# nahomes-15/pointclouds-rs

Hardware: NVIDIA B200
Metric: sor_normals_points_per_sec (higher is better)
Workload: dtype f32

## Files before the change

include/pcr_b200.h:

```cpp
#ifndef PCR_B200_H
#define PCR_B200_H

#include <stddef.h>
#include <stdint.h>

#ifdef __cplusplus
extern "C" {
#endif

#define PCR_B200_VERSION 122

typedef enum pcr_status {
    PCR_OK = 0,
    PCR_ERR_INVALID_ARG = 1,
    PCR_ERR_NORMALS_MISMATCH = 2,
    PCR_ERR_CUDA = 3,
    PCR_ERR_NCCL = 4,
    PCR_ERR_OOM = 5,
    PCR_ERR_NO_DEVICE = 6,
    PCR_ERR_UNSUPPORTED = 7,
    PCR_ERR_CAPACITY = 8
} pcr_status;

#define PCR_MAX_K 1024

typedef struct pcr_ctx pcr_ctx;
typedef struct pcr_index pcr_index;

int pcr_version(void);
int pcr_device_count(void);
int pcr_ctx_create(int device, pcr_ctx **out);
int pcr_ctx_create_on_stream(int device, void *cuda_stream, pcr_ctx **out);
void pcr_ctx_destroy(pcr_ctx *ctx);
int pcr_ctx_synchronize(pcr_ctx *ctx);
const char *pcr_last_error(const pcr_ctx *ctx);
uint64_t pcr_ctx_launch_count(const pcr_ctx *ctx);
#define PCR_NUM_TIMING_TAGS 8
int pcr_ctx_set_timing(pcr_ctx *ctx, int enable);
int pcr_ctx_get_timing(pcr_ctx *ctx, double *ms_per_tag ,
                       uint64_t *spans_per_tag );
int pcr_ctx_get_knn_counters(pcr_ctx *ctx, uint64_t out[2]);
int pcr_ctx_set_cell_size(pcr_ctx *ctx, float cell_size);
int pcr_ctx_set_frame_stream(pcr_ctx *ctx, int enable);
#define PCR_NUM_HINT_STATS 8
int pcr_ctx_get_hint_stats(pcr_ctx *ctx, uint64_t out[PCR_NUM_HINT_STATS]);

#define PCR_UNIQUE_ID_BYTES 128
int pcr_comm_unique_id(void *out_id );
int pcr_ctx_comm_init(pcr_ctx *ctx, const void *id, int rank, int world_size);
int pcr_ctx_comm_rank(const pcr_ctx *ctx);
int pcr_ctx_comm_size(const pcr_ctx *ctx);
#define PCR_COMM_NONE 0
#define PCR_COMM_NCCL 1
#define PCR_COMM_PEER 2
int pcr_ctx_comm_kind(const pcr_ctx *ctx);
int pcr_ctx_set_query_sharding(pcr_ctx *ctx, int enable);
int pcr_ctx_debug_set_shard(pcr_ctx *ctx, int rank, int world_size);

int pcr_index_build(pcr_ctx *ctx, const float *x, const float *y, const float *z, size_t n,
                    size_t k_hint, pcr_index **out);
int pcr_index_build_dev(pcr_ctx *ctx, const float *d_x, const float *d_y, const float *d_z, size_t n,
                        size_t k_hint, pcr_index **out);
void pcr_index_free(pcr_index *index);
size_t pcr_index_len(const pcr_index *index);
int pcr_index_info(const pcr_index *index, float *cell_size, int32_t dims[3], size_t *n_indexed);

int pcr_knn(pcr_index *index, const float *qx, const float *qy, const float *qz, size_t nq,
            size_t k, uint32_t *idx, float *dist, uint32_t *counts);
int pcr_knn_dev(pcr_index *index, const float *d_qx, const float *d_qy, const float *d_qz, size_t nq,
                size_t k, uint32_t *d_idx, float *d_dist, uint32_t *d_counts);

int pcr_radius_count(pcr_index *index, const float *qx, const float *qy, const float *qz, size_t nq,
                     float radius, uint32_t *counts);
int pcr_radius_search(pcr_index *index, const float *qx, const float *qy, const float *qz, size_t nq,
                      float radius, uint64_t *offsets, uint32_t *idx, size_t cap, size_t *total);

int pcr_index_build_batch(pcr_ctx *ctx, const float *x, const float *y, const float *z,
                          const uint64_t *frame_offsets, size_t n_frames, size_t k_hint, pcr_index **out);
int pcr_index_build_batch_dev(pcr_ctx *ctx, const float *d_x, const float *d_y, const float *d_z,
                              const uint64_t *frame_offsets , size_t n_frames, size_t k_hint, pcr_index **out);
int pcr_knn_batch(pcr_index *index, const float *qx, const float *qy, const float *qz,
                  const uint64_t *query_offsets, size_t n_frames, size_t k, uint32_t *idx, float *dist, uint32_t *counts);
int pcr_knn_batch_dev(pcr_index *index, const float *d_qx, const float *d_qy, const float *d_qz,
                      const uint64_t *query_offsets , size_t n_frames, size_t k, uint32_t *d_idx,
                      float *d_dist, uint32_t *d_counts);
int pcr_radius_count_batch(pcr_index *index, const float *qx, const float *qy, const float *qz,
                           const uint64_t *query_offsets, size_t n_frames, float radius, uint32_t *counts);
int pcr_radius_count_batch_dev(pcr_index *index, const float *d_qx, const float *d_qy, const float *d_qz,
                               const uint64_t *query_offsets , size_t n_frames, float radius,
                               uint32_t *d_counts);
int pcr_radius_search_batch(pcr_index *index, const float *qx, const float *qy, const float *qz,
                            const uint64_t *query_offsets, size_t n_frames, float radius, uint64_t *offsets,
                            uint32_t *idx, size_t cap, size_t *total);
int pcr_find_correspondences_batch(pcr_index *target, const float *sx, const float *sy, const float *sz,
                                   const uint64_t *query_offsets, size_t n_frames, float max_distance,
                                   uint32_t *src_idx, uint32_t *tgt_idx, float *dist, uint64_t *corr_offsets);

int pcr_sor(pcr_ctx *ctx, const float *x, const float *y, const float *z, size_t n, size_t k,
            float std_mul, uint8_t *keep, size_t *n_kept, float *mean_d, float *stats);
int pcr_sor_dev(pcr_ctx *ctx, const float *d_x, const float *d_y, const float *d_z, size_t n,
                size_t k, float std_mul, uint8_t *d_keep, float *d_mean_d );
int pcr_radius_outlier(pcr_ctx *ctx, const float *x, const float *y, const float *z, size_t n,
                       float radius, size_t min_neighbors, uint8_t *keep, size_t *n_kept);

int pcr_radius_outlier_dev(pcr_ctx *ctx, const float *d_x, const float *d_y, const float *d_z, size_t n,
                           float radius, size_t min_neighbors, uint8_t *d_keep);
int pcr_radius_outlier_batch(pcr_ctx *ctx, const float *x, const float *y, const float *z, const uint64_t *frame_offsets,
                             size_t n_frames, float radius, size_t min_neighbors, uint8_t *keep, uint64_t *n_kept_per_frame);
int pcr_radius_outlier_batch_dev(pcr_ctx *ctx, const float *d_x, const float *d_y, const float *d_z, const uint64_t *frame_offsets,
                                 size_t n_frames, float radius, size_t min_neighbors, uint8_t *d_keep);

int pcr_estimate_normals(pcr_ctx *ctx, const float *x, const float *y, const float *z, size_t n,
                         size_t k, const float viewpoint[3], float *nx, float *ny, float *nz);
int pcr_estimate_normals_dev(pcr_ctx *ctx, const float *d_x, const float *d_y, const float *d_z,
                             size_t n, size_t k, const float viewpoint[3], float *d_nx, float *d_ny,
                             float *d_nz);

typedef struct pcr_icp_params {
    uint64_t max_iterations;
    float tolerance;
    float max_correspondence_distance;
} pcr_icp_params;

typedef struct pcr_icp_result {
    float rotation[9];
    float translation[3];
    float fitness;
    float rmse;
    int32_t converged;
    uint64_t num_iterations;
} pcr_icp_result;

int pcr_find_correspondences(pcr_index *target, const float *sx, const float *sy, const float *sz,
                             size_t ns, float max_distance, uint32_t *src_idx, uint32_t *tgt_idx,
                             float *dist, size_t *count);
int pcr_apply_transform(pcr_ctx *ctx, const float *x, const float *y, const float *z, size_t n,
                        const float rotation[9], const float translation[3], float *ox, float *oy,
                        float *oz);
int pcr_apply_transform_batch(pcr_ctx *ctx, const float *x, const float *y, const float *z,
                              const uint64_t *frame_offsets, size_t n_frames, const float *transforms,
                              float *ox, float *oy, float *oz);
int pcr_apply_transform_batch_dev(pcr_ctx *ctx, const float *d_x, const float *d_y, const float *d_z,
                                  const uint64_t *frame_offsets, size_t n_frames, const float *transforms,
                                  float *d_ox, float *d_oy, float *d_oz);
int pcr_transform_compose(const float first[12], const float then[12], float out[12]);
int pcr_icp_point_to_point(pcr_ctx *ctx, const float *sx, const float *sy, const float *sz, size_t ns,
                           const float *tx, const float *ty, const float *tz, size_t nt,
                           const pcr_icp_params *params, pcr_icp_result *result);
int pcr_icp_point_to_plane(pcr_ctx *ctx, const float *sx, const float *sy, const float *sz, size_t ns,
                           const float *tx, const float *ty, const float *tz, size_t nt,
                           const float *nx, const float *ny, const float *nz, size_t n_normals,
                           const pcr_icp_params *params, pcr_icp_result *result);
int pcr_icp_point_to_point_dev(pcr_ctx *ctx, const float *d_sx, const float *d_sy, const float *d_sz,
                               size_t ns, const float *d_tx, const float *d_ty, const float *d_tz,
                               size_t nt, const pcr_icp_params *params, pcr_icp_result *result);
int pcr_icp_point_to_plane_dev(pcr_ctx *ctx, const float *d_sx, const float *d_sy, const float *d_sz,
                               size_t ns, const float *d_tx, const float *d_ty, const float *d_tz,
                               size_t nt, const float *d_nx, const float *d_ny, const float *d_nz,
                               size_t n_normals, const pcr_icp_params *params, pcr_icp_result *result);

int pcr_icp_point_to_point_batch(pcr_ctx *ctx, const float *x, const float *y, const float *z,
                                 const uint64_t *frame_offsets, size_t n_frames,
                                 const uint32_t *pairs, size_t n_pairs,
                                 const pcr_icp_params *params, pcr_icp_result *results );
int pcr_icp_point_to_plane_batch(pcr_ctx *ctx, const float *x, const float *y, const float *z,
                                 const uint64_t *frame_offsets, size_t n_frames,
                                 const float *nx, const float *ny, const float *nz, size_t n_normals,
                                 const uint32_t *pairs, size_t n_pairs,
                                 const pcr_icp_params *params, pcr_icp_result *results);
int pcr_icp_point_to_point_batch_dev(pcr_ctx *ctx, const float *d_x, const float *d_y, const float *d_z,
                                     const uint64_t *frame_offsets, size_t n_frames,
                                     const uint32_t *pairs, size_t n_pairs,
                                     const pcr_icp_params *params, pcr_icp_result *results);
int pcr_icp_point_to_plane_batch_dev(pcr_ctx *ctx, const float *d_x, const float *d_y, const float *d_z,
                                     const uint64_t *frame_offsets, size_t n_frames,
                                     const float *d_nx, const float *d_ny, const float *d_nz, size_t n_normals,
                                     const uint32_t *pairs, size_t n_pairs,
                                     const pcr_icp_params *params, pcr_icp_result *results);

int pcr_voxel_downsample(pcr_ctx *ctx, const float *x, const float *y, const float *z, size_t n,
                         float voxel_size, float *ox, float *oy, float *oz, size_t *n_out);
int pcr_voxel_downsample_dev(pcr_ctx *ctx, const float *d_x, const float *d_y, const float *d_z,
                             size_t n, float voxel_size, float *d_ox, float *d_oy, float *d_oz,
                             size_t *n_out);

int pcr_euclidean_cluster(pcr_ctx *ctx, const float *x, const float *y, const float *z, size_t n,
                          float distance_threshold, size_t min_size, size_t max_size,
                          uint32_t *offsets, uint32_t *indices, size_t *n_clusters);
int pcr_cluster_labels_dev(pcr_ctx *ctx, const float *d_x, const float *d_y, const float *d_z,
                           size_t n, float distance_threshold, uint32_t *d_labels);

typedef struct pcr_cloud pcr_cloud;

int pcr_ransac_plane_samples(pcr_ctx *ctx, const float *x, const float *y, const float *z, size_t n,
                             float distance_threshold, const uint32_t *samples, size_t m, float model[4],
                             uint32_t *inliers, size_t *n_inliers);
int pcr_cloud_ransac_plane_samples(const pcr_cloud *cloud, float distance_threshold, const uint32_t *samples,
                                   size_t m, float model[4], uint32_t *inliers, size_t *n_inliers);
// ... 117 lines not shown
```

pointclouds_rs_b200/__init__.py:

```python
from __future__ import annotations

import ctypes as C
import math
import os
import weakref
from typing import List, Optional, Sequence

import numpy as np

from . import _ffi
from ._ffi import PcrError

__all__ = [
    "PointCloud", "KdTree", "IcpResult", "Context",
    "statistical_outlier_removal", "radius_outlier_removal", "estimate_normals",
    "icp_point_to_point", "icp_point_to_plane", "apply_transform", "find_correspondences",
    "icp_point_to_point_batch", "icp_point_to_plane_batch", "voxel_downsample_batch", "estimate_normals_batch",
    "sor_normals_batch", "default_context", "PcrError", "euclidean_cluster", "voxel_downsample", "DeviceCloud", "ransac_plane", "PlaneResult",
    "ransac_plane_samples_batch", "ransac_plane_batch", "cluster_arrays_batch", "euclidean_cluster_batch",
    "DeviceFrames", "radius_outlier_removal_batch", "KdTreeBatch", "apply_transform_batch", "compose", "chain_poses",
]


def _p(a: Optional[np.ndarray], t):
    return a.ctypes.data_as(t) if a is not None else None


class Context:

    def __init__(self, device: Optional[int] = None, stream: Optional[int] = None):
        lib = _ffi.load()
        if device is None:
            device = int(os.environ.get("LOCAL_RANK", "0"))
            if lib.pcr_device_count() and device >= lib.pcr_device_count():
                device = 0
        h = C.c_void_p()
        if stream is None:
            st = lib.pcr_ctx_create(device, C.byref(h))
        else:
            st = lib.pcr_ctx_create_on_stream(device, C.c_void_p(stream), C.byref(h))
        _ffi.check(st)
        self._h = h
        self.device = device
        self._clouds = weakref.WeakSet()

    def close(self):
        if getattr(self, "_h", None):
            for cl in list(getattr(self, "_clouds", ())):
                cl.free()
            _ffi.load().pcr_ctx_destroy(self._h)
            self._h = None

    def __del__(self):
        try:
            self.close()
        except Exception:
            pass

    def synchronize(self):
        _ffi.check(_ffi.load().pcr_ctx_synchronize(self._h), self._h)

    @property
    def launch_count(self) -> int:
        return int(_ffi.load().pcr_ctx_launch_count(self._h))

    def set_timing(self, enable: bool):
        _ffi.check(_ffi.load().pcr_ctx_set_timing(self._h, 1 if enable else 0), self._h)

    def get_timing(self):
        ms = (C.c_double * _ffi.PCR_NUM_TIMING_TAGS)()
        cnt = (C.c_uint64 * _ffi.PCR_NUM_TIMING_TAGS)()
        _ffi.check(_ffi.load().pcr_ctx_get_timing(self._h, ms, cnt), self._h)
        return {_ffi.TIMING_TAGS[i]: (ms[i], int(cnt[i])) for i in range(_ffi.PCR_NUM_TIMING_TAGS)}

    def set_frame_stream(self, enable: bool = True):
        _ffi.check(_ffi.load().pcr_ctx_set_frame_stream(self._h, 1 if enable else 0), self._h)

    def knn_counters(self) -> dict:
        out = (C.c_uint64 * 2)()
        _ffi.check(_ffi.load().pcr_ctx_get_knn_counters(self._h, out), self._h)
        return {"queries": int(out[0]), "candidates": int(out[1])}

    def hint_stats(self) -> dict:
        out = (C.c_uint64 * 8)()
        _ffi.check(_ffi.load().pcr_ctx_get_hint_stats(self._h, out), self._h)
        names = ("cell_size_reused", "cell_size_probed", "voxel_box_guess_held", "voxel_box_guess_missed", "coarser_level_ahead_needed",
                 "coarser_level_ahead_unneeded", "deferred_counts_not_awaited_zero", "deferred_counts_not_awaited_nonzero")
        return {k: int(v) for k, v in zip(names, out)}

    def set_query_sharding(self, enable: bool = True):
        _ffi.check(_ffi.load().pcr_ctx_set_query_sharding(self._h, 1 if enable else 0), self._h)

    def debug_set_shard(self, rank: int, world_size: int):
        _ffi.check(_ffi.load().pcr_ctx_debug_set_shard(self._h, int(rank), int(world_size)), self._h)

    def set_cell_size(self, cell: float):
        _ffi.check(_ffi.load().pcr_ctx_set_cell_size(self._h, float(cell)), self._h)

    @staticmethod
    def unique_id() -> bytes:
        buf = C.create_string_buffer(_ffi.PCR_UNIQUE_ID_BYTES)
        _ffi.check(_ffi.load().pcr_comm_unique_id(buf))
        return buf.raw

    def comm_init(self, uid: bytes, rank: int, world_size: int):
        buf = C.create_string_buffer(uid, _ffi.PCR_UNIQUE_ID_BYTES)
        _ffi.check(_ffi.load().pcr_ctx_comm_init(self._h, buf, rank, world_size), self._h)

    @property
    def comm_kind(self) -> str:
        return ("none", "nccl", "peer")[_ffi.load().pcr_ctx_comm_kind(self._h)]


_default_ctx: Optional[Context] = None


def default_context() -> Context:
    global _default_ctx
    if _default_ctx is None:
        _default_ctx = Context()
    return _default_ctx


def _soa(a: np.ndarray):
    x = np.ascontiguousarray(a[:, 0])
    y = np.ascontiguousarray(a[:, 1])
    z = np.ascontiguousarray(a[:, 2])
    return x, y, z


class PointCloud:

    def __init__(self):
        self.x = np.empty(0, np.float32)
        self.y = np.empty(0, np.float32)
        self.z = np.empty(0, np.float32)
        self.normals: Optional[np.ndarray] = None
        self._nsoa = None

    @staticmethod
    def _from_xyz(x, y, z, normals=None) -> "PointCloud":
        pc = PointCloud()
        pc.x, pc.y, pc.z = x, y, z
        pc.normals = normals
        return pc

    @staticmethod
    def from_numpy(array) -> "PointCloud":
        if not isinstance(array, np.ndarray) or array.dtype not in (np.float32, np.float64):
            raise TypeError("expected NumPy array with dtype float32 or float64, shape (N, 3)")
        if array.ndim != 2:
            raise TypeError("expected NumPy array with dtype float32 or float64, shape (N, 3)")
        if not array.flags["C_CONTIGUOUS"]:
            raise ValueError("array must be C-contiguous (row-major). Use numpy.ascontiguousarray(arr) to convert.")
        if array.shape[1] != 3:
            raise ValueError("expected shape (N, 3)")
        a = array.astype(np.float32, copy=False)
        return PointCloud._from_xyz(*_soa(a))

    def _normals_soa(self):
        if self._nsoa is None or self._nsoa[0] is not self.normals:
            self._nsoa = (self.normals, _soa(np.asarray(self.normals, np.float32).reshape(-1, 3)))
        return self._nsoa[1]

    def to_numpy(self) -> np.ndarray:
        return np.stack([self.x, self.y, self.z], axis=1) if len(self.x) else np.zeros((0, 3), np.float32)

    def normals_to_numpy(self) -> Optional[np.ndarray]:
        return None if self.normals is None else self.normals.copy()

    def len(self) -> int:
        return int(len(self.x))

    def is_empty(self) -> bool:
        return len(self.x) == 0

    def __len__(self) -> int:
        return int(len(self.x))

    def __repr__(self) -> str:
        return f"PointCloud(n={len(self.x)})"

    def select(self, indices: Sequence[int]) -> "PointCloud":
        idx = np.asarray(indices, dtype=np.int64).reshape(-1)
        n = len(self.x)
        bad = idx[(idx >= n) | (idx < 0)]
        if len(bad):
            raise IndexError(f"index {int(bad[0])} out of bounds for cloud with {n} points")
        nr = None if self.normals is None else self.normals[idx]
        return PointCloud._from_xyz(self.x[idx], self.y[idx], self.z[idx], nr)

    def select_inverse(self, indices: Sequence[int]) -> "PointCloud":
        idx = np.asarray(indices, dtype=np.int64).reshape(-1)
        n = len(self.x)
        bad = idx[(idx >= n) | (idx < 0)]
        if len(bad):
            raise IndexError(f"index {int(bad[0])} out of bounds for cloud with {n} points")
        keep = np.ones(n, bool)
        keep[idx] = False
        return self.select(np.nonzero(keep)[0])


class KdTree:

    def __init__(self, cloud: PointCloud, k_hint: int = 0, ctx: Optional[Context] = None):
        self._ctx = ctx or default_context()
        lib = _ffi.load()
        h = C.c_void_p()
        self._n = len(cloud)
        st = lib.pcr_index_build(self._ctx._h, _p(cloud.x, _ffi.f32p), _p(cloud.y, _ffi.f32p), _p(cloud.z, _ffi.f32p),
                                 self._n, k_hint, C.byref(h))
        _ffi.check(st, self._ctx._h)
        self._h = h

    def __del__(self):
        try:
            if getattr(self, "_h", None):
                _ffi.load().pcr_index_free(self._h)
                self._h = None
        except Exception:
            pass

    def len(self) -> int:
        return int(_ffi.load().pcr_index_len(self._h))

    __len__ = len

    def is_empty(self) -> bool:
        return self.len() == 0

    def info(self):
        cell = C.c_float()
        dims = (C.c_int32 * 3)()
        n_idx = C.c_size_t()
        _ffi.check(_ffi.load().pcr_index_info(self._h, C.byref(cell), dims, C.byref(n_idx)))
        return {"cell_size": cell.value, "dims": list(dims), "n_indexed": n_idx.value}

    def knn(self, queries: np.ndarray, k: int):
        q = np.ascontiguousarray(np.asarray(queries, np.float32).reshape(-1, 3))
        qx, qy, qz = _soa(q)
# ... 1035 lines not shown
```

pointclouds_rs_b200/_ffi.py:

```python
from __future__ import annotations

import ctypes as C
import os

_HERE = os.path.dirname(os.path.abspath(__file__))
LIB_PATH = os.environ.get("PCR_LIB_OVERRIDE") or os.path.join(_HERE, "lib", "libpcr_b200.so")

PCR_OK = 0
PCR_ERR_INVALID_ARG = 1
PCR_ERR_NORMALS_MISMATCH = 2
PCR_ERR_CUDA = 3
PCR_ERR_NCCL = 4
PCR_ERR_OOM = 5
PCR_ERR_NO_DEVICE = 6
PCR_ERR_UNSUPPORTED = 7
PCR_ERR_CAPACITY = 8
PCR_MAX_K = 1024
PCR_UNIQUE_ID_BYTES = 128
PCR_NUM_TIMING_TAGS = 8
TIMING_TAGS = ("build", "knn", "knn_deferred", "sor_stats", "icp_step", "icp_solve", "knn_normals", "other")

f32p = C.POINTER(C.c_float)
u32p = C.POINTER(C.c_uint32)
u64p = C.POINTER(C.c_uint64)
u8p = C.POINTER(C.c_uint8)
i32p = C.POINTER(C.c_int32)
szp = C.POINTER(C.c_size_t)
vp = C.c_void_p


class IcpParams(C.Structure):
    _fields_ = [("max_iterations", C.c_uint64), ("tolerance", C.c_float), ("max_correspondence_distance", C.c_float)]


class IcpResultC(C.Structure):
    _fields_ = [
        ("rotation", C.c_float * 9),
        ("translation", C.c_float * 3),
        ("fitness", C.c_float),
        ("rmse", C.c_float),
        ("converged", C.c_int32),
        ("num_iterations", C.c_uint64),
    ]


class PcrError(RuntimeError):
    def __init__(self, code: int, message: str):
        super().__init__(f"pcr_b200 error {code}: {message}")
        self.code = code
        self.message = message


SIGNATURES = {
    "pcr_version": (C.c_int, []),
    "pcr_device_count": (C.c_int, []),
    "pcr_ctx_create": (C.c_int, [C.c_int, C.POINTER(vp)]),
    "pcr_ctx_create_on_stream": (C.c_int, [C.c_int, vp, C.POINTER(vp)]),
    "pcr_ctx_destroy": (None, [vp]),
    "pcr_ctx_synchronize": (C.c_int, [vp]),
    "pcr_last_error": (C.c_char_p, [vp]),
    "pcr_ctx_launch_count": (C.c_uint64, [vp]),
    "pcr_ctx_set_cell_size": (C.c_int, [vp, C.c_float]),
    "pcr_ctx_set_frame_stream": (C.c_int, [vp, C.c_int]),
    "pcr_ctx_get_hint_stats": (C.c_int, [vp, u64p]),
    "pcr_ctx_get_knn_counters": (C.c_int, [vp, u64p]),
    "pcr_ctx_set_query_sharding": (C.c_int, [vp, C.c_int]),
    "pcr_ctx_debug_set_shard": (C.c_int, [vp, C.c_int, C.c_int]),
    "pcr_ctx_set_timing": (C.c_int, [vp, C.c_int]),
    "pcr_ctx_get_timing": (C.c_int, [vp, C.POINTER(C.c_double), u64p]),
    "pcr_comm_unique_id": (C.c_int, [vp]),
    "pcr_ctx_comm_init": (C.c_int, [vp, vp, C.c_int, C.c_int]),
    "pcr_ctx_comm_rank": (C.c_int, [vp]),
    "pcr_ctx_comm_size": (C.c_int, [vp]),
    "pcr_ctx_comm_kind": (C.c_int, [vp]),
    "pcr_index_build": (C.c_int, [vp, f32p, f32p, f32p, C.c_size_t, C.c_size_t, C.POINTER(vp)]),
    "pcr_index_build_dev": (C.c_int, [vp, vp, vp, vp, C.c_size_t, C.c_size_t, C.POINTER(vp)]),
    "pcr_index_free": (None, [vp]),
    "pcr_index_len": (C.c_size_t, [vp]),
    "pcr_index_info": (C.c_int, [vp, f32p, i32p, szp]),
    "pcr_knn": (C.c_int, [vp, f32p, f32p, f32p, C.c_size_t, C.c_size_t, u32p, f32p, u32p]),
    "pcr_knn_dev": (C.c_int, [vp, vp, vp, vp, C.c_size_t, C.c_size_t, vp, vp, vp]),
    "pcr_radius_count": (C.c_int, [vp, f32p, f32p, f32p, C.c_size_t, C.c_float, u32p]),
    "pcr_radius_search": (C.c_int, [vp, f32p, f32p, f32p, C.c_size_t, C.c_float, u64p, u32p, C.c_size_t, szp]),
    "pcr_index_build_batch": (C.c_int, [vp, f32p, f32p, f32p, u64p, C.c_size_t, C.c_size_t, C.POINTER(vp)]),
    "pcr_index_build_batch_dev": (C.c_int, [vp, vp, vp, vp, u64p, C.c_size_t, C.c_size_t, C.POINTER(vp)]),
    "pcr_knn_batch": (C.c_int, [vp, f32p, f32p, f32p, u64p, C.c_size_t, C.c_size_t, u32p, f32p, u32p]),
    "pcr_knn_batch_dev": (C.c_int, [vp, vp, vp, vp, u64p, C.c_size_t, C.c_size_t, vp, vp, vp]),
    "pcr_radius_count_batch": (C.c_int, [vp, f32p, f32p, f32p, u64p, C.c_size_t, C.c_float, u32p]),
    "pcr_radius_count_batch_dev": (C.c_int, [vp, vp, vp, vp, u64p, C.c_size_t, C.c_float, vp]),
    "pcr_radius_search_batch": (C.c_int, [vp, f32p, f32p, f32p, u64p, C.c_size_t, C.c_float, u64p, u32p, C.c_size_t, szp]),
    "pcr_find_correspondences_batch": (C.c_int, [vp, f32p, f32p, f32p, u64p, C.c_size_t, C.c_float, u32p, u32p, f32p, u64p]),
    "pcr_sor": (C.c_int, [vp, f32p, f32p, f32p, C.c_size_t, C.c_size_t, C.c_float, u8p, szp, f32p, f32p]),
    "pcr_sor_dev": (C.c_int, [vp, vp, vp, vp, C.c_size_t, C.c_size_t, C.c_float, vp, vp]),
    "pcr_radius_outlier": (C.c_int, [vp, f32p, f32p, f32p, C.c_size_t, C.c_float, C.c_size_t, u8p, szp]),
    "pcr_estimate_normals": (C.c_int, [vp, f32p, f32p, f32p, C.c_size_t, C.c_size_t, f32p, f32p, f32p, f32p]),
    "pcr_estimate_normals_dev": (C.c_int, [vp, vp, vp, vp, C.c_size_t, C.c_size_t, f32p, vp, vp, vp]),
    "pcr_find_correspondences": (C.c_int, [vp, f32p, f32p, f32p, C.c_size_t, C.c_float, u32p, u32p, f32p, szp]),
    "pcr_apply_transform": (C.c_int, [vp, f32p, f32p, f32p, C.c_size_t, f32p, f32p, f32p, f32p, f32p]),
    "pcr_icp_point_to_point": (C.c_int, [vp, f32p, f32p, f32p, C.c_size_t, f32p, f32p, f32p, C.c_size_t, C.POINTER(IcpParams), C.POINTER(IcpResultC)]),
    "pcr_icp_point_to_plane": (C.c_int, [vp, f32p, f32p, f32p, C.c_size_t, f32p, f32p, f32p, C.c_size_t, f32p, f32p, f32p, C.c_size_t, C.POINTER(IcpParams), C.POINTER(IcpResultC)]),
    "pcr_icp_point_to_point_dev": (C.c_int, [vp, vp, vp, vp, C.c_size_t, vp, vp, vp, C.c_size_t, C.POINTER(IcpParams), C.POINTER(IcpResultC)]),
    "pcr_icp_point_to_plane_dev": (C.c_int, [vp, vp, vp, vp, C.c_size_t, vp, vp, vp, C.c_size_t, vp, vp, vp, C.c_size_t, C.POINTER(IcpParams), C.POINTER(IcpResultC)]),
    "pcr_icp_point_to_point_batch": (C.c_int, [vp, f32p, f32p, f32p, u64p, C.c_size_t, u32p, C.c_size_t, C.POINTER(IcpParams), C.POINTER(IcpResultC)]),
    "pcr_icp_point_to_plane_batch": (C.c_int, [vp, f32p, f32p, f32p, u64p, C.c_size_t, f32p, f32p, f32p, C.c_size_t, u32p, C.c_size_t,
                                               C.POINTER(IcpParams), C.POINTER(IcpResultC)]),
    "pcr_icp_point_to_point_batch_dev": (C.c_int, [vp, vp, vp, vp, u64p, C.c_size_t, u32p, C.c_size_t, C.POINTER(IcpParams), C.POINTER(IcpResultC)]),
    "pcr_icp_point_to_plane_batch_dev": (C.c_int, [vp, vp, vp, vp, u64p, C.c_size_t, vp, vp, vp, C.c_size_t, u32p, C.c_size_t,
                                                   C.POINTER(IcpParams), C.POINTER(IcpResultC)]),
    "pcr_voxel_downsample": (C.c_int, [vp, f32p, f32p, f32p, C.c_size_t, C.c_float, f32p, f32p, f32p, szp]),
    "pcr_voxel_downsample_dev": (C.c_int, [vp, vp, vp, vp, C.c_size_t, C.c_float, vp, vp, vp, szp]),
    "pcr_voxel_downsample_batch": (C.c_int, [vp, f32p, f32p, f32p, u64p, C.c_size_t, C.c_float, f32p, f32p, f32p, u64p]),
    "pcr_voxel_downsample_batch_dev": (C.c_int, [vp, vp, vp, vp, u64p, C.c_size_t, C.c_float, vp, vp, vp, u64p]),
    "pcr_estimate_normals_batch": (C.c_int, [vp, f32p, f32p, f32p, u64p, C.c_size_t, C.c_size_t, f32p, f32p, f32p, f32p]),
    "pcr_estimate_normals_batch_dev": (C.c_int, [vp, vp, vp, vp, u64p, C.c_size_t, C.c_size_t, f32p, vp, vp, vp]),
    "pcr_euclidean_cluster": (C.c_int, [vp, f32p, f32p, f32p, C.c_size_t, C.c_float, C.c_size_t, C.c_size_t, u32p, u32p, szp]),
    "pcr_cluster_labels_dev": (C.c_int, [vp, vp, vp, vp, C.c_size_t, C.c_float, vp]),
    "pcr_radius_outlier_dev": (C.c_int, [vp, vp, vp, vp, C.c_size_t, C.c_float, C.c_size_t, vp]),
    "pcr_cloud_upload": (C.c_int, [vp, vp, vp, vp, C.c_size_t, C.POINTER(vp)]),
    "pcr_cloud_upload_block": (C.c_int, [vp, vp, C.c_size_t, C.c_size_t, C.POINTER(vp)]),
    "pcr_cloud_upload_block_nowait": (C.c_int, [vp, vp, C.c_size_t, C.c_size_t, C.POINTER(vp)]),
    "pcr_cloud_download_block": (C.c_int, [vp, vp, C.c_size_t, C.c_int]),
    "pcr_cloud_free": (None, [vp]),
    "pcr_cloud_len": (C.c_size_t, [vp]),
    "pcr_cloud_has_normals": (C.c_int, [vp]),
    "pcr_cloud_download": (C.c_int, [vp, vp, vp, vp]),
    "pcr_cloud_download_normals": (C.c_int, [vp, vp, vp, vp]),
    "pcr_cloud_upload_rows": (C.c_int, [vp, vp, C.c_size_t, C.POINTER(vp)]),
    "pcr_cloud_download_rows": (C.c_int, [vp, vp, vp]),
    "pcr_cloud_device_pointers": (C.c_int, [vp] + [C.POINTER(vp)] * 6),
    "pcr_cloud_select": (C.c_int, [vp, u32p, C.c_size_t, C.POINTER(vp)]),
    "pcr_cloud_voxel_downsample": (C.c_int, [vp, C.c_float, C.POINTER(vp)]),
    "pcr_cloud_statistical_outlier_removal": (C.c_int, [vp, C.c_size_t, C.c_float, C.POINTER(vp)]),
    "pcr_cloud_radius_outlier_removal": (C.c_int, [vp, C.c_float, C.c_size_t, C.POINTER(vp)]),
    "pcr_cloud_estimate_normals": (C.c_int, [vp, C.c_size_t, f32p, C.POINTER(vp)]),
    "pcr_cloud_sor_normals": (C.c_int, [vp, C.c_size_t, C.c_float, C.c_size_t, f32p, C.POINTER(vp)]),
    "pcr_cloud_euclidean_cluster": (C.c_int, [vp, C.c_float, C.c_size_t, C.c_size_t, u32p, u32p, szp]),
    "pcr_cloud_apply_transform": (C.c_int, [vp, f32p, f32p, C.POINTER(vp)]),
    "pcr_cloud_icp_point_to_point": (C.c_int, [vp, vp, C.POINTER(IcpParams), C.POINTER(IcpResultC)]),
    "pcr_cloud_icp_point_to_plane": (C.c_int, [vp, vp, C.POINTER(IcpParams), C.POINTER(IcpResultC)]),
    "pcr_ransac_plane_samples": (C.c_int, [vp, f32p, f32p, f32p, C.c_size_t, C.c_float, u32p, C.c_size_t, f32p, u32p, szp]),
    "pcr_cloud_ransac_plane_samples": (C.c_int, [vp, C.c_float, u32p, C.c_size_t, f32p, u32p, szp]),
    "pcr_ransac_plane_samples_batch": (C.c_int, [vp, f32p, f32p, f32p, u64p, C.c_size_t, C.c_float, u32p, u64p, f32p, u32p, u64p]),
    "pcr_ransac_plane_samples_batch_dev": (C.c_int, [vp, vp, vp, vp, u64p, C.c_size_t, C.c_float, u32p, u64p, f32p, vp, u64p]),
    "pcr_euclidean_cluster_batch": (C.c_int, [vp, f32p, f32p, f32p, u64p, C.c_size_t, C.c_float, C.c_size_t, C.c_size_t, u32p, u32p, u64p]),
    "pcr_euclidean_cluster_batch_dev": (C.c_int, [vp, vp, vp, vp, u64p, C.c_size_t, C.c_float, C.c_size_t, C.c_size_t, vp, vp, u64p]),
    "pcr_cluster_labels_batch_dev": (C.c_int, [vp, vp, vp, vp, u64p, C.c_size_t, C.c_float, vp]),
    "pcr_sor_normals_batch": (C.c_int, [vp, f32p, f32p, f32p, u64p, C.c_size_t, C.c_size_t, C.c_float, C.c_size_t, f32p, u8p, f32p, f32p, f32p, u64p]),
    "pcr_sor_normals_batch_rows": (C.c_int, [vp, f32p, u64p, C.c_size_t, C.c_size_t, C.c_float, C.c_size_t, f32p, u8p, f32p, u64p]),
    "pcr_sor_normals_batch_dev": (C.c_int, [vp, vp, vp, vp, u64p, C.c_size_t, C.c_size_t, C.c_float, C.c_size_t, f32p, vp, vp, vp, vp]),
    "pcr_radius_outlier_batch": (C.c_int, [vp, f32p, f32p, f32p, u64p, C.c_size_t, C.c_float, C.c_size_t, u8p, u64p]),
    "pcr_radius_outlier_batch_dev": (C.c_int, [vp, vp, vp, vp, u64p, C.c_size_t, C.c_float, C.c_size_t, vp]),
    "pcr_frames_upload": (C.c_int, [vp, vp, vp, vp, u64p, C.c_size_t, C.POINTER(vp)]),
    "pcr_frames_upload_rows": (C.c_int, [vp, vp, u64p, C.c_size_t, C.POINTER(vp)]),
    "pcr_frames_free": (None, [vp]),
    "pcr_frames_len": (C.c_size_t, [vp]),
    "pcr_frames_count": (C.c_size_t, [vp]),
    "pcr_frames_offsets": (C.c_int, [vp, u64p]),
    "pcr_frames_has_normals": (C.c_int, [vp]),
    "pcr_frames_device_pointers": (C.c_int, [vp] + [C.POINTER(vp)] * 6),
    "pcr_frames_download": (C.c_int, [vp, vp, vp, vp, vp, vp, vp]),
    "pcr_frames_download_rows": (C.c_int, [vp, vp, vp]),
    "pcr_frames_frame": (C.c_int, [vp, C.c_size_t, C.POINTER(vp)]),
    "pcr_frames_merge": (C.c_int, [vp, C.POINTER(vp)]),
    "pcr_frames_apply_transform": (C.c_int, [vp, f32p, C.POINTER(vp)]),
    "pcr_apply_transform_batch": (C.c_int, [vp, f32p, f32p, f32p, u64p, C.c_size_t, f32p, f32p, f32p, f32p]),
    "pcr_apply_transform_batch_dev": (C.c_int, [vp, vp, vp, vp, u64p, C.c_size_t, f32p, vp, vp, vp]),
    "pcr_transform_compose": (C.c_int, [f32p, f32p, f32p]),
    "pcr_frames_select": (C.c_int, [vp, u32p, u64p, C.c_int, C.POINTER(vp)]),
    "pcr_frames_voxel_downsample": (C.c_int, [vp, C.c_float, C.POINTER(vp)]),
    "pcr_frames_statistical_outlier_removal": (C.c_int, [vp, C.c_size_t, C.c_float, C.POINTER(vp)]),
    "pcr_frames_radius_outlier_removal": (C.c_int, [vp, C.c_float, C.c_size_t, C.POINTER(vp)]),
    "pcr_frames_estimate_normals": (C.c_int, [vp, C.c_size_t, f32p, C.POINTER(vp)]),
    "pcr_frames_sor_normals": (C.c_int, [vp, C.c_size_t, C.c_float, C.c_size_t, f32p, C.POINTER(vp)]),
    "pcr_frames_ransac_plane_samples": (C.c_int, [vp, C.c_float, u32p, u64p, f32p, u32p, u64p, C.POINTER(vp)]),
    "pcr_frames_euclidean_cluster": (C.c_int, [vp, C.c_float, C.c_size_t, C.c_size_t, u32p, u32p, u64p]),
    "pcr_frames_icp_point_to_point": (C.c_int, [vp, u32p, C.c_size_t, C.POINTER(IcpParams), C.POINTER(IcpResultC)]),
    "pcr_frames_icp_point_to_plane": (C.c_int, [vp, u32p, C.c_size_t, C.POINTER(IcpParams), C.POINTER(IcpResultC)]),
}

_lib = None


def load():
    global _lib
    if _lib is None:
        if not os.path.exists(LIB_PATH):
            raise ImportError(
                f"{LIB_PATH} is missing: build the CUDA extension first "
                "(python -c 'import __graft_entry__ as g; g.build()'). There is no CPU fallback."
            )
        L = C.CDLL(LIB_PATH, mode=C.RTLD_GLOBAL)
        for name, (res, args) in SIGNATURES.items():
            fn = getattr(L, name)
            fn.restype = res
            fn.argtypes = args
        _lib = L
    return _lib


def last_error(ctx=None) -> str:
    msg = load().pcr_last_error(ctx)
    return msg.decode(errors="replace") if msg else "unknown error"


def check(status: int, ctx=None):
    if status != PCR_OK:
        msg = last_error(ctx)
        if status == PCR_ERR_INVALID_ARG or status == PCR_ERR_NORMALS_MISMATCH:
            raise ValueError(msg)
        raise PcrError(status, msg)
```

pointclouds_rs_b200/csrc/api.cu:

```cuda
#include "pcr_internal.cuh"

#include <stdarg.h>

#include <atomic>
#include <chrono>
#include <cstring>
#include <utility>
#include <vector>
#include <algorithm>
#include <new>

namespace pcr {

static thread_local std::string g_thread_error = "no error";
static thread_local uint64_t g_thread_err_seq = 0;
static std::atomic<uint64_t> g_err_seq{0};

void set_thread_error(const char *msg) {
    g_thread_error = msg ? msg : "unknown error";
    g_thread_err_seq = ++g_err_seq;
}

int fail(Ctx *ctx, int code, const char *fmt, ...) {
    char buf[512];
    va_list ap;
    va_start(ap, fmt);
    vsnprintf(buf, sizeof(buf), fmt, ap);
    va_end(ap);
    g_thread_error = buf;
    g_thread_err_seq = ++g_err_seq;
    if (ctx) {
        ctx->err = buf;
        ctx->err_seq = g_thread_err_seq;
    }
    return code;
}

TimeScope::TimeScope(Ctx *ctx, int tag) : c(ctx) {
    if (!c->timing) return;
    Ctx::TimedSpan sp;
    sp.tag = tag;
    for (cudaEvent_t *e : {&sp.a, &sp.b}) {
        if (!c->event_pool.empty()) {
            *e = c->event_pool.back();
            c->event_pool.pop_back();
        } else if (cudaEventCreate(e) != cudaSuccess) {
            cudaGetLastError();
            return;
        }
    }
    cudaEventRecord(sp.a, c->stream);
    idx = (int)c->spans.size();
    c->spans.push_back(sp);
}
TimeScope::~TimeScope() {
    if (idx >= 0) cudaEventRecord(c->spans[idx].b, c->stream);
}

bool g_trace_on = getenv("PCR_TRACE") != nullptr;
namespace {
thread_local std::vector<std::pair<const char *, double>> t_trace;
}
static void trace_dump();
static const double g_trace_slow_us = getenv("PCR_TRACE_SLOW_US") ? atof(getenv("PCR_TRACE_SLOW_US")) : 0.0;
void trace_mark(const char *label) {
    const size_t len = strlen(label);
    if (g_trace_slow_us > 0.0 && len >= 5 && !strcmp(label + len - 5, "enter")) t_trace.clear();
    t_trace.emplace_back(label, std::chrono::duration<double, std::micro>(std::chrono::steady_clock::now().time_since_epoch()).count());
    if (g_trace_slow_us > 0.0 && len >= 4 && !strcmp(label + len - 4, "exit")) {
        if (t_trace.back().second - t_trace.front().second > g_trace_slow_us) trace_dump();
        else t_trace.clear();
    }
}
static void trace_dump() {
    if (!g_trace_on || t_trace.empty()) return;
    const size_t n = t_trace.size(), b = n > 160 ? n - 160 : 0;
    for (size_t i = b; i < n; i++)
        fprintf(stderr, "[trace] %9.1f us  +%6.1f  %s\n", t_trace[i].second - t_trace[b].second, i > b ? t_trace[i].second - t_trace[i - 1].second : 0.0,
                t_trace[i].first);
    t_trace.clear();
}

int ensure(Ctx *ctx, DevBuf &b, size_t bytes) {
    if (bytes <= b.cap) return PCR_OK;
    size_t want = std::max(bytes, b.cap + b.cap / 2);
    want = (want + 255) & ~(size_t)255;
    if (b.p) {
        PCR_CUDA(ctx, cudaFreeAsync(b.p, ctx->stream));
        b.p = nullptr;
        b.cap = 0;
    }
    PCR_CUDA(ctx, cudaMallocAsync(&b.p, want, ctx->stream));
    b.cap = want;
    return PCR_OK;
}

int ensure_pinned(Ctx *ctx, size_t bytes) {
    if (bytes <= ctx->pinned_cap) return PCR_OK;
    size_t want = std::max<size_t>(bytes, 1 << 16);
    if (ctx->pinned) {
        PCR_CUDA(ctx, cudaStreamSynchronize(ctx->stream));
        cudaFreeHost(ctx->pinned);
        ctx->pinned = nullptr;
        ctx->pinned_cap = 0;
    }
    PCR_CUDA(ctx, cudaHostAlloc(&ctx->pinned, want, cudaHostAllocMapped | cudaHostAllocPortable));
    ctx->pinned_cap = want;
    return PCR_OK;
}

namespace {

void free_buf(Ctx *ctx, DevBuf &b) {
    if (b.p) cudaFreeAsync(b.p, ctx->stream);
    b.p = nullptr;
    b.cap = 0;
}

int ctx_create(int device, void *stream, bool have_stream, Ctx **out) {
    *out = nullptr;
    int count = 0;
    cudaError_t e = cudaGetDeviceCount(&count);
    if (e != cudaSuccess || count == 0) {
        cudaGetLastError();
        return fail(nullptr, PCR_ERR_NO_DEVICE, "no CUDA device available (%s); this library has no CPU fallback",
                    e != cudaSuccess ? cudaGetErrorString(e) : "device count is 0");
    }
    if (device < 0 || device >= count) return fail(nullptr, PCR_ERR_INVALID_ARG, "device %d out of range [0,%d)", device, count);
    Ctx *ctx = new (std::nothrow) Ctx();
    if (!ctx) return fail(nullptr, PCR_ERR_OOM, "host allocation failed");
    ctx->device = device;
    struct Guard {
        Ctx *c;
        ~Guard() {
            if (!c) return;
            if (c->pinned) cudaFreeHost(c->pinned);
            if (c->owns_stream && c->stream) cudaStreamDestroy(c->stream);
            delete c;
        }
    } g{ctx};
    PCR_CUDA(ctx, cudaSetDevice(device));
    cudaDeviceProp prop;
    PCR_CUDA(ctx, cudaGetDeviceProperties(&prop, device));
    if (prop.major < 10)
        return fail(nullptr, PCR_ERR_NO_DEVICE, "device %d is sm_%d%d; this library is built for sm_100a only", device, prop.major,
                    prop.minor);
    ctx->sm_count = prop.multiProcessorCount;
    if (have_stream) {
        ctx->stream = (cudaStream_t)stream;
        ctx->owns_stream = false;
    } else {
        PCR_CUDA(ctx, cudaStreamCreateWithFlags(&ctx->stream, cudaStreamNonBlocking));
        ctx->owns_stream = true;
    }
    cudaMemPool_t pool;
    if (cudaDeviceGetDefaultMemPool(&pool, device) == cudaSuccess) {
        uint64_t thr = UINT64_MAX;
        cudaMemPoolSetAttribute(pool, cudaMemPoolAttrReleaseThreshold, &thr);
    }
    cudaGetLastError();
    PCR_TRY(ensure_pinned(ctx, 1 << 16));
    g.c = nullptr;
    *out = ctx;
    return PCR_OK;
}

struct DevSetter {
    int prev = -1;
    explicit DevSetter(Ctx *c) {
        cudaGetDevice(&prev);
        if (prev != c->device) cudaSetDevice(c->device);
        else prev = -1;
    }
    ~DevSetter() {
        if (prev >= 0) cudaSetDevice(prev);
    }
};

int stage_xyz(Ctx *ctx, DevBuf &buf, const float *x, const float *y, const float *z, size_t n, float **dx, float **dy, float **dz) {
    size_t stride = (n + 63) & ~(size_t)63;
    PCR_TRY(ensure(ctx, buf, sizeof(float) * 3 * std::max<size_t>(stride, 64)));
    float *base = (float *)buf.p;
    *dx = base;
    *dy = base + stride;
    *dz = base + 2 * stride;
    if (n) {
        PCR_CUDA(ctx, cudaMemcpyAsync(*dx, x, sizeof(float) * n, cudaMemcpyHostToDevice, ctx->stream));
        PCR_CUDA(ctx, cudaMemcpyAsync(*dy, y, sizeof(float) * n, cudaMemcpyHostToDevice, ctx->stream));
        PCR_CUDA(ctx, cudaMemcpyAsync(*dz, z, sizeof(float) * n, cudaMemcpyHostToDevice, ctx->stream));
    }
    return PCR_OK;
}

#define PCR_API_BEGIN try {
#define PCR_API_END(ctx_expr)                                                         \
    }                                                                                 \
    catch (const std::bad_alloc &) { return pcr::fail((ctx_expr), PCR_ERR_OOM, "host allocation failed"); } \
    catch (...) { return pcr::fail((ctx_expr), PCR_ERR_CUDA, "unexpected C++ exception"); }

}
}

using namespace pcr;


extern "C" {

int pcr_version(void) { return PCR_B200_VERSION; }

int pcr_device_count(void) {
    int count = 0;
    if (cudaGetDeviceCount(&count) != cudaSuccess) {
        cudaGetLastError();
        return 0;
    }
    return count;
}

const char *pcr_last_error(const pcr_ctx *ctx) {
    if (ctx && !ctx->c.err.empty() && ctx->c.err_seq >= g_thread_err_seq) return ctx->c.err.c_str();
    return g_thread_error.c_str();
}

static int create_common(int device, void *stream, bool have, pcr_ctx **out) {
    if (!out) return fail(nullptr, PCR_ERR_INVALID_ARG, "out is NULL");
    *out = nullptr;
    PCR_API_BEGIN
    Ctx *c = nullptr;
    PCR_TRY(ctx_create(device, stream, have, &c));
    pcr_ctx *w = new (std::nothrow) pcr_ctx();
    if (!w) {
        delete c;
        return fail(nullptr, PCR_ERR_OOM, "host allocation failed");
    }
    w->c = *c;
    delete c;
    *out = w;
    return PCR_OK;
    PCR_API_END(nullptr)
}

int pcr_ctx_create(int device, pcr_ctx **out) { return create_common(device, nullptr, false, out); }
int pcr_ctx_create_on_stream(int device, void *cuda_stream, pcr_ctx **out) { return create_common(device, cuda_stream, true, out); }

void pcr_ctx_destroy(pcr_ctx *ctx) {
    if (!ctx) return;
    trace_dump();
    Ctx *c = &ctx->c;
    DevSetter ds(c);
    cudaStreamSynchronize(c->stream);
    comm_destroy(c);
    free_buf(c, c->b_in);
    free_buf(c, c->b_in2);
    free_buf(c, c->b_out);
    free_buf(c, c->b_misc);
    free_buf(c, c->b_misc2);
    free_buf(c, c->b_small);
    free_buf(c, c->b_table);
    free_buf(c, c->b_scan);
    free_buf(c, c->b_fine_misc);
    free_buf(c, c->b_fine_scan);
    free_buf(c, c->b_list);
    free_buf(c, c->b_qoff);
    for (auto &b : c->b_cells) free_buf(c, b);
    for (auto &b : c->b_lsorted) free_buf(c, b);
    for (auto &b : c->b_lgrids) free_buf(c, b);
    cudaStreamSynchronize(c->stream);
    for (auto &sp : c->spans) {
        cudaEventDestroy(sp.a);
        cudaEventDestroy(sp.b);
    }
    for (auto e : c->event_pool) cudaEventDestroy(e);
    if (c->d_knn_stats) cudaFree(c->d_knn_stats);
    for (int i = 0; i < 2; i++) {
        if (c->side[i]) cudaStreamDestroy(c->side[i]);
        if (c->ev_join[i]) cudaEventDestroy(c->ev_join[i]);
    }
    if (c->ev_fork) cudaEventDestroy(c->ev_fork);
    if (c->ev_count) cudaEventDestroy(c->ev_count);
    if (c->pinned) cudaFreeHost(c->pinned);
    if (c->owns_stream) cudaStreamDestroy(c->stream);
    cudaGetLastError();
    delete ctx;
}

int pcr_ctx_synchronize(pcr_ctx *ctx) {
    if (!ctx) return fail(nullptr, PCR_ERR_INVALID_ARG, "ctx is NULL");
    DevSetter ds(&ctx->c);
    PCR_CUDA(&ctx->c, cudaStreamSynchronize(ctx->c.stream));
    return PCR_OK;
}

uint64_t pcr_ctx_launch_count(const pcr_ctx *ctx) { return ctx ? ctx->c.launches : 0; }

int pcr_ctx_set_timing(pcr_ctx *ctx, int enable) {
    if (!ctx) return fail(nullptr, PCR_ERR_INVALID_ARG, "ctx is NULL");
    Ctx *c = &ctx->c;
    c->timing = enable != 0;
    if (c->timing && !c->d_knn_stats) {
        DevSetter ds(c);
        PCR_CUDA(c, cudaMalloc((void **)&c->d_knn_stats, 2 * sizeof(unsigned long long)));
        PCR_CUDA(c, cudaMemsetAsync(c->d_knn_stats, 0, 2 * sizeof(unsigned long long), c->stream));
    }
    return PCR_OK;
}

int pcr_ctx_get_timing(pcr_ctx *ctx, double *ms_per_tag, uint64_t *spans_per_tag) {
    if (!ctx || !ms_per_tag) return fail(nullptr, PCR_ERR_INVALID_ARG, "null pointer");
    Ctx *c = &ctx->c;
    DevSetter ds(c);
    PCR_CUDA(c, cudaStreamSynchronize(c->stream));
    for (int t = 0; t < PCR_NUM_TIMING_TAGS; t++) {
        ms_per_tag[t] = 0.0;
        if (spans_per_tag) spans_per_tag[t] = 0;
    }
    for (auto &sp : c->spans) {
        float ms = 0.f;
        if (cudaEventElapsedTime(&ms, sp.a, sp.b) == cudaSuccess && sp.tag >= 0 && sp.tag < PCR_NUM_TIMING_TAGS) {
            ms_per_tag[sp.tag] += ms;
            if (spans_per_tag) spans_per_tag[sp.tag]++;
        }
        c->event_pool.push_back(sp.a);
        c->event_pool.push_back(sp.b);
    }
    cudaGetLastError();
    c->spans.clear();
    return PCR_OK;
}

int pcr_ctx_get_knn_counters(pcr_ctx *ctx, uint64_t out[2]) {
    if (!ctx || !out) return fail(ctx ? &ctx->c : nullptr, PCR_ERR_INVALID_ARG, "null pointer");
    Ctx *c = &ctx->c;
    out[0] = out[1] = 0;
    if (!c->d_knn_stats) return PCR_OK;
    DevSetter ds(c);
    unsigned long long h[2] = {0, 0};
    PCR_CUDA(c, cudaMemcpyAsync(h, c->d_knn_stats, sizeof(h), cudaMemcpyDeviceToHost, c->stream));
    PCR_CUDA(c, cudaMemsetAsync(c->d_knn_stats, 0, sizeof(h), c->stream));
    PCR_CUDA(c, cudaStreamSynchronize(c->stream));
    out[0] = h[0];
    out[1] = h[1];
    return PCR_OK;
}

int pcr_ctx_set_frame_stream(pcr_ctx *ctx, int enable) {
    if (!ctx) return fail(nullptr, PCR_ERR_INVALID_ARG, "ctx is NULL");
    ctx->c.frame_stream = enable != 0;
    ctx->c.cell_cache.valid = false;
    ctx->c.vox_cache.valid = false;
    return PCR_OK;
}

int pcr_ctx_set_query_sharding(pcr_ctx *ctx, int enable) {
    if (!ctx) return fail(nullptr, PCR_ERR_INVALID_ARG, "ctx is NULL");
    ctx->c.shard_queries = enable != 0;
    return PCR_OK;
}

int pcr_ctx_debug_set_shard(pcr_ctx *ctx, int rank, int world_size) {
    if (!ctx) return fail(nullptr, PCR_ERR_INVALID_ARG, "ctx is NULL");
    Ctx *c = &ctx->c;
    if (world_size < 1 || rank < 0 || rank >= world_size) return fail(c, PCR_ERR_INVALID_ARG, "bad rank/world");
    comm_destroy(c);
    c->rank = rank;
    c->world = world_size;
    c->fake_comm = world_size > 1;
    return PCR_OK;
}

int pcr_ctx_get_hint_stats(pcr_ctx *ctx, uint64_t out[PCR_NUM_HINT_STATS]) {
    if (!ctx || !out) return fail(ctx ? &ctx->c : nullptr, PCR_ERR_INVALID_ARG, "null pointer");
    const Ctx &c = ctx->c;
    const uint64_t v[PCR_NUM_HINT_STATS] = {c.stat_cell_hits, c.stat_cell_misses, c.stat_vox_hits, c.stat_vox_misses, c.stat_spec_hits, c.stat_spec_misses,
                                             c.stat_nowait_hits, c.stat_nowait_misses};
    for (int i = 0; i < PCR_NUM_HINT_STATS; i++) out[i] = v[i];
    return PCR_OK;
}

int pcr_ctx_set_cell_size(pcr_ctx *ctx, float cell_size) {
    if (!ctx) return fail(nullptr, PCR_ERR_INVALID_ARG, "ctx is NULL");
    if (!(cell_size >= 0.f) || !std::isfinite(cell_size)) return fail(&ctx->c, PCR_ERR_INVALID_ARG, "cell_size must be >= 0 and finite");
    ctx->c.forced_cell = cell_size;
    return PCR_OK;
}

int pcr_comm_unique_id(void *out_id) {
    if (!out_id) return fail(nullptr, PCR_ERR_INVALID_ARG, "out_id is NULL");
    PCR_API_BEGIN
    return comm_unique_id(out_id);
    PCR_API_END(nullptr)
}
int pcr_ctx_comm_init(pcr_ctx *ctx, const void *id, int rank, int world_size) {
    if (!ctx || !id) return fail(nullptr, PCR_ERR_INVALID_ARG, "ctx/id is NULL");
    PCR_API_BEGIN
    DevSetter ds(&ctx->c);
    return comm_init(&ctx->c, id, rank, world_size);
    PCR_API_END(&ctx->c)
}
int pcr_ctx_comm_rank(const pcr_ctx *ctx) { return ctx ? ctx->c.rank : 0; }
int pcr_ctx_comm_size(const pcr_ctx *ctx) { return ctx ? ctx->c.world : 1; }
int pcr_ctx_comm_kind(const pcr_ctx *ctx) {
    if (!ctx || ctx->c.world <= 1 || ctx->c.fake_comm) return PCR_COMM_NONE;
    return ctx->c.peer_ok ? PCR_COMM_PEER : PCR_COMM_NCCL;
}

static int wrap_index(pcr_ctx *ctx, Index *ix, pcr_index **out) {
    pcr_index *w = new (std::nothrow) pcr_index();
    if (!w) {
        index_free(ix);
        return fail(&ctx->c, PCR_ERR_OOM, "host allocation failed");
    }
    w->ix = ix;
    w->owner = ctx;
    *out = w;
    return PCR_OK;
}

int pcr_index_build_dev(pcr_ctx *ctx, const float *d_x, const float *d_y, const float *d_z, size_t n, size_t k_hint,
                        pcr_index **out) {
    if (!ctx || !out) return fail(nullptr, PCR_ERR_INVALID_ARG, "ctx/out is NULL");
    *out = nullptr;
    if (n && (!d_x || !d_y || !d_z)) return fail(&ctx->c, PCR_ERR_INVALID_ARG, "x/y/z is NULL");
    PCR_API_BEGIN
    DevSetter ds(&ctx->c);
    BuildOpts bo;
    bo.k_hint = k_hint;
    Index *ix = nullptr;
    PCR_TRY(index_build_dev(&ctx->c, d_x, d_y, d_z, n, bo, &ix));
    return wrap_index(ctx, ix, out);
    PCR_API_END(&ctx->c)
}

int pcr_index_build(pcr_ctx *ctx, const float *x, const float *y, const float *z, size_t n, size_t k_hint, pcr_index **out) {
    if (!ctx || !out) return fail(nullptr, PCR_ERR_INVALID_ARG, "ctx/out is NULL");
    *out = nullptr;
    if (n && (!x || !y || !z)) return fail(&ctx->c, PCR_ERR_INVALID_ARG, "x/y/z is NULL");
    PCR_API_BEGIN
    Ctx *c = &ctx->c;
    DevSetter ds(c);
    float *dx, *dy, *dz;
    PCR_TRY(stage_xyz(c, c->b_in, x, y, z, n, &dx, &dy, &dz));
    BuildOpts bo;
    bo.k_hint = k_hint;
    Index *ix = nullptr;
    PCR_TRY(index_build_dev(c, dx, dy, dz, n, bo, &ix));
    PCR_CUDA(c, cudaStreamSynchronize(c->stream));
    return wrap_index(ctx, ix, out);
    PCR_API_END(&ctx->c)
}

void pcr_index_free(pcr_index *index) {
    if (!index) return;
    if (index->ix) {
        DevSetter ds(index->ix->ctx);
        index_free(index->ix);
    }
    delete index;
}

size_t pcr_index_len(const pcr_index *index) { return index && index->ix ? index->ix->n : 0; }

int pcr_index_info(const pcr_index *index, float *cell_size, int32_t dims[3], size_t *n_indexed) {
    if (!index || !index->ix) return fail(nullptr, PCR_ERR_INVALID_ARG, "index is NULL");
    const GridDesc &g = index->ix->grids_h[0];
    if (cell_size) *cell_size = (float)g.h;
    if (dims)
        for (int j = 0; j < 3; j++) dims[g.ax[j]] = g.dims[j];
    if (n_indexed) *n_indexed = index->ix->n_indexed;
    return PCR_OK;
}

static int single_cloud_check(const Index *ix, const char *batch_call) {
    if (ix->n_frames == 1) return PCR_OK;
    return fail(ix->ctx, PCR_ERR_INVALID_ARG, "the index holds %d frames: query it with %s", ix->n_frames, batch_call);
}

int pcr_knn_dev(pcr_index *index, const float *d_qx, const float *d_qy, const float *d_qz, size_t nq, size_t k, uint32_t *d_idx,
                float *d_dist, uint32_t *d_counts) {
    if (!index || !index->ix) return fail(nullptr, PCR_ERR_INVALID_ARG, "index is NULL");
    Ctx *c = index->ix->ctx;
    PCR_TRY(single_cloud_check(index->ix, "pcr_knn_batch_dev"));
    if (nq && k && (!d_qx || !d_qy || !d_qz || !d_idx)) return fail(c, PCR_ERR_INVALID_ARG, "null query/output pointer");
    PCR_API_BEGIN
    DevSetter ds(c);
    if (k == 0 && d_counts && nq) PCR_CUDA(c, cudaMemsetAsync(d_counts, 0, sizeof(uint32_t) * nq, c->stream));
    return knn_queries_dev(index->ix, d_qx, d_qy, d_qz, nq, k, d_idx, d_dist, d_counts);
    PCR_API_END(c)
}

int pcr_knn(pcr_index *index, const float *qx, const float *qy, const float *qz, size_t nq, size_t k, uint32_t *idx, float *dist,
            uint32_t *counts) {
    if (!index || !index->ix) return fail(nullptr, PCR_ERR_INVALID_ARG, "index is NULL");
    Ctx *c = index->ix->ctx;
    PCR_TRY(single_cloud_check(index->ix, "pcr_knn_batch"));
    if (nq == 0) return PCR_OK;
    if (!qx || !qy || !qz) return fail(c, PCR_ERR_INVALID_ARG, "null query pointer");
    if (k == 0) {
        if (counts) memset(counts, 0, sizeof(uint32_t) * nq);
        return PCR_OK;
    }
    if (!idx) return fail(c, PCR_ERR_INVALID_ARG, "idx is NULL");
    if (k > PCR_MAX_K) return fail(c, PCR_ERR_UNSUPPORTED, "k = %zu exceeds PCR_MAX_K = %d", k, PCR_MAX_K);
    PCR_API_BEGIN
    DevSetter ds(c);
    float *dx, *dy, *dz;
    PCR_TRY(stage_xyz(c, c->b_in2, qx, qy, qz, nq, &dx, &dy, &dz));
    size_t rows = nq * k;
    size_t bytes = rows * sizeof(uint32_t) + (dist ? rows * sizeof(float) : 0) + nq * sizeof(uint32_t) + 512;
    PCR_TRY(ensure(c, c->b_out, bytes));
    uint32_t *d_idx = (uint32_t *)c->b_out.p;
    float *d_dist = dist ? (float *)(d_idx + rows) : nullptr;
    uint32_t *d_cnt = (uint32_t *)((char *)c->b_out.p + rows * sizeof(uint32_t) + (dist ? rows * sizeof(float) : 0));
    PCR_TRY(knn_queries_dev(index->ix, dx, dy, dz, nq, k, d_idx, d_dist, d_cnt));
    PCR_CUDA(c, cudaMemcpyAsync(idx, d_idx, rows * sizeof(uint32_t), cudaMemcpyDeviceToHost, c->stream));
    if (dist) PCR_CUDA(c, cudaMemcpyAsync(dist, d_dist, rows * sizeof(float), cudaMemcpyDeviceToHost, c->stream));
    if (counts) PCR_CUDA(c, cudaMemcpyAsync(counts, d_cnt, nq * sizeof(uint32_t), cudaMemcpyDeviceToHost, c->stream));
    PCR_CUDA(c, cudaStreamSynchronize(c->stream));
    return PCR_OK;
    PCR_API_END(c)
}

int pcr_radius_count(pcr_index *index, const float *qx, const float *qy, const float *qz, size_t nq, float radius,
                     uint32_t *counts) {
    if (!index || !index->ix) return fail(nullptr, PCR_ERR_INVALID_ARG, "index is NULL");
    Ctx *c = index->ix->ctx;
    PCR_TRY(single_cloud_check(index->ix, "pcr_radius_count_batch"));
    if (nq == 0) return PCR_OK;
    if (!qx || !qy || !qz || !counts) return fail(c, PCR_ERR_INVALID_ARG, "null pointer");
// ... 920 lines not shown
        return euclidean_cluster_batch_dev(c, x, y, z, frame_offsets, n_frames, distance_threshold, min_size, max_size, offsets, indices,
                                           cluster_offsets, &total);
    const float *dx = x, *dy = y, *dz = z;
    if (!in_dev) {
        float *sx, *sy, *sz;
        PCR_TRY(stage_xyz(c, c->b_in, x, y, z, n, &sx, &sy, &sz));
        dx = sx, dy = sy, dz = sz;
    }
    PCR_TRY(ensure(c, c->b_out, sizeof(uint32_t) * (2 * n + 1)));
    uint32_t *d_off = (uint32_t *)c->b_out.p, *d_idx = d_off + n + 1;
    PCR_TRY(euclidean_cluster_batch_dev(c, dx, dy, dz, frame_offsets, n_frames, distance_threshold, min_size, max_size, d_off, d_idx,
                                        cluster_offsets, &total));
    const size_t k = (size_t)cluster_offsets[n_frames];
    if (k) {
        PCR_CUDA(c, cudaMemcpyAsync(offsets, d_off, sizeof(uint32_t) * (k + 1), cudaMemcpyDeviceToHost, c->stream));
        PCR_CUDA(c, cudaMemcpyAsync(indices, d_idx, sizeof(uint32_t) * total, cudaMemcpyDeviceToHost, c->stream));
        PCR_CUDA(c, cudaStreamSynchronize(c->stream));
    }
    return PCR_OK;
    PCR_API_END(c)
}

int pcr_euclidean_cluster_batch(pcr_ctx *ctx, const float *x, const float *y, const float *z, const uint64_t *frame_offsets, size_t n_frames,
                                float distance_threshold, size_t min_size, size_t max_size, uint32_t *offsets, uint32_t *indices,
                                uint64_t *cluster_offsets) {
    return cluster_batch_entry(ctx, false, false, x, y, z, frame_offsets, n_frames, distance_threshold, min_size, max_size, offsets, indices,
                               cluster_offsets);
}
int pcr_euclidean_cluster_batch_dev(pcr_ctx *ctx, const float *d_x, const float *d_y, const float *d_z, const uint64_t *frame_offsets,
                                    size_t n_frames, float distance_threshold, size_t min_size, size_t max_size, uint32_t *d_offsets,
                                    uint32_t *d_indices, uint64_t *cluster_offsets) {
    return cluster_batch_entry(ctx, true, true, d_x, d_y, d_z, frame_offsets, n_frames, distance_threshold, min_size, max_size, d_offsets, d_indices,
                               cluster_offsets);
}

int pcr_cluster_labels_batch_dev(pcr_ctx *ctx, const float *d_x, const float *d_y, const float *d_z, const uint64_t *frame_offsets,
                                 size_t n_frames, float distance_threshold, uint32_t *d_labels) {
    if (!ctx) return fail(nullptr, PCR_ERR_INVALID_ARG, "ctx is NULL");
    Ctx *c = &ctx->c;
    PCR_TRY(offsets_check(c, "frame_offsets", frame_offsets, n_frames));
    const size_t n = (size_t)frame_offsets[n_frames];
    PCR_TRY(batch_size_check(c, n, n_frames));
    if (n && (!d_x || !d_y || !d_z || !d_labels)) return fail(c, PCR_ERR_INVALID_ARG, "null pointer");
    if (distance_threshold <= 0.0f) return fail(c, PCR_ERR_INVALID_ARG, "distance_threshold must be > 0");
    if (n == 0) return PCR_OK;
    PCR_API_BEGIN
    DevSetter ds(c);
    return cluster_labels_batch_dev(c, d_x, d_y, d_z, frame_offsets, n_frames, distance_threshold, d_labels);
    PCR_API_END(c)
}

static int ror_batch_entry(pcr_ctx *ctx, bool dev, const float *x, const float *y, const float *z, const uint64_t *frame_offsets,
                           size_t n_frames, float radius, size_t min_neighbors, uint8_t *keep, uint64_t *n_kept_per_frame) {
    if (!ctx) return fail(nullptr, PCR_ERR_INVALID_ARG, "ctx is NULL");
    Ctx *c = &ctx->c;
    PCR_TRY(offsets_check(c, "frame_offsets", frame_offsets, n_frames));
    if (n_kept_per_frame)
        for (size_t f = 0; f < n_frames; f++) n_kept_per_frame[f] = 0;
    const size_t n = (size_t)frame_offsets[n_frames];
    PCR_TRY(batch_size_check(c, n, n_frames));
    if (n && (!x || !y || !z || !keep)) return fail(c, PCR_ERR_INVALID_ARG, "null pointer");
    if (n == 0) return PCR_OK;
    PCR_API_BEGIN
    DevSetter ds(c);
    if (dev) {
        PCR_TRY(ensure(c, c->b_small, 4096));
        return ror_core(c, x, y, z, n, radius, min_neighbors, keep, (unsigned long long *)((char *)c->b_small.p + 1024), frame_offsets,
                        n_frames);
    }
    float *dx, *dy, *dz;
    PCR_TRY(stage_xyz(c, c->b_in, x, y, z, n, &dx, &dy, &dz));
    const size_t o_kept = (n + 255) & ~(size_t)255;
    PCR_TRY(ensure(c, c->b_out, o_kept + 64));
    uint8_t *d_keep = (uint8_t *)c->b_out.p;
    PCR_TRY(ror_core(c, dx, dy, dz, n, radius, min_neighbors, d_keep, (unsigned long long *)((char *)c->b_out.p + o_kept), frame_offsets,
                     n_frames));
    PCR_CUDA(c, cudaMemcpyAsync(keep, d_keep, n, cudaMemcpyDeviceToHost, c->stream));
    PCR_CUDA(c, cudaStreamSynchronize(c->stream));
    if (n_kept_per_frame)
        for (size_t f = 0; f < n_frames; f++)
            for (uint64_t i = frame_offsets[f]; i < frame_offsets[f + 1]; i++) n_kept_per_frame[f] += keep[i];
    return PCR_OK;
    PCR_API_END(c)
}

int pcr_radius_outlier_batch(pcr_ctx *ctx, const float *x, const float *y, const float *z, const uint64_t *frame_offsets, size_t n_frames,
                             float radius, size_t min_neighbors, uint8_t *keep, uint64_t *n_kept_per_frame) {
    return ror_batch_entry(ctx, false, x, y, z, frame_offsets, n_frames, radius, min_neighbors, keep, n_kept_per_frame);
}
int pcr_radius_outlier_batch_dev(pcr_ctx *ctx, const float *d_x, const float *d_y, const float *d_z, const uint64_t *frame_offsets,
                                 size_t n_frames, float radius, size_t min_neighbors, uint8_t *d_keep) {
    return ror_batch_entry(ctx, true, d_x, d_y, d_z, frame_offsets, n_frames, radius, min_neighbors, d_keep, nullptr);
}

static int apply_transform_batch_entry(pcr_ctx *ctx, bool dev, const float *x, const float *y, const float *z, const uint64_t *frame_offsets,
                                       size_t n_frames, const float *transforms, float *ox, float *oy, float *oz) {
    if (!ctx) return fail(nullptr, PCR_ERR_INVALID_ARG, "ctx is NULL");
    Ctx *c = &ctx->c;
    PCR_TRY(offsets_check(c, "frame_offsets", frame_offsets, n_frames));
    const size_t n = (size_t)frame_offsets[n_frames];
    PCR_TRY(batch_size_check(c, n, n_frames));
    if ((n_frames && !transforms) || (n && (!x || !y || !z || !ox || !oy || !oz))) return fail(c, PCR_ERR_INVALID_ARG, "null pointer");
    if (n == 0) return PCR_OK;
    PCR_API_BEGIN
    DevSetter ds(c);
    if (dev) return apply_transform_batch_dev(c, x, y, z, frame_offsets, n_frames, nullptr, transforms, ox, oy, oz);
    float *dx, *dy, *dz;
    PCR_TRY(stage_xyz(c, c->b_in, x, y, z, n, &dx, &dy, &dz));
    const size_t stride = (n + 63) & ~(size_t)63;
    PCR_TRY(ensure(c, c->b_out, sizeof(float) * 3 * stride));
    float *o0 = (float *)c->b_out.p, *o1 = o0 + stride, *o2 = o1 + stride;
    PCR_TRY(apply_transform_batch_dev(c, dx, dy, dz, frame_offsets, n_frames, nullptr, transforms, o0, o1, o2));
    PCR_CUDA(c, cudaMemcpyAsync(ox, o0, n * sizeof(float), cudaMemcpyDeviceToHost, c->stream));
    PCR_CUDA(c, cudaMemcpyAsync(oy, o1, n * sizeof(float), cudaMemcpyDeviceToHost, c->stream));
    PCR_CUDA(c, cudaMemcpyAsync(oz, o2, n * sizeof(float), cudaMemcpyDeviceToHost, c->stream));
    PCR_CUDA(c, cudaStreamSynchronize(c->stream));
    return PCR_OK;
    PCR_API_END(c)
}

int pcr_apply_transform_batch(pcr_ctx *ctx, const float *x, const float *y, const float *z, const uint64_t *frame_offsets, size_t n_frames,
                              const float *transforms, float *ox, float *oy, float *oz) {
    return apply_transform_batch_entry(ctx, false, x, y, z, frame_offsets, n_frames, transforms, ox, oy, oz);
}
int pcr_apply_transform_batch_dev(pcr_ctx *ctx, const float *d_x, const float *d_y, const float *d_z, const uint64_t *frame_offsets,
                                  size_t n_frames, const float *transforms, float *d_ox, float *d_oy, float *d_oz) {
    return apply_transform_batch_entry(ctx, true, d_x, d_y, d_z, frame_offsets, n_frames, transforms, d_ox, d_oy, d_oz);
}

int pcr_transform_compose(const float first[12], const float then[12], float out[12]) {
    if (!first || !then || !out) return fail(nullptr, PCR_ERR_INVALID_ARG, "null pointer");
    const float *A = then, *B = first;
    float r[12];
    for (int i = 0; i < 3; i++) {
        for (int j = 0; j < 3; j++) r[i * 3 + j] = (A[i * 3 + 0] * B[0 * 3 + j] + A[i * 3 + 1] * B[1 * 3 + j]) + A[i * 3 + 2] * B[2 * 3 + j];
        r[9 + i] = ((A[i * 3 + 0] * B[9] + A[i * 3 + 1] * B[10]) + A[i * 3 + 2] * B[11]) + A[9 + i];
    }
    memcpy(out, r, sizeof(r));
    return PCR_OK;
}

namespace pcr {
__global__ void single_point_frames_kernel(const uint32_t *__restrict__ frame_off, int n_frames, size_t n,
                                           uint8_t *__restrict__ keep, unsigned long long *__restrict__ kept) {
    int f = blockIdx.x * blockDim.x + threadIdx.x;
    if (f >= n_frames) return;
    const size_t b = frame_off ? frame_off[f] : 0, e = frame_off ? frame_off[f + 1] : n;
    if (e - b == 1) {
        keep[b] = 1;
        kept[f] = 1;
    }
}
}
static int batch_core(Ctx *c, const float *dx, const float *dy, const float *dz, const uint64_t *frame_offsets, size_t n_frames,
                      size_t n, size_t k_sor, float std_mul, size_t k_normals, const float vp[3], uint8_t *d_keep, float *d_nx,
                      float *d_ny, float *d_nz, unsigned long long *d_kept ,
                      unsigned long long *h_kept0 = nullptr ,
                      const CloudStats *known_stats = nullptr ,
                      bool allow_nowait = true ) {
    const int F = (int)n_frames;
    StreamAlloc<float> mean_mem(c->stream), stats_mem(c->stream);
    PCR_CUDA(c, mean_mem.alloc(sizeof(float) * std::max<size_t>(n, 1)));
    PCR_CUDA(c, stats_mem.alloc(sizeof(float) * 4 * F));
    float *d_mean = mean_mem.p, *d_stats = stats_mem.p;

    const size_t K = std::max(k_sor, k_normals) + 1;
    static const bool no_fuse = getenv("PCR_NO_LIST_REUSE") != nullptr;
    const bool may_fuse = !no_fuse && k_sor > 0 && k_normals > 0 && K <= 32 && n > 1;
    SorLists sl;
    bool early = false;
    StreamAlloc<uint32_t> list_mem(c->stream);
    if (may_fuse) {
        sl.K = K;
        sl.stride = (n + 63) & ~(size_t)63;
        const size_t bytes = sizeof(uint32_t) * (K * sl.stride + sl.stride + 64) + sl.stride;
        PCR_CUDA(c, list_mem.alloc(bytes));
        sl.lists = list_mem.p;
        sl.fallback = sl.lists + K * sl.stride;
        sl.cnt = (uint8_t *)(sl.fallback + sl.stride + 64);
        PCR_CUDA(c, cudaMemsetAsync(sl.fallback + sl.stride, 0, 64 * sizeof(uint32_t), c->stream));
        PCR_CUDA(c, cudaMemsetAsync(sl.cnt, 0xff, sl.stride, c->stream));
        sl.initialised = true;
        PCR_MARK("core: lists allocated");
    }
    if (k_sor > 0) PCR_CUDA(c, cudaMemsetAsync(d_kept, 0, sizeof(unsigned long long) * F, c->stream));
    BuildOpts bo;
    bo.k_hint = std::max(k_sor + 1, k_normals);
    bo.self_knn = true;
    if (const char *e = getenv("PCR_BATCH_KHINT")) bo.k_hint = (size_t)atoi(e);
    bo.n_frames = F;
    bo.transient = true;
    bo.known_stats = known_stats;
    bo.frame_offsets = frame_offsets;
    Index *ix = nullptr;
    PCR_MARK("core: build begin");
    PCR_TRY(index_build_dev(c, dx, dy, dz, n, bo, &ix));
    PCR_MARK("core: build queued");
    const IndexPtr guard(ix);
    const bool fused = may_fuse && ix->n_indexed > 0;
    struct EarlyJoin {
        Ctx *c;
        bool *armed;
        ~EarlyJoin() {
            if (*armed) cudaStreamWaitEvent(c->stream, c->ev_join[0], 0);
        }
    } early_join{c, &early};
    if (k_sor == 0) {
        PCR_CUDA(c, cudaMemsetAsync(d_keep, 0, n, c->stream));
        PCR_CUDA(c, cudaMemsetAsync(d_kept, 0, sizeof(unsigned long long) * F, c->stream));
    } else {
        c->spec_request = fused && allow_nowait && F == 1 && k_normals > 0 && !c->shard_queries;
        c->spec_pending = false;
        const int ss = sor_mean_dist_dev(ix, k_sor, d_mean, fused ? &sl : nullptr);
        c->spec_request = false;
        PCR_TRY(ss);
        PCR_MARK("core: sor search done");
        if (fused) PCR_TRY(normals_early_fork(c));
        PCR_TRY(sor_threshold_mask_dev(c, d_mean, ix->frame_in_off, F, n, std_mul, d_keep, d_stats, d_kept, true));
        if (fused) PCR_TRY(normals_early_from_lists_dev(ix, k_normals, vp, sl, d_nx, d_ny, d_nz, &early));
        PCR_MARK("core: stats queued");
        if (F > 1 || n == 1) {
            single_point_frames_kernel<<<(F + 127) / 128, 128, 0, c->stream>>>(ix->frame_in_off, F, n, d_keep, d_kept);
            PCR_LAUNCH_CHECK(c);
        }
    }
    if (k_normals == 0) return PCR_OK;
    if (early) PCR_CUDA(c, cudaStreamWaitEvent(c->stream, c->ev_join[0], 0));
    PCR_TRY(index_apply_mask_dev(ix, d_keep));
    if (fused) {
        const int sn = normals_from_lists_dev(ix, k_normals, vp, sl, d_keep, d_nx, d_ny, d_nz, F == 1 ? d_kept : nullptr, h_kept0, early);
        if (c->spec_pending) {
            c->spec_pending = false;
            if (sn == PCR_OK) {
                const uint32_t *m2 = (const uint32_t *)c->pinned + 128;
                const bool zero = m2[0] == 0 && m2[1] == 0;
                c->spec_zero = zero;
                (zero ? c->stat_nowait_hits : c->stat_nowait_misses)++;
                if (!zero)
                    return batch_core(c, dx, dy, dz, frame_offsets, (size_t)F, n, k_sor, std_mul, k_normals, vp, d_keep, d_nx, d_ny, d_nz, d_kept,
                                      h_kept0, known_stats, false);
            }
        }
        return sn;
    }
    return normals_dev(ix, k_normals, vp, d_nx, d_ny, d_nz, d_keep);
}

static int sor_normals_batch_check(Ctx *c, size_t n, size_t n_frames, size_t k_sor, float std_mul, size_t k_normals) {
    if (!std::isfinite(std_mul) || std_mul < 0.f) return fail(c, PCR_ERR_INVALID_ARG, "std_mul must be >= 0 and finite");
    if (k_sor + 1 > PCR_MAX_K || k_normals > PCR_MAX_K) return fail(c, PCR_ERR_UNSUPPORTED, "k exceeds PCR_MAX_K");
    return batch_size_check(c, n, n_frames);
}

int pcr_sor_normals_batch_dev(pcr_ctx *ctx, const float *d_x, const float *d_y, const float *d_z, const uint64_t *frame_offsets,
                              size_t n_frames, size_t k_sor, float std_mul, size_t k_normals, const float viewpoint[3],
                              uint8_t *d_keep, float *d_nx, float *d_ny, float *d_nz) {
    if (!ctx) return fail(nullptr, PCR_ERR_INVALID_ARG, "ctx is NULL");
    Ctx *c = &ctx->c;
    if (n_frames == 0) return PCR_OK;
    PCR_TRY(offsets_check(c, "frame_offsets", frame_offsets, n_frames));
    const size_t n = (size_t)frame_offsets[n_frames];
    if (n == 0) return PCR_OK;
    if (!d_x || !d_y || !d_z || !d_keep || !viewpoint || (k_normals && (!d_nx || !d_ny || !d_nz)))
        return fail(c, PCR_ERR_INVALID_ARG, "null pointer");
    PCR_TRY(sor_normals_batch_check(c, n, n_frames, k_sor, std_mul, k_normals));
    PCR_API_BEGIN
    DevSetter ds(c);
    PCR_MARK("batch_dev: enter");
    StreamAlloc<unsigned long long> d_kept(c->stream);
    PCR_CUDA(c, d_kept.alloc(sizeof(unsigned long long) * n_frames));
    const int s = batch_core(c, d_x, d_y, d_z, frame_offsets, n_frames, n, k_sor, std_mul, k_normals, viewpoint, d_keep, d_nx, d_ny, d_nz,
                             d_kept.p);
    if (g_trace_on) {
        cudaStreamSynchronize(c->stream);
        PCR_MARK("batch_dev: synced, exit");
    }
    return s;
    PCR_API_END(c)
}

int pcr_sor_normals_batch(pcr_ctx *ctx, const float *x, const float *y, const float *z, const uint64_t *frame_offsets, size_t n_frames,
                          size_t k_sor, float std_mul, size_t k_normals, const float viewpoint[3], uint8_t *keep, float *nx, float *ny,
                          float *nz, uint64_t *n_kept_per_frame) {
    if (!ctx) return fail(nullptr, PCR_ERR_INVALID_ARG, "ctx is NULL");
    Ctx *c = &ctx->c;
    if (n_frames == 0) return PCR_OK;
    PCR_TRY(offsets_check(c, "frame_offsets", frame_offsets, n_frames));
    const size_t n = (size_t)frame_offsets[n_frames];
    if (n_kept_per_frame) memset(n_kept_per_frame, 0, sizeof(uint64_t) * n_frames);
    if (n == 0) return PCR_OK;
    if (!x || !y || !z || !keep || !viewpoint || (k_normals && (!nx || !ny || !nz))) return fail(c, PCR_ERR_INVALID_ARG, "null pointer");
    PCR_TRY(sor_normals_batch_check(c, n, n_frames, k_sor, std_mul, k_normals));
    PCR_API_BEGIN
    DevSetter ds(c);
    float *dx, *dy, *dz;
    PCR_TRY(stage_xyz(c, c->b_in, x, y, z, n, &dx, &dy, &dz));
    size_t stride = (n + 63) & ~(size_t)63;
    size_t o_keep = stride * 3 * sizeof(float);
    size_t o_kept = o_keep + ((n + 255) & ~(size_t)255);
    PCR_TRY(ensure(c, c->b_out, o_kept + sizeof(unsigned long long) * n_frames));
    float *dnx = (float *)c->b_out.p, *dny = dnx + stride, *dnz = dny + stride;
    uint8_t *d_keep = (uint8_t *)c->b_out.p + o_keep;
    unsigned long long *d_kept = (unsigned long long *)((char *)c->b_out.p + o_kept);
    PCR_TRY(batch_core(c, dx, dy, dz, frame_offsets, n_frames, n, k_sor, std_mul, k_normals, viewpoint, d_keep, dnx, dny, dnz, d_kept));
    PCR_CUDA(c, cudaMemcpyAsync(keep, d_keep, n, cudaMemcpyDeviceToHost, c->stream));
    if (k_normals) {
        PCR_CUDA(c, cudaMemcpyAsync(nx, dnx, n * sizeof(float), cudaMemcpyDeviceToHost, c->stream));
        PCR_CUDA(c, cudaMemcpyAsync(ny, dny, n * sizeof(float), cudaMemcpyDeviceToHost, c->stream));
        PCR_CUDA(c, cudaMemcpyAsync(nz, dnz, n * sizeof(float), cudaMemcpyDeviceToHost, c->stream));
    }
    std::vector<unsigned long long> hk(n_frames);
    PCR_CUDA(c, cudaMemcpyAsync(hk.data(), d_kept, sizeof(unsigned long long) * n_frames, cudaMemcpyDeviceToHost, c->stream));
    PCR_CUDA(c, cudaStreamSynchronize(c->stream));
    if (n_kept_per_frame)
        for (size_t f = 0; f < n_frames; f++) n_kept_per_frame[f] = hk[f];
    return PCR_OK;
    PCR_API_END(c)
}

}

struct DevPoints {
    pcr_ctx *owner = nullptr;
    size_t n = 0, stride = 0;
    float *base = nullptr;
    bool has_normals = false;
    int arrays() const { return has_normals ? 6 : 3; }
    float *x() const { return base; }
    float *y() const { return base + stride; }
    float *z() const { return base + 2 * stride; }
    float *nx() const { return base + 3 * stride; }
    float *ny() const { return base + 4 * stride; }
    float *nz() const { return base + 5 * stride; }
};

struct pcr_cloud : DevPoints {
    pcr::CloudStats stats;
};

namespace pcr {
namespace {

struct HandleFree {
    void operator()(pcr_cloud *h) const { pcr_cloud_free(h); }
    void operator()(pcr_frames *h) const { pcr_frames_free(h); }
};
using CloudPtr = std::unique_ptr<pcr_cloud, HandleFree>;
using FramesPtr = std::unique_ptr<pcr_frames, HandleFree>;

template <class H>
int points_alloc(pcr_ctx *ctx, size_t n, bool normals, std::unique_ptr<H, HandleFree> &out, size_t tail = 0) {
    std::unique_ptr<H, HandleFree> h(new H());
    h->owner = ctx;
    h->n = n;
    h->stride = std::max<size_t>((n + 63) & ~(size_t)63, 64);
    h->has_normals = normals;
    float *base = nullptr;
    PCR_CUDA(&ctx->c, cudaMallocAsync((void **)&base, sizeof(float) * h->stride * h->arrays() + tail, ctx->c.stream));
    h->base = base;
    out = std::move(h);
    return PCR_OK;
}

template <class H>
void handle_free(H *h) {
    if (!h) return;
    if (h->base && h->owner) {
        DevSetter ds(&h->owner->c);
        cudaFreeAsync(h->base, h->owner->c.stream);
    }
    delete h;
}

__global__ void mask_to_u32_kernel(const uint8_t *__restrict__ keep, size_t n, uint32_t *__restrict__ flag) {
    PCR_GRID_DEP_SYNC();
    const size_t i = (size_t)blockIdx.x * blockDim.x + threadIdx.x;
    if (i <= n) flag[i] = (i < n && keep[i]) ? 1u : 0u;
}

__global__ void compact_kernel(const float *__restrict__ a, size_t a_stride, int n_a, const float *__restrict__ b, size_t b_stride, int n_b,
                               size_t n, const uint32_t *__restrict__ pos ,
                               float *__restrict__ dst, size_t dst_stride) {
    PCR_GRID_DEP_SYNC();
    const size_t i = (size_t)blockIdx.x * blockDim.x + threadIdx.x;
    if (i >= n) return;
    const uint32_t p = pos[i];
    if (pos[i + 1] == p) return;
    for (int r = 0; r < n_a; r++) dst[(size_t)r * dst_stride + p] = a[(size_t)r * a_stride + i];
    for (int r = 0; r < n_b; r++) dst[(size_t)(n_a + r) * dst_stride + p] = b[(size_t)r * b_stride + i];
}

__global__ void __launch_bounds__(256) rows_to_soa_kernel(const float *__restrict__ rows, size_t n, float *__restrict__ dst, size_t dst_stride) {
    __shared__ float sh[768];
    const size_t p0 = (size_t)blockIdx.x * 256;
    const size_t m = min((size_t)256, n - p0);
    for (size_t i = threadIdx.x; i < 3 * m; i += 256) sh[i] = rows[3 * p0 + i];
    __syncthreads();
    if (threadIdx.x < m)
        for (int r = 0; r < 3; r++) dst[(size_t)r * dst_stride + p0 + threadIdx.x] = sh[3 * threadIdx.x + r];
}
__global__ void __launch_bounds__(256) soa_to_rows_kernel(const float *__restrict__ src, size_t src_stride, size_t n, float *__restrict__ rows) {
    __shared__ float sh[768];
    const size_t p0 = (size_t)blockIdx.x * 256;
    const size_t m = min((size_t)256, n - p0);
    if (threadIdx.x < m)
        for (int r = 0; r < 3; r++) sh[3 * threadIdx.x + r] = src[(size_t)r * src_stride + p0 + threadIdx.x];
    __syncthreads();
    for (size_t i = threadIdx.x; i < 3 * m; i += 256) rows[3 * p0 + i] = sh[i];
}

__global__ void gather_kernel(const float *__restrict__ src, size_t src_stride, int n_arrays, const uint32_t *__restrict__ idx, size_t m,
                              float *__restrict__ dst, size_t dst_stride) {
    const size_t t = (size_t)blockIdx.x * blockDim.x + threadIdx.x;
    if (t >= m) return;
    const uint32_t i = idx[t];
    for (int a = 0; a < n_arrays; a++) dst[(size_t)a * dst_stride + t] = src[(size_t)a * src_stride + i];
}

int keep_scan(Ctx *c, const uint8_t *d_keep, size_t n, uint32_t **pos_out) {
    PCR_TRY(ensure(c, c->b_list, sizeof(uint32_t) * (n + 1)));
    uint32_t *pos = (uint32_t *)c->b_list.p;
    PCR_CUDA(c, launch_chained(mask_to_u32_kernel, dim3((unsigned)((n + 1 + 255) / 256)), dim3(256), 0, c->stream, d_keep, n, pos));
    c->launches++;
    PCR_TRY(exclusive_scan_u32_dev(c, pos, n + 1));
    *pos_out = pos;
    return PCR_OK;
}

int compact_into(const DevPoints *in, const uint32_t *pos, const float *nrm, size_t nrm_stride, const DevPoints *out) {
    if (!out->n) return PCR_OK;
    Ctx *c = &in->owner->c;
    const int n_a = nrm ? 3 : in->arrays(), n_b = nrm ? 3 : 0;
    c->launches++;
    PCR_CUDA(c, launch_chained(compact_kernel, dim3((unsigned)((in->n + 255) / 256)), dim3(256), 0, c->stream, in->base, in->stride, n_a, nrm,
                               nrm_stride, n_b, in->n, pos, out->base, out->stride));
    return PCR_OK;
}

int cloud_compact(const pcr_cloud *in, const uint8_t *d_keep, CloudPtr &out, const float *nrm = nullptr, size_t nrm_stride = 0,
                  size_t known_m = SIZE_MAX) {
    Ctx *c = &in->owner->c;
    uint32_t *pos = nullptr;
    PCR_TRY(keep_scan(c, d_keep, in->n, &pos));
    size_t m = known_m;
    if (m == SIZE_MAX) {
        uint32_t *mail = (uint32_t *)c->pinned + 96;
        PCR_CUDA(c, cudaMemcpyAsync(mail, pos + in->n, sizeof(uint32_t), cudaMemcpyDeviceToHost, c->stream));
        PCR_CUDA(c, cudaStreamSynchronize(c->stream));
        m = *mail;
    }
    PCR_TRY(points_alloc(in->owner, m, nrm || in->has_normals, out));
    return compact_into(in, pos, nrm, nrm_stride, out.get());
}

int copy_arrays(const DevPoints *src, size_t first, int arrays, const DevPoints *dst) {
    Ctx *c = &src->owner->c;
    for (int a = 0; dst->n && a < arrays; a++)
        PCR_CUDA(c, cudaMemcpyAsync(dst->base + (size_t)a * dst->stride, src->base + (size_t)a * src->stride + first, sizeof(float) * dst->n,
                                    cudaMemcpyDeviceToDevice, c->stream));
    return PCR_OK;
}

int upload_wait(Ctx *c, cudaError_t upload) {
    const cudaError_t sync = cudaStreamSynchronize(c->stream);
    PCR_CUDA(c, upload);
    PCR_CUDA(c, sync);
    return PCR_OK;
}

int points_upload(const DevPoints *p, const float *x, const float *y, const float *z) {
    Ctx *c = &p->owner->c;
    const float *src[3] = {x, y, z};
    cudaError_t upload = cudaSuccess;
    for (int a = 0; p->n && a < 3 && upload == cudaSuccess; a++)
        upload = cudaMemcpyAsync(p->base + (size_t)a * p->stride, src[a], sizeof(float) * p->n, cudaMemcpyHostToDevice, c->stream);
    return upload_wait(c, upload);
}

int points_upload_rows(const DevPoints *p, const float *xyz) {
    Ctx *c = &p->owner->c;
    const size_t n = p->n;
    cudaError_t upload = cudaSuccess;
    if (n) {
        PCR_TRY(ensure(c, c->b_in, sizeof(float) * 3 * n));
        upload = cudaMemcpyAsync(c->b_in.p, xyz, sizeof(float) * 3 * n, cudaMemcpyHostToDevice, c->stream);
        if (upload == cudaSuccess) {
            rows_to_soa_kernel<<<(unsigned)((n + 255) / 256), 256, 0, c->stream>>>((const float *)c->b_in.p, n, p->base, p->stride);
            c->launches++;
            upload = cudaGetLastError();
        }
    }
    return upload_wait(c, upload);
}

int points_download_rows(const DevPoints *p, float *xyz, float *normals) {
    Ctx *c = &p->owner->c;
    const size_t n = p->n, row = sizeof(float) * 3 * n;
    PCR_TRY(ensure(c, c->b_out, 2 * row));
    float *d_xyz = (float *)c->b_out.p, *d_nrm = d_xyz + 3 * n;
    const unsigned blocks = (unsigned)((n + 255) / 256);
    if (xyz) {
        soa_to_rows_kernel<<<blocks, 256, 0, c->stream>>>(p->base, p->stride, n, d_xyz);
        PCR_LAUNCH_CHECK(c);
        PCR_CUDA(c, cudaMemcpyAsync(xyz, d_xyz, row, cudaMemcpyDeviceToHost, c->stream));
    }
    if (normals) {
        soa_to_rows_kernel<<<blocks, 256, 0, c->stream>>>(p->nx(), p->stride, n, d_nrm);
        PCR_LAUNCH_CHECK(c);
        PCR_CUDA(c, cudaMemcpyAsync(normals, d_nrm, row, cudaMemcpyDeviceToHost, c->stream));
    }
    PCR_CUDA(c, cudaStreamSynchronize(c->stream));
    return PCR_OK;
}

int points_download(const DevPoints *p, float *x, float *y, float *z, float *nx, float *ny, float *nz) {
    Ctx *c = &p->owner->c;
    float *const dst[6] = {x, y, z, nx, ny, nz};
    for (int a = 0; a < 6; a++)
        if (dst[a]) PCR_CUDA(c, cudaMemcpyAsync(dst[a], p->base + (size_t)a * p->stride, sizeof(float) * p->n, cudaMemcpyDeviceToHost, c->stream));
    PCR_CUDA(c, cudaStreamSynchronize(c->stream));
    return PCR_OK;
}

void points_device_pointers(const DevPoints *p, const float **d_x, const float **d_y, const float **d_z, const float **d_nx, const float **d_ny,
                            const float **d_nz) {
    const float **const dst[6] = {d_x, d_y, d_z, d_nx, d_ny, d_nz};
    for (int a = 0; a < 6; a++)
        if (dst[a]) *dst[a] = a < p->arrays() ? p->base + (size_t)a * p->stride : nullptr;
}

int handle_check(const DevPoints *h, const char *what) {
    if (h && h->owner) return PCR_OK;
    return fail(nullptr, PCR_ERR_INVALID_ARG, "%s is NULL", what);
}

}
}


extern "C" {

int pcr_cloud_upload(pcr_ctx *ctx, const float *x, const float *y, const float *z, size_t n, pcr_cloud **out) {
    if (!ctx) return fail(nullptr, PCR_ERR_INVALID_ARG, "ctx is NULL");
    Ctx *c = &ctx->c;
    if (!out || (n && (!x || !y || !z))) return fail(c, PCR_ERR_INVALID_ARG, "null pointer");
    *out = nullptr;
    PCR_API_BEGIN
    DevSetter ds(c);
    CloudPtr res;
    PCR_TRY(points_alloc(ctx, n, false, res));
    PCR_TRY(points_upload(res.get(), x, y, z));
    *out = res.release();
    return PCR_OK;
    PCR_API_END(c)
}

void pcr_cloud_free(pcr_cloud *cloud) { handle_free(cloud); }

size_t pcr_cloud_len(const pcr_cloud *cloud) { return cloud ? cloud->n : 0; }
int pcr_cloud_has_normals(const pcr_cloud *cloud) { return cloud && cloud->has_normals ? 1 : 0; }

int pcr_cloud_device_pointers(const pcr_cloud *cloud, const float **d_x, const float **d_y, const float **d_z, const float **d_nx,
                              const float **d_ny, const float **d_nz) {
    PCR_TRY(handle_check(cloud, "cloud"));
    points_device_pointers(cloud, d_x, d_y, d_z, d_nx, d_ny, d_nz);
    return PCR_OK;
}

int pcr_cloud_download(const pcr_cloud *cloud, float *x, float *y, float *z) {
    PCR_TRY(handle_check(cloud, "cloud"));
    Ctx *c = &cloud->owner->c;
    if (cloud->n && (!x || !y || !z)) return fail(c, PCR_ERR_INVALID_ARG, "null pointer");
    if (!cloud->n) return PCR_OK;
    PCR_API_BEGIN
    DevSetter ds(c);
    return points_download(cloud, x, y, z, nullptr, nullptr, nullptr);
    PCR_API_END(c)
}

int pcr_cloud_download_normals(const pcr_cloud *cloud, float *nx, float *ny, float *nz) {
    PCR_TRY(handle_check(cloud, "cloud"));
    Ctx *c = &cloud->owner->c;
    if (!cloud->has_normals) return fail(c, PCR_ERR_INVALID_ARG, "the cloud has no normals");
    if (cloud->n && (!nx || !ny || !nz)) return fail(c, PCR_ERR_INVALID_ARG, "null pointer");
    if (!cloud->n) return PCR_OK;
    PCR_API_BEGIN
    DevSetter ds(c);
    return points_download(cloud, nullptr, nullptr, nullptr, nx, ny, nz);
    PCR_API_END(c)
}

int pcr_cloud_upload_rows(pcr_ctx *ctx, const float *xyz, size_t n, pcr_cloud **out) {
    if (!ctx) return fail(nullptr, PCR_ERR_INVALID_ARG, "ctx is NULL");
    Ctx *c = &ctx->c;
    if (!out || (n && !xyz)) return fail(c, PCR_ERR_INVALID_ARG, "null pointer");
    *out = nullptr;
    PCR_API_BEGIN
    DevSetter ds(c);
    CloudPtr res;
    PCR_TRY(points_alloc(ctx, n, false, res));
    PCR_TRY(points_upload_rows(res.get(), xyz));
    *out = res.release();
    return PCR_OK;
    PCR_API_END(c)
}

int pcr_cloud_download_rows(const pcr_cloud *cloud, float *xyz, float *normals) {
    PCR_TRY(handle_check(cloud, "cloud"));
    Ctx *c = &cloud->owner->c;
    if (normals && !cloud->has_normals) return fail(c, PCR_ERR_INVALID_ARG, "the cloud has no normals");
    if (cloud->n && !xyz && !normals) return fail(c, PCR_ERR_INVALID_ARG, "null pointer");
    if (!cloud->n) return PCR_OK;
    PCR_API_BEGIN
    DevSetter ds(c);
    return points_download_rows(cloud, xyz, normals);
    PCR_API_END(c)
}

int pcr_sor_normals_batch_rows(pcr_ctx *ctx, const float *xyz, const uint64_t *frame_offsets, size_t n_frames, size_t k_sor, float std_mul,
                               size_t k_normals, const float viewpoint[3], uint8_t *keep, float *normals, uint64_t *n_kept_per_frame) {
    if (!ctx) return fail(nullptr, PCR_ERR_INVALID_ARG, "ctx is NULL");
    Ctx *c = &ctx->c;
    if (n_frames == 0) return PCR_OK;
    PCR_TRY(offsets_check(c, "frame_offsets", frame_offsets, n_frames));
    const size_t n = (size_t)frame_offsets[n_frames];
    if (n_kept_per_frame) memset(n_kept_per_frame, 0, sizeof(uint64_t) * n_frames);
    if (n == 0) return PCR_OK;
    if (!xyz || !keep || !viewpoint || (k_normals && !normals)) return fail(c, PCR_ERR_INVALID_ARG, "null pointer");
    PCR_TRY(sor_normals_batch_check(c, n, n_frames, k_sor, std_mul, k_normals));
    PCR_API_BEGIN
    DevSetter ds(c);
    const size_t stride = (n + 63) & ~(size_t)63;
    const unsigned blocks = (unsigned)((n + 255) / 256);
    PCR_TRY(ensure(c, c->b_in, sizeof(float) * (3 * stride + 3 * n)));
    float *dx = (float *)c->b_in.p, *d_rows = dx + 3 * stride;
    PCR_CUDA(c, cudaMemcpyAsync(d_rows, xyz, sizeof(float) * 3 * n, cudaMemcpyHostToDevice, c->stream));
    rows_to_soa_kernel<<<blocks, 256, 0, c->stream>>>(d_rows, n, dx, stride);
    PCR_LAUNCH_CHECK(c);
    const size_t o_keep = stride * 3 * sizeof(float);
    const size_t o_kept = o_keep + ((n + 255) & ~(size_t)255);
    const size_t o_rows = (o_kept + sizeof(unsigned long long) * n_frames + 255) & ~(size_t)255;
    PCR_TRY(ensure(c, c->b_out, o_rows + sizeof(float) * 3 * n));
    float *dnx = (float *)c->b_out.p, *dny = dnx + stride, *dnz = dny + stride;
    uint8_t *d_keep = (uint8_t *)c->b_out.p + o_keep;
    unsigned long long *d_kept = (unsigned long long *)((char *)c->b_out.p + o_kept);
    float *d_nrows = (float *)((char *)c->b_out.p + o_rows);
    PCR_TRY(batch_core(c, dx, dx + stride, dx + 2 * stride, frame_offsets, n_frames, n, k_sor, std_mul, k_normals, viewpoint, d_keep, dnx, dny, dnz,
                       d_kept));
    PCR_CUDA(c, cudaMemcpyAsync(keep, d_keep, n, cudaMemcpyDeviceToHost, c->stream));
    if (k_normals) {
        soa_to_rows_kernel<<<blocks, 256, 0, c->stream>>>(dnx, stride, n, d_nrows);
        PCR_LAUNCH_CHECK(c);
        PCR_CUDA(c, cudaMemcpyAsync(normals, d_nrows, sizeof(float) * 3 * n, cudaMemcpyDeviceToHost, c->stream));
    }
    std::vector<unsigned long long> hk(n_frames);
    PCR_CUDA(c, cudaMemcpyAsync(hk.data(), d_kept, sizeof(unsigned long long) * n_frames, cudaMemcpyDeviceToHost, c->stream));
    PCR_CUDA(c, cudaStreamSynchronize(c->stream));
    if (n_kept_per_frame)
        for (size_t f = 0; f < n_frames; f++) n_kept_per_frame[f] = hk[f];
    return PCR_OK;
    PCR_API_END(c)
}

static int upload_block(pcr_ctx *ctx, const float *xyz, size_t stride, size_t n, pcr_cloud **out, bool wait);
int pcr_cloud_upload_block(pcr_ctx *ctx, const float *xyz, size_t stride, size_t n, pcr_cloud **out) {
    return upload_block(ctx, xyz, stride, n, out, true);
}
int pcr_cloud_upload_block_nowait(pcr_ctx *ctx, const float *xyz, size_t stride, size_t n, pcr_cloud **out) {
    return upload_block(ctx, xyz, stride, n, out, false);
}
static int upload_block(pcr_ctx *ctx, const float *xyz, size_t stride, size_t n, pcr_cloud **out, bool wait) {
    if (!ctx) return fail(nullptr, PCR_ERR_INVALID_ARG, "ctx is NULL");
    Ctx *c = &ctx->c;
    if (!out || (n && !xyz) || stride < n) return fail(c, PCR_ERR_INVALID_ARG, "null pointer or stride < n");
    *out = nullptr;
    PCR_API_BEGIN
    DevSetter ds(c);
    CloudPtr res;
    PCR_TRY(points_alloc(ctx, n, false, res));
    cudaError_t e = cudaSuccess;
    if (n) e = cudaMemcpy2DAsync(res->base, res->stride * sizeof(float), xyz, stride * sizeof(float), n * sizeof(float), 3, cudaMemcpyHostToDevice, c->stream);
    if (e == cudaSuccess && wait) e = cudaStreamSynchronize(c->stream);
    if (e != cudaSuccess) {
        cudaGetLastError();
        return fail(c, PCR_ERR_CUDA, "upload failed: %s", cudaGetErrorString(e));
    }
    *out = res.release();
    return PCR_OK;
    PCR_API_END(c)
}

int pcr_cloud_download_block(const pcr_cloud *cloud, float *dst, size_t stride, int with_normals) {
    PCR_TRY(handle_check(cloud, "cloud"));
    Ctx *c = &cloud->owner->c;
    if (with_normals && !cloud->has_normals) return fail(c, PCR_ERR_INVALID_ARG, "the cloud has no normals");
    if ((cloud->n && !dst) || stride < cloud->n) return fail(c, PCR_ERR_INVALID_ARG, "null pointer or stride < len");
    if (!cloud->n) return PCR_OK;
    PCR_API_BEGIN
    DevSetter ds(c);
    PCR_CUDA(c, cudaMemcpy2DAsync(dst, stride * sizeof(float), cloud->base, cloud->stride * sizeof(float), cloud->n * sizeof(float),
                                  with_normals ? 6 : 3, cudaMemcpyDeviceToHost, c->stream));
    PCR_CUDA(c, cudaStreamSynchronize(c->stream));
    return PCR_OK;
    PCR_API_END(c)
}

int pcr_cloud_select(const pcr_cloud *cloud, const uint32_t *indices, size_t m, pcr_cloud **out) {
    PCR_TRY(handle_check(cloud, "cloud"));
    Ctx *c = &cloud->owner->c;
    if (!out || (m && !indices)) return fail(c, PCR_ERR_INVALID_ARG, "null pointer");
    *out = nullptr;
    for (size_t t = 0; t < m; t++)
        if (indices[t] >= cloud->n) return fail(c, PCR_ERR_INVALID_ARG, "index %u out of bounds for cloud with %zu points", indices[t], cloud->n);
    PCR_API_BEGIN
    DevSetter ds(c);
    CloudPtr res;
    PCR_TRY(points_alloc(cloud->owner, m, cloud->has_normals, res));
    if (m) {
        PCR_TRY(ensure(c, c->b_list, sizeof(uint32_t) * m));
        PCR_CUDA(c, cudaMemcpyAsync(c->b_list.p, indices, sizeof(uint32_t) * m, cudaMemcpyHostToDevice, c->stream));
        gather_kernel<<<(unsigned)((m + 255) / 256), 256, 0, c->stream>>>(cloud->base, cloud->stride, cloud->arrays(), (const uint32_t *)c->b_list.p,
                                                                          m, res->base, res->stride);
        PCR_LAUNCH_CHECK(c);
        PCR_CUDA(c, cudaStreamSynchronize(c->stream));
    }
    *out = res.release();
    return PCR_OK;
    PCR_API_END(c)
}

int pcr_cloud_voxel_downsample(const pcr_cloud *cloud, float voxel_size, pcr_cloud **out) {
    PCR_TRY(handle_check(cloud, "cloud"));
    Ctx *c = &cloud->owner->c;
    if (!out) return fail(c, PCR_ERR_INVALID_ARG, "null pointer");
    *out = nullptr;
    if (!std::isfinite(voxel_size) || !(voxel_size > 0.f)) return fail(c, PCR_ERR_INVALID_ARG, "voxel_size must be > 0 and finite");
    PCR_API_BEGIN
    DevSetter ds(c);
    PCR_MARK("voxel: enter");
    CloudPtr res;
    PCR_TRY(points_alloc(cloud->owner, cloud->n, false, res));
    size_t m = 0;
    PCR_TRY(voxel_downsample_dev(c, cloud->x(), cloud->y(), cloud->z(), cloud->n, voxel_size, res->x(), res->y(), res->z(), &m, &res->stats));
    res->n = m;
    *out = res.release();
    PCR_MARK("voxel: exit");
    return PCR_OK;
    PCR_API_END(c)
}

int pcr_cloud_statistical_outlier_removal(const pcr_cloud *cloud, size_t k, float std_mul, pcr_cloud **out) {
    PCR_TRY(handle_check(cloud, "cloud"));
    Ctx *c = &cloud->owner->c;
    if (!out) return fail(c, PCR_ERR_INVALID_ARG, "null pointer");
    *out = nullptr;
    PCR_API_BEGIN
    DevSetter ds(c);
    const size_t n = cloud->n;
    CloudPtr res;
    if (n == 0 || k == 0) {
        PCR_TRY(points_alloc(cloud->owner, 0, false, res));
    } else {
        PCR_TRY(ensure(c, c->b_in2, n + 256));
        uint8_t *d_keep = (uint8_t *)c->b_in2.p;
        PCR_TRY(pcr_sor_dev(cloud->owner, cloud->x(), cloud->y(), cloud->z(), n, k, std_mul, d_keep, nullptr));
        PCR_TRY(cloud_compact(cloud, d_keep, res));
    }
    *out = res.release();
    return PCR_OK;
    PCR_API_END(c)
}

int pcr_cloud_radius_outlier_removal(const pcr_cloud *cloud, float radius, size_t min_neighbors, pcr_cloud **out) {
    PCR_TRY(handle_check(cloud, "cloud"));
    Ctx *c = &cloud->owner->c;
    if (!out) return fail(c, PCR_ERR_INVALID_ARG, "null pointer");
    *out = nullptr;
    PCR_API_BEGIN
    DevSetter ds(c);
    const size_t n = cloud->n;
    CloudPtr res;
    if (n == 0) {
        PCR_TRY(points_alloc(cloud->owner, 0, cloud->has_normals, res));
    } else {
        PCR_TRY(ensure(c, c->b_in2, n + 256));
        uint8_t *d_keep = (uint8_t *)c->b_in2.p;
        PCR_TRY(pcr_radius_outlier_dev(cloud->owner, cloud->x(), cloud->y(), cloud->z(), n, radius, min_neighbors, d_keep));
        PCR_TRY(cloud_compact(cloud, d_keep, res));
    }
    *out = res.release();
    return PCR_OK;
    PCR_API_END(c)
}

int pcr_cloud_estimate_normals(const pcr_cloud *cloud, size_t k, const float viewpoint[3], pcr_cloud **out) {
    PCR_TRY(handle_check(cloud, "cloud"));
    Ctx *c = &cloud->owner->c;
    if (!out) return fail(c, PCR_ERR_INVALID_ARG, "null pointer");
    *out = nullptr;
    if (k == 0) return fail(c, PCR_ERR_INVALID_ARG, "k must be > 0");
    PCR_API_BEGIN
    DevSetter ds(c);
    CloudPtr res;
    PCR_TRY(points_alloc(cloud->owner, cloud->n, true, res));
    PCR_TRY(copy_arrays(cloud, 0, 3, res.get()));
    const float vp0[3] = {0.f, 0.f, 0.f};
    PCR_TRY(pcr_estimate_normals_dev(cloud->owner, cloud->x(), cloud->y(), cloud->z(), cloud->n, k, viewpoint ? viewpoint : vp0, res->nx(),
                                     res->ny(), res->nz()));
    *out = res.release();
    return PCR_OK;
    PCR_API_END(c)
}

int pcr_cloud_sor_normals(const pcr_cloud *cloud, size_t k_sor, float std_mul, size_t k_normals, const float viewpoint[3],
                          pcr_cloud **out) {
    PCR_TRY(handle_check(cloud, "cloud"));
    Ctx *c = &cloud->owner->c;
    if (!out) return fail(c, PCR_ERR_INVALID_ARG, "null pointer");
    *out = nullptr;
    if (k_normals == 0) return fail(c, PCR_ERR_INVALID_ARG, "k_normals must be > 0");
    if (!std::isfinite(std_mul) || std_mul < 0.f) return fail(c, PCR_ERR_INVALID_ARG, "std_mul must be >= 0 and finite");
    if (k_sor + 1 > PCR_MAX_K || k_normals > PCR_MAX_K) return fail(c, PCR_ERR_UNSUPPORTED, "k exceeds PCR_MAX_K");
    PCR_API_BEGIN
    DevSetter ds(c);
    const size_t n = cloud->n;
    CloudPtr res;
    if (n == 0 || k_sor == 0) {
        PCR_TRY(points_alloc(cloud->owner, 0, true, res));
        *out = res.release();
        return PCR_OK;
    }
    PCR_MARK("sor_normals: enter");
    const size_t stride = (n + 63) & ~(size_t)63;
    StreamAlloc<float> nrm_mem(c->stream);
    PCR_CUDA(c, nrm_mem.alloc(sizeof(float) * 3 * stride));
    float *d_nrm = nrm_mem.p;
    PCR_TRY(ensure(c, c->b_in2, n + 512));
    uint8_t *d_keep = (uint8_t *)c->b_in2.p;
    unsigned long long *d_kept = (unsigned long long *)((char *)c->b_in2.p + ((n + 255) & ~(size_t)255));
    const uint64_t offs[2] = {0, n};
    const float vp0[3] = {0.f, 0.f, 0.f};
    unsigned long long h_kept = ~0ull;
    PCR_TRY(batch_core(c, cloud->x(), cloud->y(), cloud->z(), offs, 1, n, k_sor, std_mul, k_normals, viewpoint ? viewpoint : vp0, d_keep,
                       d_nrm, d_nrm + stride, d_nrm + 2 * stride, d_kept, &h_kept, cloud->stats.valid ? &cloud->stats : nullptr));
    PCR_MARK("sor_normals: core done");
    PCR_TRY(cloud_compact(cloud, d_keep, res, d_nrm, stride, h_kept == ~0ull ? SIZE_MAX : (size_t)h_kept));
    PCR_MARK("sor_normals: exit");
    *out = res.release();
    return PCR_OK;
    PCR_API_END(c)
}

int pcr_cloud_euclidean_cluster(const pcr_cloud *cloud, float distance_threshold, size_t min_size, size_t max_size, uint32_t *offsets,
                                uint32_t *indices, size_t *n_clusters) {
    PCR_TRY(handle_check(cloud, "cloud"));
    Ctx *c = &cloud->owner->c;
    if (n_clusters) *n_clusters = 0;
    if (!offsets || !n_clusters) return fail(c, PCR_ERR_INVALID_ARG, "null pointer");
    offsets[0] = 0;
    const size_t n = cloud->n;
    if (n && !indices) return fail(c, PCR_ERR_INVALID_ARG, "null pointer");
    if (n == 0 || distance_threshold <= 0.0f || min_size == 0) return PCR_OK;
    PCR_API_BEGIN
    DevSetter ds(c);
    PCR_TRY(ensure(c, c->b_out, n * sizeof(uint32_t)));
    uint32_t *d_labels = (uint32_t *)c->b_out.p;
    PCR_TRY(cluster_labels_dev(c, cloud->x(), cloud->y(), cloud->z(), n, distance_threshold, d_labels));
    std::vector<uint32_t> labels(n), scratch;
    PCR_CUDA(c, cudaMemcpyAsync(labels.data(), d_labels, n * sizeof(uint32_t), cudaMemcpyDeviceToHost, c->stream));
    PCR_CUDA(c, cudaStreamSynchronize(c->stream));
    *n_clusters = clusters_from_labels(labels.data(), n, min_size, max_size, offsets, indices, scratch);
    return PCR_OK;
    PCR_API_END(c)
}

static int ransac_common(Ctx *c, const float *dx, const float *dy, const float *dz, size_t n, float thr, const uint32_t *samples, size_t m,
                         float model[4], uint32_t *inliers, size_t *n_inliers) {
    PCR_TRY(ensure(c, c->b_out, sizeof(uint32_t) * std::max<size_t>(n, 1)));
    uint32_t *d_inl = (uint32_t *)c->b_out.p;
    size_t k = 0;
    PCR_TRY(ransac_plane_samples_dev(c, dx, dy, dz, n, thr, samples, m, model, d_inl, &k));
    if (k) {
        PCR_CUDA(c, cudaMemcpyAsync(inliers, d_inl, sizeof(uint32_t) * k, cudaMemcpyDeviceToHost, c->stream));
        PCR_CUDA(c, cudaStreamSynchronize(c->stream));
    }
    *n_inliers = k;
    return PCR_OK;
}

int pcr_ransac_plane_samples(pcr_ctx *ctx, const float *x, const float *y, const float *z, size_t n, float distance_threshold,
                             const uint32_t *samples, size_t m, float model[4], uint32_t *inliers, size_t *n_inliers) {
    if (!ctx) return fail(nullptr, PCR_ERR_INVALID_ARG, "ctx is NULL");
    Ctx *c = &ctx->c;
    if (!model || !n_inliers || (m && !samples) || (n && (!x || !y || !z || !inliers))) return fail(c, PCR_ERR_INVALID_ARG, "null pointer");
    PCR_API_BEGIN
    DevSetter ds(c);
    float *dx = nullptr, *dy = nullptr, *dz = nullptr;
    if (n >= 3) PCR_TRY(stage_xyz(c, c->b_in, x, y, z, n, &dx, &dy, &dz));
    return ransac_common(c, dx, dy, dz, n, distance_threshold, samples, m, model, inliers, n_inliers);
    PCR_API_END(c)
}

int pcr_cloud_ransac_plane_samples(const pcr_cloud *cloud, float distance_threshold, const uint32_t *samples, size_t m, float model[4],
                                   uint32_t *inliers, size_t *n_inliers) {
    PCR_TRY(handle_check(cloud, "cloud"));
    Ctx *c = &cloud->owner->c;
    if (!model || !n_inliers || (m && !samples) || (cloud->n && !inliers)) return fail(c, PCR_ERR_INVALID_ARG, "null pointer");
    PCR_API_BEGIN
    DevSetter ds(c);
    return ransac_common(c, cloud->x(), cloud->y(), cloud->z(), cloud->n, distance_threshold, samples, m, model, inliers, n_inliers);
    PCR_API_END(c)
}

int pcr_cloud_apply_transform(const pcr_cloud *cloud, const float rotation[9], const float translation[3], pcr_cloud **out) {
    PCR_TRY(handle_check(cloud, "cloud"));
    Ctx *c = &cloud->owner->c;
    if (!out || !rotation || !translation) return fail(c, PCR_ERR_INVALID_ARG, "null pointer");
    *out = nullptr;
    PCR_API_BEGIN
    DevSetter ds(c);
    CloudPtr res;
    PCR_TRY(points_alloc(cloud->owner, cloud->n, false, res));
    if (cloud->n) PCR_TRY(apply_transform_dev(c, cloud->x(), cloud->y(), cloud->z(), cloud->n, rotation, translation, res->x(), res->y(), res->z()));
    *out = res.release();
    return PCR_OK;
    PCR_API_END(c)
}

int pcr_cloud_icp_point_to_point(const pcr_cloud *source, const pcr_cloud *target, const pcr_icp_params *params, pcr_icp_result *result) {
    PCR_TRY(handle_check(source, "cloud"));
    Ctx *c = &source->owner->c;
    if (!target || target->owner != source->owner) return fail(c, PCR_ERR_INVALID_ARG, "source and target must live on the same context");
    return pcr_icp_point_to_point_dev(source->owner, source->x(), source->y(), source->z(), source->n, target->x(), target->y(), target->z(),
                                      target->n, params, result);
}

int pcr_cloud_icp_point_to_plane(const pcr_cloud *source, const pcr_cloud *target, const pcr_icp_params *params, pcr_icp_result *result) {
    PCR_TRY(handle_check(source, "cloud"));
    Ctx *c = &source->owner->c;
    if (!target || target->owner != source->owner) return fail(c, PCR_ERR_INVALID_ARG, "source and target must live on the same context");
    if (!target->has_normals)
        return fail(c, PCR_ERR_INVALID_ARG, "target cloud must have normals (call estimate_normals first)");
    return pcr_icp_point_to_plane_dev(source->owner, source->x(), source->y(), source->z(), source->n, target->x(), target->y(), target->z(),
                                      target->n, target->nx(), target->ny(), target->nz(), target->n, params, result);
}

}

struct pcr_frames : DevPoints {
    uint32_t *d_off = nullptr;
    std::vector<uint64_t> off;
    size_t count() const { return off.size() - 1; }
};

namespace pcr {
namespace {

int offsets_upload(Ctx *c, const std::vector<uint64_t> &off, uint32_t *d_off) {
    const std::vector<uint32_t> h(off.begin(), off.end());
    PCR_CUDA(c, cudaMemcpyAsync(d_off, h.data(), sizeof(uint32_t) * h.size(), cudaMemcpyHostToDevice, c->stream));
    return PCR_OK;
}

int frames_alloc(pcr_ctx *ctx, size_t n, bool normals, std::vector<uint64_t> off, FramesPtr &out, const uint32_t *d_off_src = nullptr) {
    Ctx *c = &ctx->c;
    FramesPtr fr;
    PCR_TRY(points_alloc(ctx, n, normals, fr, sizeof(uint32_t) * off.size()));
    fr->off = std::move(off);
    fr->d_off = (uint32_t *)(fr->base + fr->stride * fr->arrays());
    if (d_off_src)
        PCR_CUDA(c, cudaMemcpyAsync(fr->d_off, d_off_src, sizeof(uint32_t) * fr->off.size(), cudaMemcpyDeviceToDevice, c->stream));
    else
        PCR_TRY(offsets_upload(c, fr->off, fr->d_off));
    out = std::move(fr);
    return PCR_OK;
}

__global__ void frame_starts_kernel(const uint32_t *__restrict__ pos, const uint32_t *__restrict__ frame_off, int n_frames,
                                    uint32_t *__restrict__ new_off) {
    const int f = blockIdx.x * blockDim.x + threadIdx.x;
    if (f <= n_frames) new_off[f] = pos[frame_off[f]];
}

int frames_compact(const pcr_frames *in, const uint8_t *d_keep, FramesPtr &out, const float *nrm = nullptr, size_t nrm_stride = 0) {
    Ctx *c = &in->owner->c;
    const size_t F = in->count();
    uint32_t *pos = nullptr;
    PCR_TRY(keep_scan(c, d_keep, in->n, &pos));
    StreamAlloc<uint32_t> new_off(c->stream);
    PCR_CUDA(c, new_off.alloc(sizeof(uint32_t) * (F + 1)));
    uint32_t *d_new = new_off.p;
    frame_starts_kernel<<<(unsigned)((F + 1 + 255) / 256), 256, 0, c->stream>>>(pos, in->d_off, (int)F, d_new);
    PCR_LAUNCH_CHECK(c);
    PCR_TRY(ensure_pinned(c, sizeof(uint32_t) * (F + 1)));
    uint32_t *mail = (uint32_t *)c->pinned;
    PCR_CUDA(c, cudaMemcpyAsync(mail, d_new, sizeof(uint32_t) * (F + 1), cudaMemcpyDeviceToHost, c->stream));
    PCR_CUDA(c, cudaStreamSynchronize(c->stream));
    std::vector<uint64_t> off(F + 1);
    for (size_t f = 0; f <= F; f++) off[f] = mail[f];
    const size_t m = (size_t)off[F];
    PCR_TRY(frames_alloc(in->owner, m, nrm || in->has_normals, std::move(off), out, d_new));
    return compact_into(in, pos, nrm, nrm_stride, out.get());
}

int frames_empty(const pcr_frames *in, bool normals, FramesPtr &out) {
    return frames_alloc(in->owner, 0, normals, std::vector<uint64_t>(in->count() + 1, 0), out);
}

__device__ __forceinline__ uint32_t list_point(const uint32_t *__restrict__ idx, const uint32_t *__restrict__ list_off,
                                               const uint32_t *__restrict__ frame_off, int n_frames, uint32_t t) {
    return frame_off[frame_of(list_off, n_frames, t)] + idx[t];
}

__global__ void frames_gather_kernel(const float *__restrict__ src, size_t src_stride, int n_arrays, const uint32_t *__restrict__ idx,
                                     const uint32_t *__restrict__ list_off, const uint32_t *__restrict__ frame_off, int n_frames, size_t m,
                                     float *__restrict__ dst, size_t dst_stride) {
    const size_t t = (size_t)blockIdx.x * blockDim.x + threadIdx.x;
    if (t >= m) return;
    const uint32_t i = list_point(idx, list_off, frame_off, n_frames, (uint32_t)t);
    for (int a = 0; a < n_arrays; a++) dst[(size_t)a * dst_stride + t] = src[(size_t)a * src_stride + i];
}

__global__ void frames_unkeep_kernel(const uint32_t *__restrict__ idx, const uint32_t *__restrict__ list_off,
                                     const uint32_t *__restrict__ frame_off, int n_frames, size_t m, uint8_t *__restrict__ keep) {
    const size_t t = (size_t)blockIdx.x * blockDim.x + threadIdx.x;
    if (t < m) keep[list_point(idx, list_off, frame_off, n_frames, (uint32_t)t)] = 0;
}

int frames_select_inverse_dev(const pcr_frames *in, const uint32_t *d_idx, const std::vector<uint64_t> &list_off, FramesPtr &out) {
    Ctx *c = &in->owner->c;
    const size_t n = in->n, F = in->count(), m = (size_t)list_off[F];
    const size_t o_loff = (n + 3) & ~(size_t)3;
    StreamAlloc<uint8_t> keep_mem(c->stream);
    PCR_CUDA(c, keep_mem.alloc(o_loff + sizeof(uint32_t) * (F + 1)));
    uint8_t *d_keep = keep_mem.p;
    uint32_t *d_loff = (uint32_t *)(d_keep + o_loff);
    if (n) PCR_CUDA(c, cudaMemsetAsync(d_keep, 1, n, c->stream));
    if (m) {
        PCR_TRY(offsets_upload(c, list_off, d_loff));
        frames_unkeep_kernel<<<(unsigned)((m + 255) / 256), 256, 0, c->stream>>>(d_idx, d_loff, in->d_off, (int)F, m, d_keep);
        PCR_LAUNCH_CHECK(c);
    }
    return frames_compact(in, d_keep, out);
}

}
}

extern "C" {

static int frames_upload_check(Ctx *c, const uint64_t *frame_offsets, size_t n_frames, pcr_frames **out, size_t *n) {
    if (!out) return fail(c, PCR_ERR_INVALID_ARG, "null pointer");
    *out = nullptr;
    if (n_frames == 0) return fail(c, PCR_ERR_INVALID_ARG, "a batch holds at least one frame");
    PCR_TRY(offsets_check(c, "frame_offsets", frame_offsets, n_frames));
    *n = (size_t)frame_offsets[n_frames];
    return batch_size_check(c, *n, n_frames);
}

int pcr_frames_upload(pcr_ctx *ctx, const float *x, const float *y, const float *z, const uint64_t *frame_offsets, size_t n_frames,
                      pcr_frames **out) {
    if (!ctx) return fail(nullptr, PCR_ERR_INVALID_ARG, "ctx is NULL");
    Ctx *c = &ctx->c;
    size_t n = 0;
    PCR_TRY(frames_upload_check(c, frame_offsets, n_frames, out, &n));
    if (n && (!x || !y || !z)) return fail(c, PCR_ERR_INVALID_ARG, "null pointer");
    PCR_API_BEGIN
    DevSetter ds(c);
    FramesPtr res;
    PCR_TRY(frames_alloc(ctx, n, false, std::vector<uint64_t>(frame_offsets, frame_offsets + n_frames + 1), res));
    PCR_TRY(points_upload(res.get(), x, y, z));
    *out = res.release();
    return PCR_OK;
    PCR_API_END(c)
}

int pcr_frames_upload_rows(pcr_ctx *ctx, const float *xyz, const uint64_t *frame_offsets, size_t n_frames, pcr_frames **out) {
    if (!ctx) return fail(nullptr, PCR_ERR_INVALID_ARG, "ctx is NULL");
    Ctx *c = &ctx->c;
    size_t n = 0;
    PCR_TRY(frames_upload_check(c, frame_offsets, n_frames, out, &n));
    if (n && !xyz) return fail(c, PCR_ERR_INVALID_ARG, "null pointer");
    PCR_API_BEGIN
    DevSetter ds(c);
    FramesPtr res;
    PCR_TRY(frames_alloc(ctx, n, false, std::vector<uint64_t>(frame_offsets, frame_offsets + n_frames + 1), res));
    PCR_TRY(points_upload_rows(res.get(), xyz));
    *out = res.release();
    return PCR_OK;
    PCR_API_END(c)
}

void pcr_frames_free(pcr_frames *frames) { handle_free(frames); }
// ... 305 lines not shown
```

pointclouds_rs_b200/csrc/pcr_internal.cuh:

```cuda
#pragma once
#include <cstdlib>

#include <cuda_runtime.h>
#include <math.h>
#include <stdint.h>
#include <stdio.h>
#include <string.h>

#include <memory>
#include <string>
#include <vector>

#include "../../include/pcr_b200.h"

namespace pcr {

struct GridDesc {
    double o[3];
    double h, inv_h;
    int32_t dims[3];
    int32_t ax[3];
    uint32_t cell_base;
    uint32_t n_cells;
    uint32_t pt_begin;
    uint32_t pt_end;
    uint32_t in_begin;
    uint32_t in_end;
};

constexpr int kLevelFactor = 6;

struct DevBuf {
    void *p = nullptr;
    size_t cap = 0;
};

struct Ctx;

constexpr int kPeerMaxWorld = 8;
constexpr int kPeerWords = 32;
constexpr size_t kPeerDataBytes = 2 * kPeerMaxWorld * kPeerWords * sizeof(double);
constexpr size_t kPeerBlockBytes = kPeerDataBytes + 2 * kPeerMaxWorld * sizeof(unsigned long long);
struct PeerComm {
    double *data[kPeerMaxWorld];
    unsigned long long *flag[kPeerMaxWorld];
    int rank, world;
};

struct Index {
    Ctx *ctx = nullptr;
    size_t n = 0;
    size_t n_indexed = 0;
    int n_frames = 1;
    std::vector<GridDesc> grids_h;
    GridDesc *grids = nullptr;
    uint32_t *frame_in_off = nullptr;
    float4 *sorted = nullptr;
    float4 *orig4 = nullptr;
    uint32_t *cell_start = nullptr;
    uint32_t total_cells = 0;
    bool owns_memory = true;
    std::vector<double> box_min, box_ext;
    std::vector<uint32_t> box_count;
    const uint8_t *d_mask = nullptr;
    Index *coarser = nullptr;
    Index *finer = nullptr;
    bool shares_orig4 = false;
    int cell_slot = -1;
    bool level_bufs_borrowed = false;
    uint32_t q_begin = 0;
    uint32_t q_count = 0xffffffffu;
};

struct Ctx {
    int device = 0;
    cudaStream_t stream = nullptr;
    bool owns_stream = false;
    int sm_count = 148;
    std::string err;
    uint64_t err_seq = 0;
    uint64_t launches = 0;
    float forced_cell = 0.f;
    bool frame_stream = false;
    struct {
        bool valid = false;
        size_t k_hint = 0;
        uint32_t count = 0;
        double ext[3] = {0, 0, 0};
        double h = 0;
    } cell_cache;
    struct {
        bool valid = false;
        float voxel = 0.f;
        int mn[3] = {0, 0, 0}, mx[3] = {0, 0, 0};
        int uses = 0;
        int pad_shift = 6;
    } vox_cache;
    DevBuf b_in;
    DevBuf b_in2;
    DevBuf b_out;
    DevBuf b_misc;
    DevBuf b_fine_misc, b_fine_scan;
    uint32_t fine_scan_epoch = 0;
    DevBuf b_misc2;
    DevBuf b_small;
    DevBuf b_table;
    struct Piggy {
        void *dst;
        const void *src;
        size_t bytes;
    };
    std::vector<Piggy> piggy;
    bool spec_coarser = false;
    bool spec_request = false;
    bool spec_pending = false;
    bool spec_zero = false;
    uint64_t stat_nowait_hits = 0, stat_nowait_misses = 0;
    cudaEvent_t ev_count = nullptr;
    cudaStream_t side[2] = {nullptr, nullptr};
    cudaEvent_t ev_fork = nullptr, ev_join[2] = {nullptr, nullptr};
    DevBuf b_scan;
    uint32_t scan_epoch = 0;
    DevBuf b_list;
    DevBuf b_qoff;
    DevBuf b_cells[6];
    DevBuf b_lsorted[6], b_lgrids[6];
    void *pinned = nullptr;
    size_t pinned_cap = 0;
    bool timing = false;
    struct TimedSpan {
        cudaEvent_t a, b;
        int tag;
    };
    std::vector<TimedSpan> spans;
    unsigned long long *d_knn_stats = nullptr;
    std::vector<cudaEvent_t> event_pool;
    void *nccl_comm = nullptr;
    int rank = 0, world = 1;
    PeerComm peer = {};
    void *peer_block = nullptr;
    void *peer_open[kPeerMaxWorld] = {};
    bool peer_ok = false;
    unsigned long long peer_seq = 0;
    bool shard_queries = false;
    bool fake_comm = false;
    uint64_t stat_cell_hits = 0, stat_cell_misses = 0, stat_vox_hits = 0, stat_vox_misses = 0, stat_spec_hits = 0, stat_spec_misses = 0;
};

int fail(Ctx *ctx, int code, const char *fmt, ...);
void set_thread_error(const char *msg);

#define PCR_CUDA(ctx, expr)                                                                       \
    do {                                                                                          \
        cudaError_t _e = (expr);                                                                  \
        if (_e != cudaSuccess) {                                                                  \
            cudaGetLastError();                                                                   \
            return pcr::fail((ctx), _e == cudaErrorMemoryAllocation ? PCR_ERR_OOM : PCR_ERR_CUDA, \
                             "%s failed: %s (%s:%d)", #expr, cudaGetErrorString(_e), __FILE__,    \
                             __LINE__);                                                           \
        }                                                                                         \
    } while (0)

#define PCR_TRY(expr)              \
    do {                           \
        int _s = (expr);           \
        if (_s != PCR_OK) return _s; \
    } while (0)

#define PCR_LAUNCH_CHECK(ctx)                                                                   \
    do {                                                                                        \
        (ctx)->launches++;                                                                      \
        cudaError_t _e = cudaGetLastError();                                                    \
        if (_e != cudaSuccess)                                                                  \
            return pcr::fail((ctx), PCR_ERR_CUDA, "kernel launch failed: %s (%s:%d)",           \
                             cudaGetErrorString(_e), __FILE__, __LINE__);                       \
    } while (0)

enum TimeTag { kTagBuild = 0, kTagKnn = 1, kTagKnnDeferred = 2, kTagSorStats = 3, kTagIcpStep = 4, kTagIcpSolve = 5, kTagKnnNormals = 6, kTagOther = 7, kNumTags = 8 };

extern bool g_trace_on;
void trace_mark(const char *label);
#define PCR_MARK(label)                            \
    do {                                           \
        if (pcr::g_trace_on) pcr::trace_mark(label); \
    } while (0)

struct TimeScope {
    Ctx *c;
    int idx = -1;
    TimeScope(Ctx *ctx, int tag);
    ~TimeScope();
};

int ensure(Ctx *ctx, DevBuf &b, size_t bytes);
int ensure_pinned(Ctx *ctx, size_t bytes);

template <class T = void>
struct StreamAlloc {
    T *p = nullptr;
    cudaStream_t s;
    explicit StreamAlloc(cudaStream_t stream) : s(stream) {}
    StreamAlloc(const StreamAlloc &) = delete;
    StreamAlloc &operator=(const StreamAlloc &) = delete;
    ~StreamAlloc() {
        if (p) cudaFreeAsync(p, s);
    }
    cudaError_t alloc(size_t bytes) {
        const cudaError_t e = cudaMallocAsync((void **)&p, bytes, s);
        if (e != cudaSuccess) p = nullptr;
        return e;
    }
};

struct CloudStats {
    unsigned mn[3], mx[3];
    unsigned count;
    unsigned valid;
};

struct BuildOpts {
    const CloudStats *known_stats = nullptr;
    size_t k_hint = 0;
    bool self_knn = false;
    int n_frames = 1;
    const uint64_t *frame_offsets = nullptr;
    const uint8_t *d_mask = nullptr;
    bool transient = false;
};
int index_build_dev(Ctx *ctx, const float *dx, const float *dy, const float *dz, size_t n,
                    const BuildOpts &opts, Index **out);
void index_free(Index *ix);
struct IndexFree {
    void operator()(Index *ix) const { index_free(ix); }
};
using IndexPtr = std::unique_ptr<Index, IndexFree>;
int index_coarser_level(Index *ix, Index **out);
int index_finer_level(Index *ix, Index **out);

struct QueryFrames {
    const uint64_t *offsets;
    size_t n_frames;
};
int knn_queries_dev(Index *ix, const float *dqx, const float *dqy, const float *dqz, size_t nq,
                    size_t k, uint32_t *d_idx, float *d_dist, uint32_t *d_counts, const QueryFrames *qf = nullptr);
struct SorLists {
    size_t K = 0;
    size_t stride = 0;
    uint32_t *lists = nullptr;
    uint8_t *cnt = nullptr;
    uint32_t *fallback = nullptr;
    bool initialised = false;
};
int sor_mean_dist_dev(Index *ix, size_t k, float *d_mean_d, const SorLists *keep_lists = nullptr, bool allow_shard = false);
int normals_from_lists_dev(Index *ix, size_t k, const float vp[3], const SorLists &sl, const uint8_t *d_keep, float *d_nx, float *d_ny,
                           float *d_nz,
                           const unsigned long long *d_kept0 = nullptr, unsigned long long *h_kept0 = nullptr, bool early = false);
int normals_early_fork(Ctx *ctx);
int normals_early_from_lists_dev(Index *ix, size_t k, const float vp[3], const SorLists &sl, float *d_nx, float *d_ny, float *d_nz, bool *launched);
int normals_dev(Index *ix, size_t k, const float vp[3], float *d_nx, float *d_ny, float *d_nz,
                const uint8_t *d_mask, bool allow_shard = false);
bool query_sharding_active(const Ctx *ctx, const Index *ix);
int index_shard_queries(Index *ix);
int index_apply_mask_dev(Index *ix, const uint8_t *d_keep);
int radius_count_dev(Index *ix, const float *dqx, const float *dqy, const float *dqz, size_t nq,
                     float radius, uint32_t *d_counts, const QueryFrames *qf = nullptr);
int radius_fill_dev(Index *ix, const float *dqx, const float *dqy, const float *dqz, size_t nq,
                    float radius, const uint64_t *d_offsets, uint32_t *d_idx, const QueryFrames *qf = nullptr);

int sor_threshold_mask_dev(Ctx *ctx, const float *d_mean_d, const uint32_t *d_frame_off ,
                           int n_frames, size_t n, float std_mul, uint8_t *d_keep, float *d_stats,
                           unsigned long long *d_kept, bool kept_zeroed = false );

int exclusive_scan_u32_dev(Ctx *ctx, uint32_t *d_data, size_t n_plus_1);
int exclusive_scan_u64_from_u32_dev(Ctx *ctx, const uint32_t *d_in, uint64_t *d_out, size_t n);

struct IcpArgs {
    const float *d_sx, *d_sy, *d_sz;
    size_t ns;
    const float *d_tx, *d_ty, *d_tz;
    size_t nt;
    const float *d_nx, *d_ny, *d_nz;
    pcr_icp_params params;
};
int icp_dev(Ctx *ctx, const IcpArgs &a, pcr_icp_result *result);
struct IcpBatchArgs {
    const float *d_x, *d_y, *d_z;
    size_t n;
    const uint64_t *frame_offsets;
    size_t n_frames;
    const float *d_nx, *d_ny, *d_nz;
    const uint32_t *pairs;
    size_t n_pairs;
    pcr_icp_params params;
};
int icp_batch_dev(Ctx *ctx, const IcpBatchArgs &a, pcr_icp_result *results);
int find_correspondences_dev(Index *target, const float *dsx, const float *dsy, const float *dsz,
                             size_t ns, float max_distance, uint32_t *d_tgt, float *d_dist, const QueryFrames *qf = nullptr);
int apply_transform_dev(Ctx *ctx, const float *dx, const float *dy, const float *dz, size_t n,
                        const float R[9], const float t[3], float *ox, float *oy, float *oz);
int apply_transform_batch_dev(Ctx *ctx, const float *dx, const float *dy, const float *dz, const uint64_t *frame_offsets, size_t n_frames,
                              const uint32_t *d_frame_off, const float *transforms, float *ox, float *oy, float *oz);

int cluster_labels_dev(Ctx *ctx, const float *dx, const float *dy, const float *dz, size_t n, float threshold, uint32_t *d_labels,
                       const uint32_t *d_frame_off = nullptr, int n_frames = 1);
size_t clusters_from_labels(const uint32_t *labels, size_t n, size_t min_size, size_t max_size, uint32_t *offsets, uint32_t *indices,
                            std::vector<uint32_t> &scratch);
int cluster_labels_batch_dev(Ctx *ctx, const float *dx, const float *dy, const float *dz, const uint64_t *frame_offsets, size_t n_frames,
                             float threshold, uint32_t *d_labels);
int euclidean_cluster_batch_dev(Ctx *ctx, const float *dx, const float *dy, const float *dz, const uint64_t *frame_offsets, size_t n_frames,
                                float threshold, size_t min_size, size_t max_size, uint32_t *d_offsets, uint32_t *d_indices,
                                uint64_t *cluster_offsets, size_t *total);

int voxel_downsample_dev(Ctx *ctx, const float *dx, const float *dy, const float *dz, size_t n, float voxel, float *d_ox, float *d_oy,
                         float *d_oz, size_t *n_out, CloudStats *stats_out = nullptr ,
                         bool allow_guess = true );
int voxel_downsample_batch_dev(Ctx *ctx, const float *dx, const float *dy, const float *dz, const uint64_t *frame_offsets,
                               size_t n_frames, float voxel, float *d_ox, float *d_oy, float *d_oz, uint64_t *out_offsets);
int radix_sort_pairs_dev(Ctx *ctx, unsigned long long **keys, uint32_t **vals, unsigned long long **keys_alt, uint32_t **vals_alt,
                         size_t n, int bits, uint32_t *d_hist);
size_t radix_sort_hist_words(size_t n);
int bits_for(uint64_t range);

int ransac_plane_samples_dev(Ctx *ctx, const float *dx, const float *dy, const float *dz, size_t n, float threshold,
                             const uint32_t *h_samples, size_t m, float model_out[4], uint32_t *d_inliers, size_t *n_inliers);
int ransac_plane_samples_batch_dev(Ctx *ctx, const float *dx, const float *dy, const float *dz, const uint64_t *frame_offsets,
                                   size_t n_frames, float threshold, const uint32_t *h_samples, const uint64_t *sample_offsets,
                                   float *models_out, uint32_t *d_inliers, uint64_t *inlier_offsets);

int comm_unique_id(void *out);
int comm_init(Ctx *ctx, const void *id, int rank, int world);
void comm_destroy(Ctx *ctx);
int comm_allreduce_f64(Ctx *ctx, double *d_buf, size_t count);
int comm_allgather_bytes(Ctx *ctx, const void *d_send, void *d_recv, size_t bytes);
int comm_allreduce_u32(Ctx *ctx, uint32_t *d_buf, size_t count);

}

struct pcr_ctx {
    pcr::Ctx c;
};
struct pcr_index {
    pcr::Index *ix;
    pcr_ctx *owner;
};

namespace pcr {

#ifdef __CUDACC__

#define PCR_GRID_DEP_SYNC() cudaGridDependencySynchronize()

template <class... KArgs, class... Args>
inline cudaError_t launch_chained(void (*kernel)(KArgs...), dim3 grid, dim3 block, size_t smem, cudaStream_t st, Args &&...args) {
    static const bool off = getenv("PCR_NO_PDL") != nullptr;
    cudaLaunchConfig_t cfg = {};
    cfg.gridDim = grid;
    cfg.blockDim = block;
    cfg.dynamicSmemBytes = smem;
    cfg.stream = st;
    cudaLaunchAttribute at[1];
    at[0].id = cudaLaunchAttributeProgrammaticStreamSerialization;
    at[0].val.programmaticStreamSerializationAllowed = 1;
    cfg.attrs = at;
    cfg.numAttrs = off ? 0 : 1;
    return cudaLaunchKernelEx(&cfg, kernel, static_cast<KArgs>(args)...);
}

#define PCR_FULL 0xffffffffu
#define PCR_EMPTY_KEY 0x7f80000100000000ull

__device__ __forceinline__ float dist2_exact(float ax, float ay, float az, float bx, float by, float bz) {
    float dx = __fsub_rn(ax, bx), dy = __fsub_rn(ay, by), dz = __fsub_rn(az, bz);
    float s = __fmul_rn(dx, dx);
    s = __fadd_rn(s, __fmul_rn(dy, dy));
    s = __fadd_rn(s, __fmul_rn(dz, dz));
    return s;
}

__device__ __forceinline__ unsigned long long make_key(float d2, uint32_t idx) {
    return ((unsigned long long)__float_as_uint(d2) << 32) | idx;
}
__device__ __forceinline__ float key_d2(unsigned long long k) { return __uint_as_float((uint32_t)(k >> 32)); }
__device__ __forceinline__ uint32_t key_idx(unsigned long long k) { return (uint32_t)k; }

__device__ __forceinline__ bool finite3(float a, float b, float c) { return isfinite(a) && isfinite(b) && isfinite(c); }
__device__ __forceinline__ unsigned f32_ordered(float f) {
    unsigned u = __float_as_uint(f);
    return (u & 0x80000000u) ? ~u : (u | 0x80000000u);
}

__device__ __forceinline__ float pick_axis(int ax, float x, float y, float z) { return ax == 0 ? x : (ax == 1 ? y : z); }

__device__ __forceinline__ int cell_coord(const GridDesc &g, int j, float v, double *frac) {
    double t = ((double)v - g.o[j]) * g.inv_h;
    double f = floor(t);
    f = fmin(fmax(f, 0.0), (double)(g.dims[j] - 1));
    if (frac) *frac = t - f;
    return (int)f;
}

__device__ __forceinline__ uint32_t cell_linear(const GridDesc &g, int c0, int c1, int c2) {
    return g.cell_base + ((uint32_t)c0 * (uint32_t)g.dims[1] + (uint32_t)c1) * (uint32_t)g.dims[2] + (uint32_t)c2;
}

__device__ __forceinline__ int frame_of(const uint32_t *__restrict__ off, int n_frames, uint32_t i) {
    if (n_frames <= 1) return 0;
    int lo = 0, hi = n_frames - 1;
    while (lo < hi) {
        int mid = (lo + hi + 1) >> 1;
        if (off[mid] <= i) lo = mid;
        else hi = mid - 1;
    }
    return lo;
}

#endif

}
```

pointclouds_rs_b200/csrc/voxel.cu:

```cuda
#include "pcr_internal.cuh"

#include <algorithm>

namespace pcr {

namespace {

constexpr int kSortRounds = 8;
constexpr int kSortTile = 32 * kSortRounds;
constexpr int kSortWarps = 4;

struct VoxHeader {
    unsigned mn_c[3], mx[3];
    unsigned count;
    unsigned outside;
    unsigned total;
    unsigned tall;
    unsigned pad[6];
};
constexpr uint32_t kTallColumn = 256;
constexpr uint32_t kLocalColumn = 32;
static_assert(sizeof(VoxHeader) == 64, "header layout");

struct VoxRange {
// ... 323 lines not shown
                if (ch >= end) break;
                if (ch + 1 < end && a[ch] < a[ch + 1]) ch++;
                if (a[root] >= a[ch]) break;
                const unsigned long long t = a[root]; a[root] = a[ch]; a[ch] = t;
                root = ch;
            }
        }
    }
    uint32_t nv = 1;
    for (uint32_t i = 1; i < m; i++) nv += (uint32_t)(a[i] >> 32) != (uint32_t)(a[i - 1] >> 32) ? 1u : 0u;
    nvox[b] = nv;
}

__global__ void __launch_bounds__(256) vox_col_emit_kernel(const float *__restrict__ x, const float *__restrict__ y,
                                                           const float *__restrict__ z, const uint32_t *__restrict__ col_of,
                                                           const uint32_t *__restrict__ rank_of, size_t n,
                                                           const uint32_t *__restrict__ start, const uint32_t *__restrict__ vstart,
                                                           const unsigned long long *__restrict__ members, float *__restrict__ ox,
                                                           float *__restrict__ oy, float *__restrict__ oz) {
    PCR_GRID_DEP_SYNC();
    const size_t t = (size_t)blockIdx.x * blockDim.x + threadIdx.x;
    if (t >= n) return;
    const uint32_t c = col_of[t];
    if (c == 0xffffffffu || rank_of[t] != 0u) return;
    const uint32_t b = start[c], e = start[c + 1];
    if (e - b > kTallColumn) return;
    uint32_t v = vstart[b];
    uint32_t cur = (uint32_t)(members[b] >> 32);
    float sx = 0.f, sy = 0.f, sz = 0.f;
    uint32_t cnt = 0;
    for (uint32_t i = b; i < e; i += 8) {
        unsigned long long mm[8];
#pragma unroll
        for (int u = 0; u < 8; u++) mm[u] = members[min(i + u, e - 1)];
        float X[8], Y[8], Z[8];
#pragma unroll
        for (int u = 0; u < 8; u++) {
            const uint32_t p = (uint32_t)mm[u];
            X[u] = x[p];
            Y[u] = y[p];
            Z[u] = z[p];
        }
#pragma unroll
        for (int u = 0; u < 8; u++) {
            if (i + u >= e) break;
            const uint32_t kz = (uint32_t)(mm[u] >> 32);
            if (kz != cur) {
                const float denom = (float)cnt;
                ox[v] = __fdiv_rn(sx, denom);
                oy[v] = __fdiv_rn(sy, denom);
                oz[v] = __fdiv_rn(sz, denom);
                v++;
                sx = sy = sz = 0.f;
                cnt = 0;
                cur = kz;
            }
            sx = __fadd_rn(sx, X[u]);
            sy = __fadd_rn(sy, Y[u]);
            sz = __fadd_rn(sz, Z[u]);
            cnt++;
        }
    }
    const float denom = (float)cnt;
    ox[v] = __fdiv_rn(sx, denom);
    oy[v] = __fdiv_rn(sy, denom);
    oz[v] = __fdiv_rn(sz, denom);
}

__global__ void __launch_bounds__(256) vox_out_stats_kernel(const float *__restrict__ x, const float *__restrict__ y,
                                                            const float *__restrict__ z, const uint32_t *__restrict__ d_n,
                                                            VoxHeader *hdr) {
    PCR_GRID_DEP_SYNC();
    const uint32_t n = *d_n;
    if (blockIdx.x == 0 && threadIdx.x == 0) hdr->total = n;
    unsigned mn_c[3] = {0u, 0u, 0u}, mx[3] = {0u, 0u, 0u}, cnt = 0;
    for (uint32_t i = blockIdx.x * blockDim.x + threadIdx.x; i < n; i += gridDim.x * blockDim.x) {
        const float px = x[i], py = y[i], pz = z[i];
        if (!finite3(px, py, pz)) continue;
        const unsigned u[3] = {f32_ordered(px), f32_ordered(py), f32_ordered(pz)};
        for (int a = 0; a < 3; a++) {
            mn_c[a] = max(mn_c[a], ~u[a]);
            mx[a] = max(mx[a], u[a]);
        }
        cnt++;
    }
    for (int a = 0; a < 3; a++) {
        mn_c[a] = __reduce_max_sync(PCR_FULL, mn_c[a]);
        mx[a] = __reduce_max_sync(PCR_FULL, mx[a]);
    }
    cnt = __reduce_add_sync(PCR_FULL, cnt);
    __shared__ unsigned s_mn[3], s_mx[3], s_cnt;
    if (threadIdx.x == 0) {
        s_mn[0] = s_mn[1] = s_mn[2] = 0u;
        s_mx[0] = s_mx[1] = s_mx[2] = 0u;
        s_cnt = 0;
    }
    __syncthreads();
    if ((threadIdx.x & 31) == 0 && cnt) {
        for (int a = 0; a < 3; a++) {
            atomicMax(&s_mn[a], mn_c[a]);
            atomicMax(&s_mx[a], mx[a]);
        }
        atomicAdd(&s_cnt, cnt);
    }
    __syncthreads();
    if (threadIdx.x == 0 && s_cnt) {
        for (int a = 0; a < 3; a++) {
            atomicMax(&hdr->mn_c[a], s_mn[a]);
            atomicMax(&hdr->mx[a], s_mx[a]);
        }
        atomicAdd(&hdr->count, s_cnt);
    }
}

__global__ void __launch_bounds__(256) vox_frame_starts_kernel(const unsigned long long *__restrict__ keys, const uint32_t *__restrict__ vals,
                                                               uint32_t m, int fshift ,
                                                               const uint32_t *__restrict__ frame_off, int n_frames,
                                                               const uint32_t *__restrict__ vid, uint32_t *__restrict__ out_off) {
    const uint32_t i = blockIdx.x * blockDim.x + threadIdx.x;
    if (i > m) return;
    auto frame = [&](uint32_t j) { return fshift >= 0 ? (int)(keys[j] >> fshift) : frame_of(frame_off, n_frames, vals[j]); };
    const int hi = i < m ? frame(i) : n_frames;
    const int lo = i > 0 ? frame(i - 1) : -1;
    for (int f = lo + 1; f <= hi; f++) out_off[f] = vid[i];
}

}

int bits_for(uint64_t range) {
    int b = 0;
    while (b < 64 && (1ull << b) < range) b++;
    return b;
}

size_t radix_sort_hist_words(size_t n) { return (size_t)256 * ((n + kSortTile - 1) / kSortTile) + 1; }

int radix_sort_pairs_dev(Ctx *ctx, unsigned long long **keys, uint32_t **vals, unsigned long long **keys_alt, uint32_t **vals_alt,
                         size_t n, int bits, uint32_t *d_hist ) {
    if (n == 0) return PCR_OK;
    const uint32_t n_tiles = (uint32_t)((n + kSortTile - 1) / kSortTile);
    const unsigned blocks = (n_tiles + kSortWarps - 1) / kSortWarps;
    for (int shift = 0; shift < bits; shift += 8) {
        sort_hist_kernel<<<blocks, 32 * kSortWarps, 0, ctx->stream>>>(*keys, n, shift, n_tiles, d_hist);
        PCR_LAUNCH_CHECK(ctx);
        PCR_TRY(exclusive_scan_u32_dev(ctx, d_hist, (size_t)256 * n_tiles + 1));
        sort_scatter_kernel<<<blocks, 32 * kSortWarps, 0, ctx->stream>>>(*keys, *vals, n, shift, n_tiles, d_hist, *keys_alt, *vals_alt);
        PCR_LAUNCH_CHECK(ctx);
        std::swap(*keys, *keys_alt);
        std::swap(*vals, *vals_alt);
    }
    return PCR_OK;
}

int voxel_downsample_dev(Ctx *ctx, const float *dx, const float *dy, const float *dz, size_t n, float voxel, float *d_ox, float *d_oy,
                         float *d_oz, size_t *n_out, CloudStats *stats_out, bool allow_guess) {
    *n_out = 0;
    if (stats_out) stats_out->valid = 0;
    if (n == 0) return PCR_OK;
    if (n > 0x7fffffffull) return fail(ctx, PCR_ERR_UNSUPPORTED, "clouds above 2^31 points are not supported");
    cudaStream_t st = ctx->stream;
    TimeScope ts(ctx, kTagOther);
    PCR_TRY(ensure(ctx, ctx->b_small, 4096));
    PCR_TRY(ensure_pinned(ctx, 4096));
    VoxRange *d_range = (VoxRange *)ctx->b_small.p;
    uint32_t *d_nvox = (uint32_t *)((char *)ctx->b_small.p + 256);
    VoxRange *h_range = (VoxRange *)ctx->pinned;
    auto &vc = ctx->vox_cache;
    static const bool no_guess = getenv("PCR_NO_VOXEL_GUESS") != nullptr;
    const bool guessed = allow_guess && !no_guess && ctx->frame_stream && vc.valid && vc.voxel == voxel && vc.uses < 32;
    uint32_t m;
    if (guessed) {
        vc.uses++;
        for (int a = 0; a < 3; a++) {
            h_range->mn[a] = vc.mn[a];
            h_range->mx[a] = vc.mx[a];
        }
        m = (uint32_t)n;
    } else {
        vox_init_kernel<<<1, 1, 0, st>>>(d_range, 1);
        PCR_LAUNCH_CHECK(ctx);
        const unsigned bx = (unsigned)std::min<size_t>((n + 255) / 256, (size_t)ctx->sm_count * 2);
        vox_range_kernel<<<bx, 256, 0, st>>>(dx, dy, dz, nullptr, n, voxel, d_range);
        PCR_LAUNCH_CHECK(ctx);
        PCR_CUDA(ctx, cudaMemcpyAsync(h_range, d_range, sizeof(VoxRange), cudaMemcpyDeviceToHost, st));
        PCR_MARK("voxel: wait for range");
        PCR_CUDA(ctx, cudaStreamSynchronize(st));
        PCR_MARK("voxel: got range");
        m = h_range->finite;
        if (m == 0) return PCR_OK;
        vc.valid = false;
        if (ctx->frame_stream) {
            bool ok = true;
            for (int a = 0; a < 3; a++) {
                const long long ext = (long long)h_range->mx[a] - (long long)h_range->mn[a] + 1;
                const long long pad = std::max<long long>(2, ext >> vc.pad_shift);
                const long long lo = (long long)h_range->mn[a] - pad, hi = (long long)h_range->mx[a] + pad;
                if (lo < -2147483647ll || hi > 2147483646ll) ok = false;
                vc.mn[a] = (int)lo;
                vc.mx[a] = (int)hi;
            }
            vc.valid = ok;
            vc.voxel = voxel;
            vc.uses = 0;
        }
    }
    {
        const uint64_t nx = (uint64_t)((int64_t)h_range->mx[0] - (int64_t)h_range->mn[0]) + 1;
        const uint64_t ny = (uint64_t)((int64_t)h_range->mx[1] - (int64_t)h_range->mn[1]) + 1;
        const uint64_t nz = (uint64_t)((int64_t)h_range->mx[2] - (int64_t)h_range->mn[2]) + 1;
        int ys = 0;
        static const int ys_max = getenv("PCR_VOXEL_YS") ? atoi(getenv("PCR_VOXEL_YS")) : 0;
        while (ys < ys_max && nz < (1ull << (32 - (ys + 1))) && nx * ((ny + (2ull << ys) - 1) >> (ys + 1)) >= (uint64_t)m) ys++;
        while (ys < 4 && nz < (1ull << (32 - (ys + 1))) && nx * ((ny + (1ull << ys) - 1) >> ys) > (1ull << 24)) ys++;
        const uint64_t nyc64 = (ny + (1ull << ys) - 1) >> ys;
        const uint64_t n_cols64 = nx * nyc64;
        static const bool no_cols = getenv("PCR_VOXEL_RADIX") != nullptr;
        if (!no_cols && nx < (1ull << 31) && ny < (1ull << 31) && nz < (1ull << (32 - ys)) && n_cols64 <= (1ull << 24) &&
            n_cols64 <= 64ull * m + 65536ull) {
            const uint32_t n_cols = (uint32_t)n_cols64;
            const size_t tab = (sizeof(uint32_t) * ((size_t)n_cols + 1) + 15) & ~(size_t)15;
            const size_t tab_v = (sizeof(uint32_t) * ((size_t)n + 1) + 15) & ~(size_t)15;
            const size_t o_count = sizeof(VoxHeader), o_nvox = o_count + tab;
            const size_t o_col = (o_nvox + tab_v + 15) & ~(size_t)15;
            const size_t o_rank = o_col + sizeof(uint32_t) * n;
            const size_t o_mem = (o_rank + sizeof(uint32_t) * n + 15) & ~(size_t)15;
            PCR_TRY(ensure(ctx, ctx->b_table, o_mem + sizeof(unsigned long long) * n));
            char *base = (char *)ctx->b_table.p;
            VoxHeader *d_hdr = (VoxHeader *)base;
            uint32_t *count = (uint32_t *)(base + o_count), *nvox = (uint32_t *)(base + o_nvox);
            uint32_t *col_of = (uint32_t *)(base + o_col), *rank_of = (uint32_t *)(base + o_rank);
            unsigned long long *members = (unsigned long long *)(base + o_mem);
            PCR_CUDA(ctx, cudaMemsetAsync(base, 0, o_nvox + tab_v, st));
            const unsigned nbp = (unsigned)((n + 255) / 256);
            vox_col_count_kernel<<<nbp, 256, 0, st>>>(dx, dy, dz, n, voxel, h_range->mn[0], h_range->mn[1], h_range->mn[2], nx, ny, nz,
                                                      (uint32_t)nyc64, ys, count, col_of, rank_of, &d_hdr->outside);
            PCR_LAUNCH_CHECK(ctx);
            PCR_TRY(exclusive_scan_u32_dev(ctx, count, (size_t)n_cols + 1));
            PCR_CUDA(ctx, launch_chained(vox_col_scatter_kernel, dim3(nbp), dim3(256), 0, st, dy, dz, n, voxel, h_range->mn[1], h_range->mn[2], ys,
                                         count, col_of, rank_of, members));
            PCR_CUDA(ctx, launch_chained(vox_col_sort_kernel, dim3(nbp), dim3(256), 0, st, col_of, rank_of, n, count, members, nvox, &d_hdr->tall));
            ctx->launches += 2;
            PCR_TRY(exclusive_scan_u32_dev(ctx, nvox, n + 1));
            PCR_CUDA(ctx, launch_chained(vox_col_emit_kernel, dim3(nbp), dim3(256), 0, st, dx, dy, dz, col_of, rank_of, n, count, nvox, members, d_ox,
                                         d_oy, d_oz));
            ctx->launches++;
            PCR_CUDA(ctx, launch_chained(vox_out_stats_kernel, dim3((unsigned)ctx->sm_count), dim3(256), 0, st, d_ox, d_oy, d_oz, nvox + n, d_hdr));
            ctx->launches++;
            VoxHeader *mail = (VoxHeader *)((uint32_t *)ctx->pinned + 64);
            PCR_CUDA(ctx, cudaMemcpyAsync(mail, d_hdr, sizeof(VoxHeader), cudaMemcpyDeviceToHost, st));
            PCR_MARK("voxel: wait for count");
            PCR_CUDA(ctx, cudaStreamSynchronize(st));
            PCR_MARK("voxel: got count");
            if (guessed) (mail->outside ? ctx->stat_vox_misses : ctx->stat_vox_hits)++;
            if (guessed && mail->outside) {
                vc.valid = false;
                vc.pad_shift = std::max(2, vc.pad_shift - 1);
                return voxel_downsample_dev(ctx, dx, dy, dz, n, voxel, d_ox, d_oy, d_oz, n_out, stats_out, false);
            }
            const bool tall = mail->tall != 0;
            if (tall && guessed) {
                vc.valid = false;
                return voxel_downsample_dev(ctx, dx, dy, dz, n, voxel, d_ox, d_oy, d_oz, n_out, stats_out, false);
            }
            if (!tall) *n_out = mail->total;
            if (!tall && stats_out) {
                for (int a = 0; a < 3; a++) {
                    stats_out->mn[a] = ~mail->mn_c[a];
                    stats_out->mx[a] = mail->mx[a];
                }
                stats_out->count = mail->count;
                stats_out->valid = 1;
            }
            if (!tall) return PCR_OK;
        }
    }
    if (guessed) {
        vc.valid = false;
        return voxel_downsample_dev(ctx, dx, dy, dz, n, voxel, d_ox, d_oy, d_oz, n_out, stats_out, false);
    }
    int bits[3];
    for (int a = 0; a < 3; a++) bits[a] = bits_for((uint64_t)((int64_t)h_range->mx[a] - (int64_t)h_range->mn[a]) + 1);
    const int total_bits = bits[0] + bits[1] + bits[2];
    const bool packed = total_bits <= 63;

    const size_t n_tiles = (n + kSortTile - 1) / kSortTile;
    const size_t need = 2 * sizeof(unsigned long long) * n + sizeof(uint32_t) * (2 * n + 256 * n_tiles + 1 + 2 * (n + 1)) + 1024;
    PCR_TRY(ensure(ctx, ctx->b_table, need));
    char *p = (char *)ctx->b_table.p;
    unsigned long long *kA = (unsigned long long *)p;
    p += sizeof(unsigned long long) * n;
    unsigned long long *kB = (unsigned long long *)p;
    p += sizeof(unsigned long long) * n;
    uint32_t *vA = (uint32_t *)p;
    p += sizeof(uint32_t) * n;
    uint32_t *vB = (uint32_t *)p;
    p += sizeof(uint32_t) * n;
    uint32_t *hist = (uint32_t *)p;
    p += sizeof(uint32_t) * (256 * n_tiles + 1);
    uint32_t *vid = (uint32_t *)p;
    p += sizeof(uint32_t) * (n + 1);
    uint32_t *start = (uint32_t *)p;
    const unsigned nb = (unsigned)((n + 255) / 256);
    if (packed) {
        const unsigned long long last = 1ull << total_bits;
        vox_pack_kernel<<<nb, 256, 0, st>>>(dx, dy, dz, nullptr, n, voxel, -1, h_range->mn[0], h_range->mn[1], h_range->mn[2],
                                            bits[1] + bits[2], bits[2], last, kA, vA, nullptr, 1, nullptr, 0);
        PCR_LAUNCH_CHECK(ctx);
        PCR_TRY(radix_sort_pairs_dev(ctx, &kA, &vA, &kB, &vB, n, total_bits + 1, hist));
        vox_heads_kernel<<<(m + 1 + 255) / 256, 256, 0, st>>>(kA, m, vid);
        PCR_LAUNCH_CHECK(ctx);
    } else {
        const unsigned long long last = 1ull << 32;
        for (int axis = 2; axis >= 0; axis--) {
            vox_pack_kernel<<<nb, 256, 0, st>>>(dx, dy, dz, axis == 2 ? nullptr : vA, n, voxel, axis, 0, 0, 0, 0, 0, last, kA, vA, nullptr, 1,
                                                nullptr, 0);
            PCR_LAUNCH_CHECK(ctx);
            PCR_TRY(radix_sort_pairs_dev(ctx, &kA, &vA, &kB, &vB, n, 33, hist));
        }
        vox_heads_triple_kernel<<<(m + 1 + 255) / 256, 256, 0, st>>>(dx, dy, dz, vA, m, voxel, nullptr, 1, vid);
        PCR_LAUNCH_CHECK(ctx);
    }
    PCR_TRY(exclusive_scan_u32_dev(ctx, vid, (size_t)m + 1));
    vox_starts_kernel<<<(m + 1 + 255) / 256, 256, 0, st>>>(vid, m, start);
    PCR_LAUNCH_CHECK(ctx);
    PCR_CUDA(ctx, cudaMemcpyAsync(d_nvox, vid + m, sizeof(uint32_t), cudaMemcpyDeviceToDevice, st));
    vox_mean_kernel<<<(m + 127) / 128, 128, 0, st>>>(dx, dy, dz, vA, start, d_nvox, d_ox, d_oy, d_oz);
    PCR_LAUNCH_CHECK(ctx);
    uint32_t *mail = (uint32_t *)ctx->pinned + 64;
    PCR_CUDA(ctx, cudaMemcpyAsync(mail, d_nvox, sizeof(uint32_t), cudaMemcpyDeviceToHost, st));
    PCR_CUDA(ctx, cudaStreamSynchronize(st));
    *n_out = *mail;
    return PCR_OK;
}

int voxel_downsample_batch_dev(Ctx *ctx, const float *dx, const float *dy, const float *dz, const uint64_t *frame_offsets,
                               size_t n_frames, float voxel, float *d_ox, float *d_oy, float *d_oz, uint64_t *out_offsets) {
    const int F = (int)n_frames;
    for (int f = 0; f <= F; f++) out_offsets[f] = 0;
    const size_t n = F ? (size_t)frame_offsets[F] : 0;
    if (n == 0) return PCR_OK;
    cudaStream_t st = ctx->stream;
    TimeScope ts(ctx, kTagOther);
    const size_t n_tiles = (n + kSortTile - 1) / kSortTile;
    const size_t need = 2 * sizeof(unsigned long long) * n + sizeof(uint32_t) * (2 * n + 256 * n_tiles + 1 + 2 * (n + 1)) +
                        sizeof(uint32_t) * 2 * (F + 1) + sizeof(VoxRange) * F + 1024;
    PCR_TRY(ensure(ctx, ctx->b_table, need));
    PCR_TRY(ensure_pinned(ctx, std::max<size_t>(4096, std::max(sizeof(VoxRange) * F, sizeof(uint32_t) * (F + 1)))));
    char *p = (char *)ctx->b_table.p;
    unsigned long long *kA = (unsigned long long *)p;
    p += sizeof(unsigned long long) * n;
    unsigned long long *kB = (unsigned long long *)p;
    p += sizeof(unsigned long long) * n;
    uint32_t *vA = (uint32_t *)p;
    p += sizeof(uint32_t) * n;
    uint32_t *vB = (uint32_t *)p;
    p += sizeof(uint32_t) * n;
    uint32_t *hist = (uint32_t *)p;
    p += sizeof(uint32_t) * (256 * n_tiles + 1);
    uint32_t *vid = (uint32_t *)p;
    p += sizeof(uint32_t) * (n + 1);
    uint32_t *start = (uint32_t *)p;
    p += sizeof(uint32_t) * (n + 1);
    uint32_t *d_off = (uint32_t *)p;
    p += sizeof(uint32_t) * (F + 1);
    uint32_t *d_out_off = (uint32_t *)p;
    p += sizeof(uint32_t) * (F + 1);
    VoxRange *d_range = (VoxRange *)p;

    std::vector<uint32_t> h_off(F + 1);
    size_t longest = 0;
    for (int f = 0; f <= F; f++) h_off[f] = (uint32_t)frame_offsets[f];
    for (int f = 0; f < F; f++) longest = std::max<size_t>(longest, h_off[f + 1] - h_off[f]);
    PCR_CUDA(ctx, cudaMemcpyAsync(d_off, h_off.data(), sizeof(uint32_t) * (F + 1), cudaMemcpyHostToDevice, st));
    vox_init_kernel<<<(F + 255) / 256, 256, 0, st>>>(d_range, F);
    PCR_LAUNCH_CHECK(ctx);
    const unsigned bx = (unsigned)std::max<size_t>(1, std::min<size_t>((longest + 255) / 256, (size_t)ctx->sm_count * 8 / F));
    vox_range_kernel<<<dim3(bx, F), 256, 0, st>>>(dx, dy, dz, d_off, n, voxel, d_range);
    PCR_LAUNCH_CHECK(ctx);
    VoxRange *h_range = (VoxRange *)ctx->pinned;
    PCR_CUDA(ctx, cudaMemcpyAsync(h_range, d_range, sizeof(VoxRange) * F, cudaMemcpyDeviceToHost, st));
    PCR_MARK("voxel batch: wait for ranges");
    PCR_CUDA(ctx, cudaStreamSynchronize(st));
    uint64_t m64 = 0;
    int bits[3] = {0, 0, 0};
    for (int f = 0; f < F; f++) {
        if (!h_range[f].finite) continue;
        m64 += h_range[f].finite;
        for (int a = 0; a < 3; a++)
            bits[a] = std::max(bits[a], bits_for((uint64_t)((int64_t)h_range[f].mx[a] - (int64_t)h_range[f].mn[a]) + 1));
    }
    if (m64 == 0) return PCR_OK;
    const uint32_t m = (uint32_t)m64;
    const int fbits = bits_for((uint64_t)F), key_bits = bits[0] + bits[1] + bits[2];
    const bool packed = fbits + key_bits <= 63;

    const unsigned nb = (unsigned)((n + 255) / 256);
    if (packed) {
        const unsigned long long last = 1ull << (fbits + key_bits);
        vox_pack_kernel<<<nb, 256, 0, st>>>(dx, dy, dz, nullptr, n, voxel, -1, 0, 0, 0, bits[1] + bits[2], bits[2], last, kA, vA, d_off, F,
                                            d_range, key_bits);
        PCR_LAUNCH_CHECK(ctx);
        PCR_TRY(radix_sort_pairs_dev(ctx, &kA, &vA, &kB, &vB, n, fbits + key_bits + 1, hist));
        vox_heads_kernel<<<(m + 1 + 255) / 256, 256, 0, st>>>(kA, m, vid);
        PCR_LAUNCH_CHECK(ctx);
    } else {
        for (int axis = 2; axis >= 0; axis--) {
            vox_pack_kernel<<<nb, 256, 0, st>>>(dx, dy, dz, axis == 2 ? nullptr : vA, n, voxel, axis, 0, 0, 0, 0, 0, 1ull << 32, kA, vA, nullptr, 1,
                                                nullptr, 0);
            PCR_LAUNCH_CHECK(ctx);
            PCR_TRY(radix_sort_pairs_dev(ctx, &kA, &vA, &kB, &vB, n, 33, hist));
        }
        if (F > 1) {
            vox_pack_kernel<<<nb, 256, 0, st>>>(dx, dy, dz, vA, n, voxel, 3, 0, 0, 0, 0, 0, (unsigned long long)F, kA, vA, d_off, F, nullptr, 0);
            PCR_LAUNCH_CHECK(ctx);
            PCR_TRY(radix_sort_pairs_dev(ctx, &kA, &vA, &kB, &vB, n, bits_for((uint64_t)F + 1), hist));
        }
        vox_heads_triple_kernel<<<(m + 1 + 255) / 256, 256, 0, st>>>(dx, dy, dz, vA, m, voxel, d_off, F, vid);
        PCR_LAUNCH_CHECK(ctx);
    }
    PCR_TRY(exclusive_scan_u32_dev(ctx, vid, (size_t)m + 1));
    vox_starts_kernel<<<(m + 1 + 255) / 256, 256, 0, st>>>(vid, m, start);
    PCR_LAUNCH_CHECK(ctx);
    vox_mean_kernel<<<(m + 127) / 128, 128, 0, st>>>(dx, dy, dz, vA, start, vid + m, d_ox, d_oy, d_oz);
    PCR_LAUNCH_CHECK(ctx);
    vox_frame_starts_kernel<<<(m + 1 + 255) / 256, 256, 0, st>>>(kA, vA, m, packed ? key_bits : -1, d_off, F, vid, d_out_off);
    PCR_LAUNCH_CHECK(ctx);
// ... 10 lines not shown
```

Baseline: 267.2 million.

## Defer voxel downsample count sync until the cloud is used

```diff
diff --git a/include/pcr_b200.h b/include/pcr_b200.h
--- a/include/pcr_b200.h
+++ b/include/pcr_b200.h
@@ -44,6 +44,8 @@
 int pcr_ctx_set_frame_stream(pcr_ctx *ctx, int enable);
 #define PCR_NUM_HINT_STATS 8
 int pcr_ctx_get_hint_stats(pcr_ctx *ctx, uint64_t out[PCR_NUM_HINT_STATS]);
+#define PCR_NUM_HINT_STATS_EX 10
+int pcr_ctx_get_hint_stats_ex(pcr_ctx *ctx, uint64_t *out, size_t n);
 
 #define PCR_UNIQUE_ID_BYTES 128
 int pcr_comm_unique_id(void *out_id );
diff --git a/pointclouds_rs_b200/__init__.py b/pointclouds_rs_b200/__init__.py
--- a/pointclouds_rs_b200/__init__.py
+++ b/pointclouds_rs_b200/__init__.py
@@ -82,10 +82,11 @@
         return {"queries": int(out[0]), "candidates": int(out[1])}
 
     def hint_stats(self) -> dict:
-        out = (C.c_uint64 * 8)()
-        _ffi.check(_ffi.load().pcr_ctx_get_hint_stats(self._h, out), self._h)
         names = ("cell_size_reused", "cell_size_probed", "voxel_box_guess_held", "voxel_box_guess_missed", "coarser_level_ahead_needed",
-                 "coarser_level_ahead_unneeded", "deferred_counts_not_awaited_zero", "deferred_counts_not_awaited_nonzero")
+                 "coarser_level_ahead_unneeded", "deferred_counts_not_awaited_zero", "deferred_counts_not_awaited_nonzero",
+                 "voxel_count_left_pending", "voxel_guess_tall_column_redone")
+        out = (C.c_uint64 * len(names))()
+        _ffi.check(_ffi.load().pcr_ctx_get_hint_stats_ex(self._h, out, len(names)), self._h)
         return {k: int(v) for k, v in zip(names, out)}
 
     def set_query_sharding(self, enable: bool = True):
diff --git a/pointclouds_rs_b200/_ffi.py b/pointclouds_rs_b200/_ffi.py
--- a/pointclouds_rs_b200/_ffi.py
+++ b/pointclouds_rs_b200/_ffi.py
@@ -63,6 +63,7 @@
     "pcr_ctx_set_cell_size": (C.c_int, [vp, C.c_float]),
     "pcr_ctx_set_frame_stream": (C.c_int, [vp, C.c_int]),
     "pcr_ctx_get_hint_stats": (C.c_int, [vp, u64p]),
+    "pcr_ctx_get_hint_stats_ex": (C.c_int, [vp, u64p, C.c_size_t]),
     "pcr_ctx_get_knn_counters": (C.c_int, [vp, u64p]),
     "pcr_ctx_set_query_sharding": (C.c_int, [vp, C.c_int]),
     "pcr_ctx_debug_set_shard": (C.c_int, [vp, C.c_int, C.c_int]),
diff --git a/pointclouds_rs_b200/csrc/api.cu b/pointclouds_rs_b200/csrc/api.cu
--- a/pointclouds_rs_b200/csrc/api.cu
+++ b/pointclouds_rs_b200/csrc/api.cu
@@ -5,6 +5,7 @@
 #include <atomic>
 #include <chrono>
 #include <cstring>
+#include <string>
 #include <utility>
 #include <vector>
 #include <algorithm>
@@ -278,6 +279,10 @@
     }
     if (c->ev_fork) cudaEventDestroy(c->ev_fork);
     if (c->ev_count) cudaEventDestroy(c->ev_count);
+    for (auto &mb : c->vox_mail) {
+        cudaFreeHost(mb.hdr);
+        cudaEventDestroy(mb.ev);
+    }
     if (c->pinned) cudaFreeHost(c->pinned);
     if (c->owns_stream) cudaStreamDestroy(c->stream);
     cudaGetLastError();
@@ -374,6 +379,16 @@
     const uint64_t v[PCR_NUM_HINT_STATS] = {c.stat_cell_hits, c.stat_cell_misses, c.stat_vox_hits, c.stat_vox_misses, c.stat_spec_hits, c.stat_spec_misses,
                                              c.stat_nowait_hits, c.stat_nowait_misses};
     for (int i = 0; i < PCR_NUM_HINT_STATS; i++) out[i] = v[i];
+    return PCR_OK;
+}
+
+int pcr_ctx_get_hint_stats_ex(pcr_ctx *ctx, uint64_t *out, size_t n) {
+    if (!ctx || (n && !out)) return fail(ctx ? &ctx->c : nullptr, PCR_ERR_INVALID_ARG, "null pointer");
+    uint64_t v[PCR_NUM_HINT_STATS_EX];
+    PCR_TRY(pcr_ctx_get_hint_stats(ctx, v));
+    v[PCR_NUM_HINT_STATS] = ctx->c.stat_vox_pending;
+    v[PCR_NUM_HINT_STATS + 1] = ctx->c.stat_vox_tall;
+    for (size_t i = 0; i < n && i < PCR_NUM_HINT_STATS_EX; i++) out[i] = v[i];
     return PCR_OK;
 }
 
@@ -1600,30 +1615,26 @@
     }
 }
 }
-static int batch_core(Ctx *c, const float *dx, const float *dy, const float *dz, const uint64_t *frame_offsets, size_t n_frames,
-                      size_t n, size_t k_sor, float std_mul, size_t k_normals, const float vp[3], uint8_t *d_keep, float *d_nx,
-                      float *d_ny, float *d_nz, unsigned long long *d_kept ,
-                      unsigned long long *h_kept0 = nullptr ,
-                      const CloudStats *known_stats = nullptr ,
-                      bool allow_nowait = true ) {
-    const int F = (int)n_frames;
-    StreamAlloc<float> mean_mem(c->stream), stats_mem(c->stream);
-    PCR_CUDA(c, mean_mem.alloc(sizeof(float) * std::max<size_t>(n, 1)));
-    PCR_CUDA(c, stats_mem.alloc(sizeof(float) * 4 * F));
-    float *d_mean = mean_mem.p, *d_stats = stats_mem.p;
-
+struct CorePrelude {
+    StreamAlloc<float> mean, stats;
+    StreamAlloc<uint32_t> lists;
+    SorLists sl;
+    bool fuse = false;
+    explicit CorePrelude(cudaStream_t s) : mean(s), stats(s), lists(s) {}
+};
+static int core_prelude(Ctx *c, size_t n_cap, int F, size_t k_sor, size_t k_normals, unsigned long long *d_kept, CorePrelude &pre) {
+    PCR_CUDA(c, pre.mean.alloc(sizeof(float) * std::max<size_t>(n_cap, 1)));
+    PCR_CUDA(c, pre.stats.alloc(sizeof(float) * 4 * F));
     const size_t K = std::max(k_sor, k_normals) + 1;
     static const bool no_fuse = getenv("PCR_NO_LIST_REUSE") != nullptr;
-    const bool may_fuse = !no_fuse && k_sor > 0 && k_normals > 0 && K <= 32 && n > 1;
-    SorLists sl;
-    bool early = false;
-    StreamAlloc<uint32_t> list_mem(c->stream);
-    if (may_fuse) {
+    pre.fuse = !no_fuse && k_sor > 0 && k_normals > 0 && K <= 32 && n_cap > 1;
+    if (pre.fuse) {
+        SorLists &sl = pre.sl;
         sl.K = K;
-        sl.stride = (n + 63) & ~(size_t)63;
+        sl.stride = (n_cap + 63) & ~(size_t)63;
         const size_t bytes = sizeof(uint32_t) * (K * sl.stride + sl.stride + 64) + sl.stride;
-        PCR_CUDA(c, list_mem.alloc(bytes));
-        sl.lists = list_mem.p;
+        PCR_CUDA(c, pre.lists.alloc(bytes));
+        sl.lists = pre.lists.p;
         sl.fallback = sl.lists + K * sl.stride;
         sl.cnt = (uint8_t *)(sl.fallback + sl.stride + 64);
         PCR_CUDA(c, cudaMemsetAsync(sl.fallback + sl.stride, 0, 64 * sizeof(uint32_t), c->stream));
@@ -1632,6 +1643,24 @@
         PCR_MARK("core: lists allocated");
     }
     if (k_sor > 0) PCR_CUDA(c, cudaMemsetAsync(d_kept, 0, sizeof(unsigned long long) * F, c->stream));
+    return PCR_OK;
+}
+
+static int batch_core(Ctx *c, const float *dx, const float *dy, const float *dz, const uint64_t *frame_offsets, size_t n_frames,
+                      size_t n, size_t k_sor, float std_mul, size_t k_normals, const float vp[3], uint8_t *d_keep, float *d_nx,
+                      float *d_ny, float *d_nz, unsigned long long *d_kept ,
+                      unsigned long long *h_kept0 = nullptr ,
+                      const CloudStats *known_stats = nullptr ,
+                      bool allow_nowait = true ,
+                      CorePrelude *queued = nullptr ) {
+    const int F = (int)n_frames;
+    CorePrelude own(c->stream);
+    if (!queued) PCR_TRY(core_prelude(c, n, F, k_sor, k_normals, d_kept, own));
+    CorePrelude &pre = queued ? *queued : own;
+    float *d_mean = pre.mean.p, *d_stats = pre.stats.p;
+    const bool may_fuse = pre.fuse;
+    SorLists &sl = pre.sl;
+    bool early = false;
     BuildOpts bo;
     bo.k_hint = std::max(k_sor + 1, k_normals);
     bo.self_knn = true;
@@ -1772,6 +1801,7 @@
     pcr_ctx *owner = nullptr;
     size_t n = 0, stride = 0;
     float *base = nullptr;
+    std::shared_ptr<float> mem;
     bool has_normals = false;
     int arrays() const { return has_normals ? 6 : 3; }
     float *x() const { return base; }
@@ -1784,6 +1814,12 @@
 
 struct pcr_cloud : DevPoints {
     pcr::CloudStats stats;
+    pcr::VoxPending pend;
+    std::shared_ptr<float> src;
+    const float *sx = nullptr, *sy = nullptr, *sz = nullptr;
+    float voxel = 0.f;
+    int resolve_status = PCR_OK;
+    std::string resolve_error;
 };
 
 namespace pcr {
@@ -1806,18 +1842,36 @@
     float *base = nullptr;
     PCR_CUDA(&ctx->c, cudaMallocAsync((void **)&base, sizeof(float) * h->stride * h->arrays() + tail, ctx->c.stream));
     h->base = base;
+    h->mem.reset(base, [ctx](float *p) {
+        DevSetter ds(&ctx->c);
+        cudaFreeAsync(p, ctx->c.stream);
+    });
     out = std::move(h);
     return PCR_OK;
 }
 
 template <class H>
 void handle_free(H *h) {
-    if (!h) return;
-    if (h->base && h->owner) {
-        DevSetter ds(&h->owner->c);
-        cudaFreeAsync(h->base, h->owner->c.stream);
-    }
     delete h;
+}
+
+int cloud_resolve(const pcr_cloud *cloud) {
+    pcr_cloud *cl = const_cast<pcr_cloud *>(cloud);
+    Ctx *c = &cl->owner->c;
+    if (cl->resolve_status != PCR_OK) return fail(c, cl->resolve_status, "%s", cl->resolve_error.c_str());
+    if (!cl->pend.active) return PCR_OK;
+    DevSetter ds(c);
+    size_t m = 0;
+    const int s = voxel_finish(c, &cl->pend, cl->sx, cl->sy, cl->sz, cl->n, cl->voxel, cl->x(), cl->y(), cl->z(), &m, &cl->stats);
+    cl->src.reset();
+    if (s != PCR_OK) {
+        cl->n = 0;
+        cl->resolve_status = s;
+        cl->resolve_error = "voxel_downsample failed: " + c->err;
+        return s;
+    }
+    cl->n = m;
+    return PCR_OK;
 }
 
 __global__ void mask_to_u32_kernel(const uint8_t *__restrict__ keep, size_t n, uint32_t *__restrict__ flag) {
@@ -1982,6 +2036,11 @@
     return fail(nullptr, PCR_ERR_INVALID_ARG, "%s is NULL", what);
 }
 
+int cloud_ready(const pcr_cloud *cloud) {
+    PCR_TRY(handle_check(cloud, "cloud"));
+    return cloud_resolve(cloud);
+}
+
 }
 }
 
@@ -2003,20 +2062,23 @@
     PCR_API_END(c)
 }
 
-void pcr_cloud_free(pcr_cloud *cloud) { handle_free(cloud); }
-
-size_t pcr_cloud_len(const pcr_cloud *cloud) { return cloud ? cloud->n : 0; }
+void pcr_cloud_free(pcr_cloud *cloud) {
+    if (cloud && cloud->owner) vox_mail_release(&cloud->owner->c, &cloud->pend);
+    handle_free(cloud);
+}
+
+size_t pcr_cloud_len(const pcr_cloud *cloud) { return cloud && cloud->owner && cloud_resolve(cloud) == PCR_OK ? cloud->n : 0; }
 int pcr_cloud_has_normals(const pcr_cloud *cloud) { return cloud && cloud->has_normals ? 1 : 0; }
 
 int pcr_cloud_device_pointers(const pcr_cloud *cloud, const float **d_x, const float **d_y, const float **d_z, const float **d_nx,
                               const float **d_ny, const float **d_nz) {
-    PCR_TRY(handle_check(cloud, "cloud"));
+    PCR_TRY(cloud_ready(cloud));
     points_device_pointers(cloud, d_x, d_y, d_z, d_nx, d_ny, d_nz);
     return PCR_OK;
 }
 
 int pcr_cloud_download(const pcr_cloud *cloud, float *x, float *y, float *z) {
-    PCR_TRY(handle_check(cloud, "cloud"));
+    PCR_TRY(cloud_ready(cloud));
     Ctx *c = &cloud->owner->c;
     if (cloud->n && (!x || !y || !z)) return fail(c, PCR_ERR_INVALID_ARG, "null pointer");
     if (!cloud->n) return PCR_OK;
@@ -2027,7 +2089,7 @@
 }
 
 int pcr_cloud_download_normals(const pcr_cloud *cloud, float *nx, float *ny, float *nz) {
-    PCR_TRY(handle_check(cloud, "cloud"));
+    PCR_TRY(cloud_ready(cloud));
     Ctx *c = &cloud->owner->c;
     if (!cloud->has_normals) return fail(c, PCR_ERR_INVALID_ARG, "the cloud has no normals");
     if (cloud->n && (!nx || !ny || !nz)) return fail(c, PCR_ERR_INVALID_ARG, "null pointer");
@@ -2054,7 +2116,7 @@
 }
 
 int pcr_cloud_download_rows(const pcr_cloud *cloud, float *xyz, float *normals) {
-    PCR_TRY(handle_check(cloud, "cloud"));
+    PCR_TRY(cloud_ready(cloud));
     Ctx *c = &cloud->owner->c;
     if (normals && !cloud->has_normals) return fail(c, PCR_ERR_INVALID_ARG, "the cloud has no normals");
     if (cloud->n && !xyz && !normals) return fail(c, PCR_ERR_INVALID_ARG, "null pointer");
@@ -2139,7 +2201,7 @@
 }
 
 int pcr_cloud_download_block(const pcr_cloud *cloud, float *dst, size_t stride, int with_normals) {
-    PCR_TRY(handle_check(cloud, "cloud"));
+    PCR_TRY(cloud_ready(cloud));
     Ctx *c = &cloud->owner->c;
     if (with_normals && !cloud->has_normals) return fail(c, PCR_ERR_INVALID_ARG, "the cloud has no normals");
     if ((cloud->n && !dst) || stride < cloud->n) return fail(c, PCR_ERR_INVALID_ARG, "null pointer or stride < len");
@@ -2154,7 +2216,7 @@
 }
 
 int pcr_cloud_select(const pcr_cloud *cloud, const uint32_t *indices, size_t m, pcr_cloud **out) {
-    PCR_TRY(handle_check(cloud, "cloud"));
+    PCR_TRY(cloud_ready(cloud));
     Ctx *c = &cloud->owner->c;
     if (!out || (m && !indices)) return fail(c, PCR_ERR_INVALID_ARG, "null pointer");
     *out = nullptr;
@@ -2178,7 +2240,7 @@
 }
 
 int pcr_cloud_voxel_downsample(const pcr_cloud *cloud, float voxel_size, pcr_cloud **out) {
-    PCR_TRY(handle_check(cloud, "cloud"));
+    PCR_TRY(cloud_ready(cloud));
     Ctx *c = &cloud->owner->c;
     if (!out) return fail(c, PCR_ERR_INVALID_ARG, "null pointer");
     *out = nullptr;
@@ -2189,8 +2251,14 @@
     CloudPtr res;
     PCR_TRY(points_alloc(cloud->owner, cloud->n, false, res));
     size_t m = 0;
-    PCR_TRY(voxel_downsample_dev(c, cloud->x(), cloud->y(), cloud->z(), cloud->n, voxel_size, res->x(), res->y(), res->z(), &m, &res->stats));
+    PCR_TRY(voxel_downsample_dev(c, cloud->x(), cloud->y(), cloud->z(), cloud->n, voxel_size, res->x(), res->y(), res->z(), &m, &res->stats, true,
+                                 &res->pend));
     res->n = m;
+    if (res->pend.active) {
+        res->src = cloud->mem;
+        res->sx = cloud->x(), res->sy = cloud->y(), res->sz = cloud->z();
+        res->voxel = voxel_size;
+    }
     *out = res.release();
     PCR_MARK("voxel: exit");
     return PCR_OK;
@@ -2198,7 +2266,7 @@
 }
 
 int pcr_cloud_statistical_outlier_removal(const pcr_cloud *cloud, size_t k, float std_mul, pcr_cloud **out) {
-    PCR_TRY(handle_check(cloud, "cloud"));
+    PCR_TRY(cloud_ready(cloud));
     Ctx *c = &cloud->owner->c;
     if (!out) return fail(c, PCR_ERR_INVALID_ARG, "null pointer");
     *out = nullptr;
@@ -2220,7 +2288,7 @@
 }
 
 int pcr_cloud_radius_outlier_removal(const pcr_cloud *cloud, float radius, size_t min_neighbors, pcr_cloud **out) {
-    PCR_TRY(handle_check(cloud, "cloud"));
+    PCR_TRY(cloud_ready(cloud));
     Ctx *c = &cloud->owner->c;
     if (!out) return fail(c, PCR_ERR_INVALID_ARG, "null pointer");
     *out = nullptr;
@@ -2242,7 +2310,7 @@
 }
 
 int pcr_cloud_estimate_normals(const pcr_cloud *cloud, size_t k, const float viewpoint[3], pcr_cloud **out) {
-    PCR_TRY(handle_check(cloud, "cloud"));
+    PCR_TRY(cloud_ready(cloud));
     Ctx *c = &cloud->owner->c;
     if (!out) return fail(c, PCR_ERR_INVALID_ARG, "null pointer");
     *out = nullptr;
@@ -2274,6 +2342,7 @@
     const size_t n = cloud->n;
     CloudPtr res;
     if (n == 0 || k_sor == 0) {
+        PCR_TRY(cloud_resolve(cloud));
         PCR_TRY(points_alloc(cloud->owner, 0, true, res));
         *out = res.release();
         return PCR_OK;
@@ -2286,11 +2355,21 @@
     PCR_TRY(ensure(c, c->b_in2, n + 512));
     uint8_t *d_keep = (uint8_t *)c->b_in2.p;
     unsigned long long *d_kept = (unsigned long long *)((char *)c->b_in2.p + ((n + 255) & ~(size_t)255));
-    const uint64_t offs[2] = {0, n};
+    CorePrelude pre(c->stream);
+    PCR_TRY(core_prelude(c, n, 1, k_sor, k_normals, d_kept, pre));
+    PCR_TRY(cloud_resolve(cloud));
+    const size_t m = cloud->n;
+    if (m == 0) {
+        PCR_TRY(points_alloc(cloud->owner, 0, true, res));
+        *out = res.release();
+        return PCR_OK;
+    }
+    const uint64_t offs[2] = {0, m};
     const float vp0[3] = {0.f, 0.f, 0.f};
     unsigned long long h_kept = ~0ull;
-    PCR_TRY(batch_core(c, cloud->x(), cloud->y(), cloud->z(), offs, 1, n, k_sor, std_mul, k_normals, viewpoint ? viewpoint : vp0, d_keep,
-                       d_nrm, d_nrm + stride, d_nrm + 2 * stride, d_kept, &h_kept, cloud->stats.valid ? &cloud->stats : nullptr));
+    PCR_TRY(batch_core(c, cloud->x(), cloud->y(), cloud->z(), offs, 1, m, k_sor, std_mul, k_normals, viewpoint ? viewpoint : vp0, d_keep,
+                       d_nrm, d_nrm + stride, d_nrm + 2 * stride, d_kept, &h_kept, cloud->stats.valid ? &cloud->stats : nullptr, true,
+                       m > 1 ? &pre : nullptr ));
     PCR_MARK("sor_normals: core done");
     PCR_TRY(cloud_compact(cloud, d_keep, res, d_nrm, stride, h_kept == ~0ull ? SIZE_MAX : (size_t)h_kept));
     PCR_MARK("sor_normals: exit");
@@ -2301,7 +2380,7 @@
 
 int pcr_cloud_euclidean_cluster(const pcr_cloud *cloud, float distance_threshold, size_t min_size, size_t max_size, uint32_t *offsets,
                                 uint32_t *indices, size_t *n_clusters) {
-    PCR_TRY(handle_check(cloud, "cloud"));
+    PCR_TRY(cloud_ready(cloud));
     Ctx *c = &cloud->owner->c;
     if (n_clusters) *n_clusters = 0;
     if (!offsets || !n_clusters) return fail(c, PCR_ERR_INVALID_ARG, "null pointer");
@@ -2351,7 +2430,7 @@
 
 int pcr_cloud_ransac_plane_samples(const pcr_cloud *cloud, float distance_threshold, const uint32_t *samples, size_t m, float model[4],
                                    uint32_t *inliers, size_t *n_inliers) {
-    PCR_TRY(handle_check(cloud, "cloud"));
+    PCR_TRY(cloud_ready(cloud));
     Ctx *c = &cloud->owner->c;
     if (!model || !n_inliers || (m && !samples) || (cloud->n && !inliers)) return fail(c, PCR_ERR_INVALID_ARG, "null pointer");
     PCR_API_BEGIN
@@ -2361,7 +2440,7 @@
 }
 
 int pcr_cloud_apply_transform(const pcr_cloud *cloud, const float rotation[9], const float translation[3], pcr_cloud **out) {
-    PCR_TRY(handle_check(cloud, "cloud"));
+    PCR_TRY(cloud_ready(cloud));
     Ctx *c = &cloud->owner->c;
     if (!out || !rotation || !translation) return fail(c, PCR_ERR_INVALID_ARG, "null pointer");
     *out = nullptr;
@@ -2376,17 +2455,19 @@
 }
 
 int pcr_cloud_icp_point_to_point(const pcr_cloud *source, const pcr_cloud *target, const pcr_icp_params *params, pcr_icp_result *result) {
-    PCR_TRY(handle_check(source, "cloud"));
+    PCR_TRY(cloud_ready(source));
     Ctx *c = &source->owner->c;
     if (!target || target->owner != source->owner) return fail(c, PCR_ERR_INVALID_ARG, "source and target must live on the same context");
+    PCR_TRY(cloud_resolve(target));
     return pcr_icp_point_to_point_dev(source->owner, source->x(), source->y(), source->z(), source->n, target->x(), target->y(), target->z(),
                                       target->n, params, result);
 }
 
 int pcr_cloud_icp_point_to_plane(const pcr_cloud *source, const pcr_cloud *target, const pcr_icp_params *params, pcr_icp_result *result) {
-    PCR_TRY(handle_check(source, "cloud"));
+    PCR_TRY(cloud_ready(source));
     Ctx *c = &source->owner->c;
     if (!target || target->owner != source->owner) return fail(c, PCR_ERR_INVALID_ARG, "source and target must live on the same context");
+    PCR_TRY(cloud_resolve(target));
     if (!target->has_normals)
         return fail(c, PCR_ERR_INVALID_ARG, "target cloud must have normals (call estimate_normals first)");
     return pcr_icp_point_to_plane_dev(source->owner, source->x(), source->y(), source->z(), source->n, target->x(), target->y(), target->z(),
diff --git a/pointclouds_rs_b200/csrc/pcr_internal.cuh b/pointclouds_rs_b200/csrc/pcr_internal.cuh
--- a/pointclouds_rs_b200/csrc/pcr_internal.cuh
+++ b/pointclouds_rs_b200/csrc/pcr_internal.cuh
@@ -36,6 +36,15 @@
 };
 
 struct Ctx;
+
+struct VoxMail {
+    void *hdr = nullptr;
+    cudaEvent_t ev = nullptr;
+};
+struct VoxPending {
+    bool active = false;
+    VoxMail mail;
+};
 
 constexpr int kPeerMaxWorld = 8;
 constexpr int kPeerWords = 32;
@@ -96,6 +105,7 @@
         int uses = 0;
         int pad_shift = 6;
     } vox_cache;
+    std::vector<VoxMail> vox_mail;
     DevBuf b_in;
     DevBuf b_in2;
     DevBuf b_out;
@@ -145,6 +155,8 @@
     bool shard_queries = false;
     bool fake_comm = false;
     uint64_t stat_cell_hits = 0, stat_cell_misses = 0, stat_vox_hits = 0, stat_vox_misses = 0, stat_spec_hits = 0, stat_spec_misses = 0;
+    uint64_t stat_vox_pending = 0;
+    uint64_t stat_vox_tall = 0;
 };
 
 int fail(Ctx *ctx, int code, const char *fmt, ...);
@@ -313,7 +325,11 @@
 
 int voxel_downsample_dev(Ctx *ctx, const float *dx, const float *dy, const float *dz, size_t n, float voxel, float *d_ox, float *d_oy,
                          float *d_oz, size_t *n_out, CloudStats *stats_out = nullptr ,
-                         bool allow_guess = true );
+                         bool allow_guess = true ,
+                         VoxPending *pending = nullptr);
+int voxel_finish(Ctx *ctx, VoxPending *pending, const float *dx, const float *dy, const float *dz, size_t n, float voxel, float *d_ox, float *d_oy,
+                 float *d_oz, size_t *n_out, CloudStats *stats_out);
+void vox_mail_release(Ctx *ctx, VoxPending *pending);
 int voxel_downsample_batch_dev(Ctx *ctx, const float *dx, const float *dy, const float *dz, const uint64_t *frame_offsets,
                                size_t n_frames, float voxel, float *d_ox, float *d_oy, float *d_oz, uint64_t *out_offsets);
 int radix_sort_pairs_dev(Ctx *ctx, unsigned long long **keys, uint32_t **vals, unsigned long long **keys_alt, uint32_t **vals_alt,
diff --git a/pointclouds_rs_b200/csrc/voxel.cu b/pointclouds_rs_b200/csrc/voxel.cu
--- a/pointclouds_rs_b200/csrc/voxel.cu
+++ b/pointclouds_rs_b200/csrc/voxel.cu
@@ -499,8 +499,62 @@
     return PCR_OK;
 }
 
+namespace {
+
+void column_result(const VoxHeader *h, size_t *n_out, CloudStats *stats_out) {
+    *n_out = h->total;
+    if (!stats_out) return;
+    for (int a = 0; a < 3; a++) {
+        stats_out->mn[a] = ~h->mn_c[a];
+        stats_out->mx[a] = h->mx[a];
+    }
+    stats_out->count = h->count;
+    stats_out->valid = 1;
+}
+
+int guessed_result(Ctx *ctx, const VoxHeader *h, const float *dx, const float *dy, const float *dz, size_t n, float voxel, float *d_ox,
+                   float *d_oy, float *d_oz, size_t *n_out, CloudStats *stats_out) {
+    auto &vc = ctx->vox_cache;
+    (h->outside ? ctx->stat_vox_misses : ctx->stat_vox_hits)++;
+    if (h->outside) {
+        vc.valid = false;
+        vc.pad_shift = std::max(2, vc.pad_shift - 1);
+        return voxel_downsample_dev(ctx, dx, dy, dz, n, voxel, d_ox, d_oy, d_oz, n_out, stats_out, false);
+    }
+    if (h->tall) {
+        ctx->stat_vox_tall++;
+        vc.valid = false;
+        return voxel_downsample_dev(ctx, dx, dy, dz, n, voxel, d_ox, d_oy, d_oz, n_out, stats_out, false);
+    }
+    column_result(h, n_out, stats_out);
+    return PCR_OK;
+}
+
+}
+
+int voxel_finish(Ctx *ctx, VoxPending *pending, const float *dx, const float *dy, const float *dz, size_t n, float voxel, float *d_ox, float *d_oy,
+                 float *d_oz, size_t *n_out, CloudStats *stats_out) {
+    *n_out = 0;
+    if (stats_out) stats_out->valid = 0;
+    const VoxMail mb = pending->mail;
+    pending->active = false;
+    PCR_MARK("voxel: wait for the pending count");
+    const cudaError_t e = cudaEventSynchronize(mb.ev);
+    PCR_MARK("voxel: got the pending count");
+    const VoxHeader h = *(const VoxHeader *)mb.hdr;
+    ctx->vox_mail.push_back(mb);
+    PCR_CUDA(ctx, e);
+    return guessed_result(ctx, &h, dx, dy, dz, n, voxel, d_ox, d_oy, d_oz, n_out, stats_out);
+}
+
+void vox_mail_release(Ctx *ctx, VoxPending *pending) {
+    if (!pending->active) return;
+    pending->active = false;
+    ctx->vox_mail.push_back(pending->mail);
+}
+
 int voxel_downsample_dev(Ctx *ctx, const float *dx, const float *dy, const float *dz, size_t n, float voxel, float *d_ox, float *d_oy,
-                         float *d_oz, size_t *n_out, CloudStats *stats_out, bool allow_guess) {
+                         float *d_oz, size_t *n_out, CloudStats *stats_out, bool allow_guess, VoxPending *pending) {
     *n_out = 0;
     if (stats_out) stats_out->valid = 0;
     if (n == 0) return PCR_OK;
@@ -593,32 +647,38 @@
             ctx->launches++;
             PCR_CUDA(ctx, launch_chained(vox_out_stats_kernel, dim3((unsigned)ctx->sm_count), dim3(256), 0, st, d_ox, d_oy, d_oz, nvox + n, d_hdr));
             ctx->launches++;
+            if (guessed && pending) {
+                if (ctx->vox_mail.empty()) {
+                    VoxMail mb;
+                    PCR_CUDA(ctx, cudaHostAlloc(&mb.hdr, sizeof(VoxHeader), cudaHostAllocPortable));
+                    const cudaError_t e = cudaEventCreateWithFlags(&mb.ev, cudaEventDisableTiming);
+                    if (e != cudaSuccess) cudaFreeHost(mb.hdr);
+                    PCR_CUDA(ctx, e);
+                    ctx->vox_mail.push_back(mb);
+                }
+                const VoxMail mb = ctx->vox_mail.back();
+                cudaError_t e = cudaStreamWaitEvent(st, mb.ev, 0);
+                if (e == cudaSuccess) e = cudaMemcpyAsync(mb.hdr, d_hdr, sizeof(VoxHeader), cudaMemcpyDeviceToHost, st);
+                if (e == cudaSuccess) e = cudaEventRecord(mb.ev, st);
+                PCR_CUDA(ctx, e);
+                ctx->vox_mail.pop_back();
+                pending->mail = mb;
+                pending->active = true;
+                ctx->stat_vox_pending++;
+                *n_out = n;
+                PCR_MARK("voxel: count left on the device");
+                return PCR_OK;
+            }
             VoxHeader *mail = (VoxHeader *)((uint32_t *)ctx->pinned + 64);
             PCR_CUDA(ctx, cudaMemcpyAsync(mail, d_hdr, sizeof(VoxHeader), cudaMemcpyDeviceToHost, st));
             PCR_MARK("voxel: wait for count");
             PCR_CUDA(ctx, cudaStreamSynchronize(st));
             PCR_MARK("voxel: got count");
-            if (guessed) (mail->outside ? ctx->stat_vox_misses : ctx->stat_vox_hits)++;
-            if (guessed && mail->outside) {
-                vc.valid = false;
-                vc.pad_shift = std::max(2, vc.pad_shift - 1);
-                return voxel_downsample_dev(ctx, dx, dy, dz, n, voxel, d_ox, d_oy, d_oz, n_out, stats_out, false);
-            }
-            const bool tall = mail->tall != 0;
-            if (tall && guessed) {
-                vc.valid = false;
-                return voxel_downsample_dev(ctx, dx, dy, dz, n, voxel, d_ox, d_oy, d_oz, n_out, stats_out, false);
-            }
-            if (!tall) *n_out = mail->total;
-            if (!tall && stats_out) {
-                for (int a = 0; a < 3; a++) {
-                    stats_out->mn[a] = ~mail->mn_c[a];
-                    stats_out->mx[a] = mail->mx[a];
-                }
-                stats_out->count = mail->count;
-                stats_out->valid = 1;
-            }
-            if (!tall) return PCR_OK;
+            if (guessed) return guessed_result(ctx, mail, dx, dy, dz, n, voxel, d_ox, d_oy, d_oz, n_out, stats_out);
+            if (!mail->tall) {
+                column_result(mail, n_out, stats_out);
+                return PCR_OK;
+            }
         }
     }
     if (guessed) {
```

Measured after the change: 279.7 million (median of 6 runs). 4.7% higher.
